# sortmerna/sortmerna

Hardware: AMD Instinct MI355X
Metric: reads/sec (150 bp vs smr_v4.3_default_db-sized DB) (higher is better)
Workload: dtype u8/i32

## Files before the change

### include/smr_hip.h

```cpp
#ifndef SMR_HIP_H
#define SMR_HIP_H
#include <stddef.h>
#include <stdint.h>

#ifdef __cplusplus
extern "C" {
#endif

#define SMR_OK 0
#define SMR_ERR_ARG (-1)
#define SMR_ERR_IO (-2)
#define SMR_ERR_DEVICE (-3)
#define SMR_ERR_CAPACITY (-4)
#define SMR_ERR_STATE (-5)

typedef struct smr_ctx smr_ctx;
typedef struct smr_index smr_index;
typedef struct smr_reads smr_reads;

typedef struct {
  uint32_t skiplengths[3];
  int32_t  num_seeds;
  int32_t  min_lis;
  int32_t  edges;
  int32_t  is_as_percent;
  int32_t  match;
  int32_t  mismatch;
  int32_t  score_N;
  int32_t  gap_open;
  int32_t  gap_ext;
  uint32_t num_alignments;
  int32_t  is_best;
  int32_t  is_full_search;
  int32_t  is_forward;
  int32_t  is_reverse;
  uint32_t minoccur;
  uint32_t minimal_score;
  uint32_t index_num;
  uint32_t part;
  int32_t  is_last_index_part;
} smr_params;

void smr_params_default(smr_params* p);
const char* smr_params_refused(const smr_params* p);

int smr_index_load_files(const char* prefix, uint32_t part, const char* ref_fasta, smr_index** out, char* err, size_t errcap);

int smr_index_build(const char* ref_fasta, uint32_t seed_win_len, double max_file_size_mb, uint32_t max_pos,
                    uint32_t threads, smr_index** parts_out, uint32_t cap_parts, uint32_t* n_parts_out,
                    char* err, size_t errcap);
int smr_index_write_files(const smr_index* const* parts, uint32_t n_parts, const char* ref_fasta, const char* prefix,
                          char* err, size_t errcap);
int smr_index_save(const smr_index*, const char* path, uint64_t stamp, char* err, size_t errcap);
int smr_index_load_flat(const char* path, uint64_t stamp, smr_index** out, char* err, size_t errcap);
int smr_index_selfcheck(smr_index*, char* err, size_t errcap);
void smr_index_free(smr_index*);

typedef struct {
  uint32_t lnwin;
  uint32_t n_kmers;
  uint64_t trie_words;
  uint32_t n_ids;
  uint64_t n_pos;
  uint32_t n_refs;
  uint64_t ref_bytes;
  uint64_t n_nodes, n_buckets, n_entries;
  double   bg[4];
  uint64_t full_len;
  uint64_t numseq;
  uint32_t n_parts;
} smr_index_info;
int smr_index_get_info(const smr_index*, smr_index_info* out);

uint32_t smr_minimal_score(double lambda, double K, const double bg[4], uint64_t full_ref_len, uint64_t numseq,
                           uint64_t all_reads_count, uint64_t all_reads_len, double evalue);
uint32_t smr_minimal_score_split(double lambda, double K, const double bg[4], uint64_t full_ref_len, uint64_t numseq,
                                 uint64_t all_reads_count, uint64_t all_reads_len, double evalue, uint32_t full_read_scale);

void smr_refstats_corrected(double K, const double bg[4], uint64_t full_ref_len, uint64_t numseq, uint64_t all_reads_count, uint64_t all_reads_len,
                            uint64_t* full_ref_corr, uint64_t* full_read_corr);
void smr_refstats_corrected_split(double K, const double bg[4], uint64_t full_ref_len, uint64_t numseq, uint64_t all_reads_count, uint64_t all_reads_len,
                                  uint32_t full_read_scale, uint64_t* full_ref_corr, uint64_t* full_read_corr);

int smr_reads_pack(const char* seqs, const uint64_t* offs, uint32_t n_reads, smr_reads** out);
int smr_reads_load_fastx(const char* path, uint64_t first, uint64_t count, smr_reads** out, char* err, size_t errcap);
int smr_reads_load_fastx_mt(const char* path, uint32_t threads, smr_reads** out, char* err, size_t errcap);
void smr_reads_free(smr_reads*);
int smr_reads_slice(const smr_reads*, uint64_t first, uint64_t count, smr_reads** out);
int smr_reads_load_fastx_text(const char* path, uint32_t threads, smr_reads** out, char* err, size_t errcap);
int smr_reads_is_fastq(const smr_reads*);
int smr_reads_record_text(const smr_reads*, uint32_t i, char* hdr, size_t hdr_cap, char* seq, size_t seq_cap, char* qual, size_t qual_cap, size_t lens[3]);
uint64_t smr_reads_digest(const smr_reads*);
uint32_t smr_reads_count(const smr_reads*);
uint64_t smr_reads_total_len(const smr_reads*);
uint32_t smr_reads_min_len(const smr_reads*);
uint32_t smr_reads_max_len(const smr_reads*);

int  smr_device_count(void);
int  smr_create(int device, smr_ctx** out, char* err, size_t errcap);
void smr_destroy(smr_ctx*);
const char* smr_last_error(const smr_ctx*);
int  smr_tuning_text(const smr_ctx*, char* buf, size_t cap);

int smr_index_upload(smr_ctx*, const smr_index*, int slot);
int smr_index_check_device(smr_ctx*, int slot, smr_index*);
int smr_index_pigeonhole(smr_index*, const uint32_t** pg, uint64_t* pg_words, const uint32_t** root3, uint64_t* root3_words, char* err, size_t errcap);
int smr_seed_tuples_fetch(smr_ctx*, uint64_t* tuples, uint64_t cap_tuples, uint32_t* cbase, uint32_t cap_cbase, uint32_t meta[8]);
int smr_seed_pool_info(smr_ctx*, uint64_t info[4]);
#define SMR_ROUTE_RECORD 1u
#define SMR_ROUTE_GATHER 2u
#define SMR_ROUTE_CHAIN 4u
#define SMR_ROUTE_EXT 8u
int smr_cand_info_enable(smr_ctx*, int on);
int smr_cand_info(smr_ctx*, uint64_t info[13]);
int smr_cand_routes(smr_ctx*, uint8_t* out, uint32_t n);
int smr_index_unload(smr_ctx*, int slot);

int smr_batch_select(smr_ctx*, int batch);

int smr_set_seed_mode(smr_ctx*, int exact_counters);

int smr_reads_upload(smr_ctx*, const smr_reads*, uint32_t max_alignments_per_read);
int smr_reads_upload_batch(smr_ctx*, int batch, const smr_reads*, uint32_t max_alignments_per_read);
#define SMR_FASTX_VIEW 1u
#define SMR_FASTX_KEEP 2u
#define SMR_FASTX_INFLATE 4u
int smr_reads_upload_fastx(smr_ctx*, const char* text, uint64_t n_bytes, uint32_t max_alignments_per_read, uint32_t flags, smr_reads** out);
int smr_reads_upload_fastx_batch(smr_ctx*, int batch, const char* text, uint64_t n_bytes, uint32_t max_alignments_per_read, uint32_t flags, smr_reads** out);
int smr_reads_upload_fastx_file(smr_ctx*, const char* path, uint32_t max_alignments_per_read, uint32_t flags, smr_reads** out, char* err, size_t errcap);
int smr_fastx_info(const smr_ctx*, uint64_t info[4]);
int smr_fastx_times(const smr_ctx*, double ms[5]);
typedef struct {
  int32_t layout;
  int32_t paired_in, paired_out, out2, sout;
  int32_t want_aligned, want_other;
} smr_fxsplit_opts;
int smr_fastx_split(smr_ctx*, int mates , const smr_fxsplit_opts*,
                    const uint8_t* hit , uint8_t* bytes, uint64_t cap, uint64_t off[9], uint64_t* need);
int smr_fastx_split_times(const smr_ctx*, double ms[4]);
typedef struct {
  int  want_sam, want_blast;
  char blast_cols[64];
  double lambda, K;
  uint64_t full_ref_corr, full_read_corr;
} smr_rows_opts;
int smr_rows_part(smr_ctx*, int slot, const smr_params*, const smr_index* ix, const smr_rows_opts*,
                  uint8_t* bytes, uint64_t cap, uint64_t off[3], uint64_t* need);
int smr_rows_times(const smr_ctx*, double ms[4]);
int smr_rows_fmt_batch(smr_ctx*, uint32_t n, const uint32_t* num, const uint32_t* den, char* out);
int smr_pairwise_part(smr_ctx*, int slot, const smr_params*, const smr_index* ix, double lambda, double K, uint64_t full_ref_corr, uint64_t full_read_corr,
                      uint8_t* bytes, uint64_t cap, uint64_t* need);
int smr_pairwise_times(const smr_ctx*, double ms[4]);
typedef struct { uint32_t ref_num, n_reads; uint64_t off; } smr_otu_group;
int smr_otu_part(smr_ctx*, int slot, const smr_params*, const smr_index* ix, double min_id, double min_cov,
                 uint8_t* bytes, uint64_t cap, smr_otu_group* groups, uint64_t groups_cap, uint64_t need[2] , int* any_yid_ycov);
int smr_otu_times(const smr_ctx*, double ms[5]);
int smr_otu_sort_batch(smr_ctx*, uint32_t n, const uint32_t* keys, uint32_t key_bits, uint32_t* perm);
int smr_fastx_denovo(smr_ctx*, int mates, const smr_fxsplit_opts*, const uint8_t* dn ,
                     uint8_t* bytes, uint64_t cap, uint64_t off[5], uint64_t* need);

uint32_t smr_gzip_chunk(void);
uint64_t smr_gzip_bound(uint64_t plain_bytes, uint64_t n_chunks);
int smr_gzip_batch(smr_ctx*, const uint8_t* plain, const uint64_t* off , uint32_t n_streams,
                   uint8_t* gz, uint64_t cap, uint64_t* gz_off , uint64_t* need);
int smr_fastx_split_gz(smr_ctx*, int mates, const smr_fxsplit_opts*, const uint8_t* hit,
                       uint8_t* gz, uint64_t cap, uint64_t gz_off[9], uint64_t plain_off[9], uint64_t* need);
int smr_fastx_denovo_gz(smr_ctx*, int mates, const smr_fxsplit_opts*, const uint8_t* dn,
                        uint8_t* gz, uint64_t cap, uint64_t gz_off[5], uint64_t plain_off[5], uint64_t* need);
uint64_t smr_gzip_lines_bound(uint64_t plain_bytes, uint32_t n_streams);
int smr_gzip_lines_batch(smr_ctx*, const uint8_t* plain, const uint64_t* off , uint32_t n_streams,
                         uint8_t* gz, uint64_t cap, uint64_t* gz_off , uint64_t* need);
int smr_rows_part_gz(smr_ctx*, int slot, const smr_params*, const smr_index* ix, const smr_rows_opts*,
                     uint8_t* gz, uint64_t cap, uint64_t gz_off[3], uint64_t plain_off[3], uint64_t* need);
int smr_pairwise_part_gz(smr_ctx*, int slot, const smr_params*, const smr_index* ix, double lambda, double K, uint64_t full_ref_corr, uint64_t full_read_corr,
                         uint8_t* gz, uint64_t cap, uint64_t* plain_bytes, uint64_t* need);
int smr_gzip_times(const smr_ctx*, double ms[5]);

int smr_rows_part_mates(smr_ctx*, int mates, int slot, const smr_params*, const smr_index* ix, const smr_rows_opts*,
                        uint8_t* bytes, uint64_t cap, uint64_t off[3], uint64_t* need);
int smr_pairwise_part_mates(smr_ctx*, int mates, int slot, const smr_params*, const smr_index* ix, double lambda, double K,
                            uint64_t full_ref_corr, uint64_t full_read_corr, uint8_t* bytes, uint64_t cap, uint64_t* need);
int smr_rows_part_mates_gz(smr_ctx*, int mates, int slot, const smr_params*, const smr_index* ix, const smr_rows_opts*,
                           uint8_t* gz, uint64_t cap, uint64_t gz_off[3], uint64_t plain_off[3], uint64_t* need);
int smr_pairwise_part_mates_gz(smr_ctx*, int mates, int slot, const smr_params*, const smr_index* ix, double lambda, double K,
                               uint64_t full_ref_corr, uint64_t full_read_corr, uint8_t* gz, uint64_t cap,
                               uint64_t* plain_bytes, uint64_t* need);
int smr_interleave_batch(smr_ctx*, uint32_t n, const uint8_t* a, const uint64_t* a_off, const uint8_t* b, const uint64_t* b_off,
                         uint8_t* out, uint64_t cap, uint64_t* need);
int smr_mates_times(const smr_ctx*, double ms[4]);

int smr_gunzip_batch(smr_ctx*, const uint8_t* gz, uint64_t n, uint64_t grain , uint8_t* plain, uint64_t cap, uint64_t* need);
int smr_gunzip_info(const smr_ctx*, uint64_t info[8]);
int smr_gunzip_times(const smr_ctx*, double ms[6]);
int smr_gunzip_tasks(const smr_ctx*, uint64_t* starts, uint64_t cap, uint64_t* count);
int smr_state_reset(smr_ctx*);

int smr_align_part(smr_ctx*, int slot, const smr_params*);
int smr_traceback(smr_ctx*, int slot, const smr_params*);

int smr_counters(smr_ctx*, uint64_t* out, uint32_t n_db);
int smr_counters_device(smr_ctx*, void** dptr, uint32_t* n_u64);
int smr_counters_accumulate(smr_ctx*, void* d_acc, uint32_t n_u64);

int smr_idcov_part(smr_ctx*, int slot, const smr_params*, double min_id, double min_cov);
int smr_idcov_counters(smr_ctx*, uint64_t out[4]);
int smr_idcov_counters_device(smr_ctx*, void** dptr, uint32_t* n_u64);
#define SMR_COUNTERS_WITH_IDCOV 70
int smr_idcov_batch(smr_ctx*, uint32_t n, const uint8_t* reads, const uint64_t* read_off, const uint8_t* refs, const uint64_t* ref_off,
                    const uint32_t* cigars, const uint64_t* cigar_off, const int32_t* read_begin, const int32_t* read_end, const uint32_t* readlen,
                    double min_id, double min_cov, uint32_t* out);

int    smr_results_fetch(smr_ctx*);
size_t smr_result_record(const smr_ctx*, uint32_t read_idx, uint8_t* buf, size_t cap);
size_t smr_result_record_batch(const smr_ctx*, int batch, uint32_t read_idx, uint8_t* buf, size_t cap);
int    smr_result_is_hit(const smr_ctx*, uint32_t read_idx);

int smr_state_import(smr_ctx*, const uint8_t* bytes, const uint64_t* off, uint32_t n);
int smr_state_export(smr_ctx*, uint8_t* bytes, uint64_t cap, uint64_t* off, uint32_t n, uint64_t* need);
int smr_counters_import(smr_ctx*, const uint64_t* in, uint32_t n_db);

int smr_seed_scan(smr_ctx*, int slot, const smr_params*, int strand, int pass, uint64_t* n_hits_out);
int smr_seed_hits_fetch(smr_ctx*, uint32_t* triples, uint64_t cap_triples, uint64_t* n_out);

typedef struct {
  double   seed_ms;  uint64_t seed_launches;
  double   chain_ms; uint64_t chain_launches;
  double   trace_ms; uint64_t trace_launches;
  uint64_t n_windows, n_lookup, n_node, n_entry, n_hit, n_read_bytes;
  uint64_t n_sw_fwd, n_sw_rev, n_sw_cells;
  uint64_t n_sw_spec, n_sw_spec_used;
  uint64_t n_seed_redo;
  uint64_t hit_list_cap;
  uint64_t n_seed_shared;
  uint64_t n_seed_shared_builds;
} smr_prof;
int smr_index_build_gpu(smr_ctx*, const char* ref_fasta, uint32_t lnwin, double max_mb, uint32_t max_pos,
                        smr_index** parts_out, uint32_t cap_parts, uint32_t* n_parts_out, char* err, size_t errcap);

int smr_sw_selfcheck(smr_ctx*, uint32_t n_cases, uint32_t seed, uint32_t max_len, uint64_t* n_bad);
int smr_sw_mode(smr_ctx*, int set_to);
int smr_walk_rounds(const smr_ctx*, uint32_t out[3]);
int smr_ssw_batch(smr_ctx*, uint32_t n_pairs, const uint8_t* reads, const uint64_t* read_off, const uint8_t* refs, const uint64_t* ref_off,
                  int match, int mismatch, int score_N, int gap_open, int gap_ext, uint32_t filters, int mode, int32_t* out);
int smr_sw_long_rows(int m);
typedef struct {
  uint32_t read, win_off;
  uint16_t aq, m, nref;
  uint8_t reversed, list_b;
} smr_sw16_task;
int smr_sw16_batch(smr_ctx*, uint32_t n_tasks, const smr_sw16_task* tasks, const uint8_t* ref, uint64_t ref_len, int force_any_n,
                   int match, int mismatch, int score_N, int gap_open, int gap_ext, uint32_t filters, int rows, uint32_t blocks, int32_t* out);
typedef struct {
  uint32_t read, win_off;
  uint16_t aq, m, nref, cols;
  uint8_t reversed, pad_[3];
} smr_sw16_prefix_task;
int smr_sw16_prefix_batch(smr_ctx*, uint32_t n_tasks, const smr_sw16_prefix_task* tasks, const uint8_t* ref, uint64_t ref_len, int force_any_n,
                          int match, int mismatch, int score_N, int gap_open, int gap_ext, int rows, uint32_t blocks, int32_t* out);
int smr_walk_prefix_stats(smr_ctx*, uint64_t out[8]);
int smr_sw16_launches(const smr_ctx*, uint64_t out[8]);
int smr_sw16_f16(smr_ctx*, int set_to, uint64_t* launches);
// ... 80 lines not shown
```

### sortmerna_amd/capi.py

```python
import ctypes as C
import os

from . import build as _build


class Params(C.Structure):
    _fields_ = [
        ("skiplengths", C.c_uint32 * 3), ("num_seeds", C.c_int32), ("min_lis", C.c_int32), ("edges", C.c_int32),
        ("is_as_percent", C.c_int32), ("match", C.c_int32), ("mismatch", C.c_int32), ("score_N", C.c_int32),
        ("gap_open", C.c_int32), ("gap_ext", C.c_int32), ("num_alignments", C.c_uint32), ("is_best", C.c_int32),
        ("is_full_search", C.c_int32), ("is_forward", C.c_int32), ("is_reverse", C.c_int32), ("minoccur", C.c_uint32),
        ("minimal_score", C.c_uint32), ("index_num", C.c_uint32), ("part", C.c_uint32),
        ("is_last_index_part", C.c_int32),
    ]


class IndexInfo(C.Structure):
    _fields_ = [
        ("lnwin", C.c_uint32), ("n_kmers", C.c_uint32), ("trie_words", C.c_uint64), ("n_ids", C.c_uint32),
        ("n_pos", C.c_uint64), ("n_refs", C.c_uint32), ("ref_bytes", C.c_uint64), ("n_nodes", C.c_uint64),
        ("n_buckets", C.c_uint64), ("n_entries", C.c_uint64), ("bg", C.c_double * 4), ("full_len", C.c_uint64),
        ("numseq", C.c_uint64), ("n_parts", C.c_uint32),
    ]


class ReportOpts(C.Structure):
    _fields_ = [("fastx", C.c_int), ("other", C.c_int), ("blast_tabular", C.c_int), ("blast_cols", C.c_char * 64), ("sam", C.c_int),
                ("blast_pairwise", C.c_int), ("sam_sq", C.c_int), ("paired_in", C.c_int), ("paired_out", C.c_int), ("out2", C.c_int), ("sout", C.c_int), ("zip_out", C.c_int),
                ("otu_map", C.c_int), ("denovo", C.c_int), ("min_id", C.c_double), ("min_cov", C.c_double)]


class FxSplitOpts(C.Structure):
    _fields_ = [("layout", C.c_int32), ("paired_in", C.c_int32), ("paired_out", C.c_int32), ("out2", C.c_int32), ("sout", C.c_int32),
                ("want_aligned", C.c_int32), ("want_other", C.c_int32)]


class RowsOpts(C.Structure):
    _fields_ = [("want_sam", C.c_int), ("want_blast", C.c_int), ("blast_cols", C.c_char * 64), ("lam", C.c_double), ("K", C.c_double),
                ("full_ref_corr", C.c_uint64), ("full_read_corr", C.c_uint64)]


class SummaryDb(C.Structure):
    _fields_ = [("ref_file", C.c_char_p), ("skiplengths", C.c_uint32 * 3), ("lam", C.c_double), ("K", C.c_double),
                ("minimal_score", C.c_uint32), ("reads_matched", C.c_uint64)]


class Summary(C.Structure):
    _fields_ = [("cmdline", C.c_char_p), ("pid", C.c_char_p), ("timestamp", C.c_char_p), ("seed_len", C.c_uint32),
                ("num_seeds", C.c_int32), ("edges", C.c_int32), ("match", C.c_int32), ("mismatch", C.c_int32), ("gap_open", C.c_int32),
                ("gap_ext", C.c_int32), ("score_N", C.c_int32), ("sam_sq", C.c_int32), ("threads", C.c_int32),
                ("reads_files", C.POINTER(C.c_char_p)), ("n_reads_files", C.c_uint32),
                ("total_reads", C.c_uint64), ("num_aligned", C.c_uint64), ("all_reads_len", C.c_uint64),
                ("min_read_len", C.c_uint32), ("max_read_len", C.c_uint32), ("dbs", C.POINTER(SummaryDb)), ("n_dbs", C.c_uint32),
                ("is_denovo", C.c_int), ("total_denovo", C.c_uint64), ("is_otu_map", C.c_int), ("total_id_cov", C.c_uint64), ("total_otu", C.c_uint64)]


class Prof(C.Structure):
    _fields_ = [
        ("seed_ms", C.c_double), ("seed_launches", C.c_uint64), ("chain_ms", C.c_double), ("chain_launches", C.c_uint64),
        ("trace_ms", C.c_double), ("trace_launches", C.c_uint64), ("n_windows", C.c_uint64), ("n_lookup", C.c_uint64),
        ("n_node", C.c_uint64), ("n_entry", C.c_uint64), ("n_hit", C.c_uint64), ("n_read_bytes", C.c_uint64),
        ("n_sw_fwd", C.c_uint64), ("n_sw_rev", C.c_uint64), ("n_sw_cells", C.c_uint64), ("n_sw_spec", C.c_uint64), ("n_sw_spec_used", C.c_uint64), ("n_seed_redo", C.c_uint64), ("hit_list_cap", C.c_uint64),
        ("n_seed_shared", C.c_uint64), ("n_seed_shared_builds", C.c_uint64),
    ]


class Kprof(C.Structure):
    _fields_ = [("name", C.c_char * 32), ("ms", C.c_double), ("launches", C.c_uint64), ("bytes", C.c_uint64)]


EXPORTS = [
    "smr_rows_part_mates", "smr_pairwise_part_mates", "smr_rows_part_mates_gz", "smr_pairwise_part_mates_gz", "smr_interleave_batch", "smr_mates_times",
    "smr_gzip_lines_bound", "smr_gzip_lines_batch", "smr_rows_part_gz", "smr_pairwise_part_gz", "smr_report_add_rows_gz", "smr_report_add_pairwise_gz",
    "smr_gunzip_batch", "smr_gunzip_info", "smr_gunzip_times", "smr_gunzip_tasks",
    "smr_gzip_chunk", "smr_gzip_bound", "smr_gzip_batch", "smr_fastx_split_gz", "smr_fastx_denovo_gz", "smr_gzip_times", "smr_report_add_fastx_gz", "smr_report_add_denovo_gz",
    "smr_otu_part", "smr_otu_times", "smr_otu_sort_batch", "smr_fastx_denovo", "smr_report_add_otu", "smr_report_skip_otu", "smr_report_add_denovo", "smr_report_skip_denovo",
    "smr_params_default", "smr_params_refused", "smr_index_load_files", "smr_index_build", "smr_index_build_gpu", "smr_index_write_files", "smr_index_save", "smr_index_load_flat", "smr_index_selfcheck", "smr_index_free",
    "smr_index_get_info", "smr_minimal_score", "smr_minimal_score_split", "smr_refstats_corrected_split", "smr_reads_pack", "smr_reads_load_fastx", "smr_reads_load_fastx_mt", "smr_reads_load_fastx_text", "smr_reads_is_fastq", "smr_reads_record_text", "smr_reads_free", "smr_reads_slice",
    "smr_reads_digest", "smr_reads_count", "smr_reads_total_len", "smr_reads_min_len", "smr_reads_max_len", "smr_create", "smr_device_count", "smr_destroy",
    "smr_last_error", "smr_tuning_text", "smr_index_upload", "smr_index_check_device", "smr_index_pigeonhole", "smr_seed_tuples_fetch", "smr_seed_pool_info", "smr_cand_info_enable", "smr_cand_info", "smr_cand_routes", "smr_index_unload", "smr_batch_select", "smr_set_seed_mode", "smr_reads_upload", "smr_reads_upload_batch", "smr_reads_upload_fastx", "smr_reads_upload_fastx_batch", "smr_reads_upload_fastx_file", "smr_fastx_info", "smr_fastx_times", "smr_fastx_split", "smr_fastx_split_times", "smr_rows_part", "smr_rows_times", "smr_rows_fmt_batch", "smr_pairwise_part", "smr_pairwise_times", "smr_state_reset", "smr_align_part",
    "smr_traceback", "smr_counters", "smr_counters_device", "smr_state_import", "smr_state_export", "smr_counters_import", "smr_results_fetch", "smr_result_record", "smr_result_record_batch", "smr_counters_accumulate",
    "smr_result_is_hit", "smr_seed_scan", "smr_seed_hits_fetch", "smr_sw_selfcheck", "smr_sw_mode", "smr_walk_rounds", "smr_ssw_batch", "smr_sw16_batch", "smr_sw16_prefix_batch", "smr_walk_prefix_stats", "smr_sw16_launches", "smr_sw16_f16", "smr_sw_long_rows", "smr_cigar_batch", "smr_idcov_part", "smr_idcov_counters", "smr_idcov_counters_device", "smr_idcov_batch", "smr_prof_reset", "smr_prof_get", "smr_prof_kernels", "smr_refstats_corrected", "smr_report_open",
    "smr_report_set_db", "smr_report_set_part", "smr_report_add", "smr_report_add_pair", "smr_report_add_fastx", "smr_report_skip_fastx", "smr_report_add_rows", "smr_report_skip_rows", "smr_report_add_pairwise", "smr_report_skip_pairwise", "smr_report_set_cmdline", "smr_report_otu_count", "smr_report_otu_merge", "smr_report_close", "smr_report_last_error",
    "smr_summary_write", "smr_readstats_record", "smr_readstats_key",
]

_lib = None


def load(rebuild_if_stale=True):
    global _lib
    if _lib is not None:
        return _lib
    path = _build.LIB
    if rebuild_if_stale and _build.is_stale():
        path = _build.build_library()
    if not os.path.isfile(path):
        raise RuntimeError("libsmr_hip.so is missing; run sortmerna_amd/build.py (needs hipcc)")
    _lib = bind(C.CDLL(path))
    return _lib


def bind(L):
    vp, cp, u32, u64, i32 = C.c_void_p, C.c_char_p, C.c_uint32, C.c_uint64, C.c_int
    L.smr_params_default.argtypes = [C.POINTER(Params)]
    L.smr_index_load_files.restype = i32
    L.smr_index_load_files.argtypes = [cp, u32, cp, C.POINTER(vp), cp, C.c_size_t]
    L.smr_index_build.restype = i32
    L.smr_index_build.argtypes = [cp, u32, C.c_double, u32, u32, C.POINTER(vp), u32, C.POINTER(u32), cp, C.c_size_t]
    L.smr_index_build_gpu.restype = i32
    L.smr_index_build_gpu.argtypes = [vp, cp, u32, C.c_double, u32, C.POINTER(vp), u32, C.POINTER(u32), cp, C.c_size_t]
    L.smr_index_write_files.restype = i32
    L.smr_index_write_files.argtypes = [C.POINTER(vp), u32, cp, cp, cp, C.c_size_t]
    L.smr_index_save.restype = i32
    L.smr_index_save.argtypes = [vp, cp, u64, cp, C.c_size_t]
    L.smr_index_load_flat.restype = i32
    L.smr_index_load_flat.argtypes = [cp, u64, C.POINTER(vp), cp, C.c_size_t]
    L.smr_index_selfcheck.restype = i32
    L.smr_index_selfcheck.argtypes = [vp, cp, C.c_size_t]
    L.smr_index_free.argtypes = [vp]
    L.smr_index_get_info.restype = i32
    L.smr_index_get_info.argtypes = [vp, C.POINTER(IndexInfo)]
    L.smr_minimal_score.restype = u32
    L.smr_minimal_score.argtypes = [C.c_double, C.c_double, C.POINTER(C.c_double), u64, u64, u64, u64, C.c_double]
    L.smr_minimal_score_split.restype = u32
    L.smr_minimal_score_split.argtypes = [C.c_double, C.c_double, C.POINTER(C.c_double), u64, u64, u64, u64, C.c_double, u32]
    L.smr_reads_pack.restype = i32
    L.smr_reads_pack.argtypes = [cp, vp, u32, C.POINTER(vp)]
    L.smr_reads_load_fastx.restype = i32
    L.smr_reads_load_fastx.argtypes = [cp, u64, u64, C.POINTER(vp), cp, C.c_size_t]
    L.smr_reads_load_fastx_mt.restype = i32
    L.smr_reads_load_fastx_mt.argtypes = [cp, u32, C.POINTER(vp), cp, C.c_size_t]
    L.smr_reads_load_fastx_text.restype = i32
    L.smr_reads_load_fastx_text.argtypes = [cp, u32, C.POINTER(vp), cp, C.c_size_t]
    L.smr_reads_is_fastq.restype = i32
    L.smr_reads_is_fastq.argtypes = [vp]
    L.smr_reads_record_text.restype = i32
    L.smr_reads_record_text.argtypes = [vp, u32, cp, C.c_size_t, cp, C.c_size_t, cp, C.c_size_t, C.POINTER(C.c_size_t)]
    L.smr_reads_free.argtypes = [vp]
    for f in ("smr_reads_count", "smr_reads_min_len", "smr_reads_max_len"):
        getattr(L, f).restype = u32
        getattr(L, f).argtypes = [vp]
    L.smr_reads_digest.restype = u64
    L.smr_reads_digest.argtypes = [vp]
    L.smr_reads_total_len.restype = u64
    L.smr_reads_total_len.argtypes = [vp]
    L.smr_create.restype = i32
    L.smr_create.argtypes = [i32, C.POINTER(vp), cp, C.c_size_t]
    L.smr_destroy.argtypes = [vp]
    L.smr_last_error.restype = cp
    L.smr_last_error.argtypes = [vp]
    L.smr_tuning_text.restype = i32
    L.smr_tuning_text.argtypes = [vp, cp, C.c_size_t]
    L.smr_index_upload.restype = i32
    L.smr_index_upload.argtypes = [vp, vp, i32]
    L.smr_index_check_device.restype = i32
    L.smr_index_check_device.argtypes = [vp, i32, vp]
    L.smr_index_pigeonhole.restype = i32
    L.smr_index_pigeonhole.argtypes = [vp, C.POINTER(C.POINTER(C.c_uint32)), C.POINTER(u64), C.POINTER(C.POINTER(C.c_uint32)), C.POINTER(u64), cp, C.c_size_t]
    L.smr_seed_tuples_fetch.restype = i32
    L.smr_seed_tuples_fetch.argtypes = [vp, vp, u64, vp, u32, C.POINTER(u32)]
    L.smr_seed_pool_info.restype = i32
    L.smr_seed_pool_info.argtypes = [vp, C.POINTER(u64)]
    L.smr_cand_info_enable.restype = i32
    L.smr_cand_info_enable.argtypes = [vp, i32]
    L.smr_cand_info.restype = i32
    L.smr_cand_info.argtypes = [vp, C.POINTER(u64)]
    L.smr_cand_routes.restype = i32
    L.smr_cand_routes.argtypes = [vp, vp, u32]
    L.smr_index_unload.restype = i32
    L.smr_index_unload.argtypes = [vp, i32]
    L.smr_batch_select.restype = i32
    L.smr_batch_select.argtypes = [vp, i32]
    L.smr_set_seed_mode.restype = i32
    L.smr_set_seed_mode.argtypes = [vp, i32]
    L.smr_reads_upload.restype = i32
    L.smr_reads_upload.argtypes = [vp, vp, u32]
    L.smr_state_reset.restype = i32
    L.smr_state_reset.argtypes = [vp]
    L.smr_align_part.restype = i32
    L.smr_align_part.argtypes = [vp, i32, C.POINTER(Params)]
    L.smr_traceback.restype = i32
    L.smr_traceback.argtypes = [vp, i32, C.POINTER(Params)]
    L.smr_counters.restype = i32
    L.smr_counters.argtypes = [vp, C.POINTER(u64), u32]
    L.smr_state_import.restype = i32
    L.smr_state_import.argtypes = [vp, vp, vp, u32]
    L.smr_state_export.restype = i32
    L.smr_state_export.argtypes = [vp, vp, u64, vp, u32, C.POINTER(u64)]
    L.smr_counters_import.restype = i32
    L.smr_counters_import.argtypes = [vp, C.POINTER(u64), u32]
    L.smr_counters_device.restype = i32
    L.smr_counters_device.argtypes = [vp, C.POINTER(vp), C.POINTER(u32)]
    L.smr_results_fetch.restype = i32
    L.smr_results_fetch.argtypes = [vp]
    L.smr_result_record.restype = C.c_size_t
    L.smr_result_record.argtypes = [vp, u32, vp, C.c_size_t]
    L.smr_result_record_batch.restype = C.c_size_t
    L.smr_result_record_batch.argtypes = [vp, i32, u32, vp, C.c_size_t]
    L.smr_counters_accumulate.restype = i32
    L.smr_counters_accumulate.argtypes = [vp, vp, u32]
    L.smr_result_is_hit.restype = i32
    L.smr_result_is_hit.argtypes = [vp, u32]
    L.smr_seed_scan.restype = i32
    L.smr_seed_scan.argtypes = [vp, i32, C.POINTER(Params), i32, i32, C.POINTER(u64)]
    L.smr_seed_hits_fetch.restype = i32
    L.smr_seed_hits_fetch.argtypes = [vp, vp, u64, C.POINTER(u64)]
    L.smr_sw_selfcheck.restype = i32
    L.smr_sw_selfcheck.argtypes = [vp, u32, u32, u32, C.POINTER(u64)]
    L.smr_ssw_batch.restype = i32
    L.smr_ssw_batch.argtypes = [vp, u32, vp, vp, vp, vp, i32, i32, i32, i32, i32, u32, i32, vp]
    L.smr_sw16_batch.restype = i32
    L.smr_sw16_batch.argtypes = [vp, u32, vp, vp, u64, i32, i32, i32, i32, i32, i32, u32, i32, u32, vp]
    L.smr_sw16_prefix_batch.restype = i32
    L.smr_sw16_prefix_batch.argtypes = [vp, u32, vp, vp, u64, i32, i32, i32, i32, i32, i32, i32, u32, vp]
    L.smr_walk_prefix_stats.restype = i32
    L.smr_walk_prefix_stats.argtypes = [vp, C.POINTER(u64)]
    L.smr_sw16_launches.restype = i32
    L.smr_sw16_launches.argtypes = [vp, C.POINTER(u64)]
    L.smr_sw16_f16.restype = i32
    L.smr_sw16_f16.argtypes = [vp, i32, C.POINTER(u64)]
    L.smr_sw_long_rows.restype = i32
    L.smr_sw_long_rows.argtypes = [i32]
    L.smr_readstats_record.restype = C.c_size_t
    L.smr_readstats_record.argtypes = [u64, u64, u32, u32, u64, u64, vp, u32, vp, C.c_size_t]
    L.smr_readstats_key.restype = C.c_size_t
    L.smr_readstats_key.argtypes = [vp, u32, vp, C.c_size_t]
    L.smr_reads_upload_batch.restype = i32
    L.smr_reads_upload_batch.argtypes = [vp, i32, vp, u32]
    L.smr_reads_upload_fastx.restype = i32
    L.smr_reads_upload_fastx.argtypes = [vp, vp, u64, u32, u32, C.POINTER(vp)]
    L.smr_reads_upload_fastx_batch.restype = i32
    L.smr_reads_upload_fastx_batch.argtypes = [vp, i32, vp, u64, u32, u32, C.POINTER(vp)]
    L.smr_reads_upload_fastx_file.restype = i32
    L.smr_reads_upload_fastx_file.argtypes = [vp, cp, u32, u32, C.POINTER(vp), cp, C.c_size_t]
    L.smr_fastx_info.restype = i32
    L.smr_fastx_info.argtypes = [vp, C.POINTER(u64)]
    L.smr_fastx_times.restype = i32
    L.smr_fastx_times.argtypes = [vp, C.POINTER(C.c_double)]
    L.smr_fastx_split.restype = i32
    L.smr_fastx_split.argtypes = [vp, i32, C.POINTER(FxSplitOpts), vp, vp, u64, C.POINTER(u64), C.POINTER(u64)]
    L.smr_fastx_split_times.restype = i32
    L.smr_fastx_split_times.argtypes = [vp, C.POINTER(C.c_double)]
    L.smr_rows_part.restype = i32
    L.smr_rows_part.argtypes = [vp, i32, C.POINTER(Params), vp, C.POINTER(RowsOpts), vp, u64, C.POINTER(u64), C.POINTER(u64)]
    L.smr_rows_times.restype = i32
    L.smr_rows_times.argtypes = [vp, C.POINTER(C.c_double)]
    L.smr_rows_fmt_batch.restype = i32
    L.smr_rows_fmt_batch.argtypes = [vp, u32, vp, vp, vp]
    L.smr_report_add_rows.restype = i32
    L.smr_report_add_rows.argtypes = [vp, u32, u32, vp, C.POINTER(u64)]
    L.smr_report_skip_rows.restype = i32
    L.smr_report_skip_rows.argtypes = [vp, i32]
    L.smr_pairwise_part.restype = i32
    L.smr_pairwise_part.argtypes = [vp, i32, C.POINTER(Params), vp, C.c_double, C.c_double, u64, u64, vp, u64, C.POINTER(u64)]
    L.smr_pairwise_times.restype = i32
    L.smr_pairwise_times.argtypes = [vp, C.POINTER(C.c_double)]
    L.smr_report_add_pairwise.restype = i32
    L.smr_report_add_pairwise.argtypes = [vp, u32, u32, vp, u64]
    L.smr_report_skip_pairwise.restype = i32
    L.smr_report_skip_pairwise.argtypes = [vp, i32]
    L.smr_otu_part.restype = i32
    L.smr_otu_part.argtypes = [vp, i32, C.POINTER(Params), vp, C.c_double, C.c_double, vp, u64, vp, u64, C.POINTER(u64), C.POINTER(i32)]
    L.smr_otu_times.restype = i32
    L.smr_otu_times.argtypes = [vp, C.POINTER(C.c_double)]
    L.smr_otu_sort_batch.restype = i32
    L.smr_otu_sort_batch.argtypes = [vp, u32, vp, u32, vp]
    L.smr_fastx_denovo.restype = i32
    L.smr_fastx_denovo.argtypes = [vp, i32, C.POINTER(FxSplitOpts), vp, vp, u64, C.POINTER(u64), C.POINTER(u64)]
    L.smr_gzip_chunk.restype = u32
    L.smr_gzip_chunk.argtypes = []
    L.smr_gzip_bound.restype = u64
    L.smr_gzip_bound.argtypes = [u64, u64]
    L.smr_gzip_batch.restype = i32
    L.smr_gzip_batch.argtypes = [vp, vp, C.POINTER(u64), u32, vp, u64, C.POINTER(u64), C.POINTER(u64)]
    L.smr_fastx_split_gz.restype = i32
    L.smr_fastx_split_gz.argtypes = [vp, i32, C.POINTER(FxSplitOpts), vp, vp, u64, C.POINTER(u64), C.POINTER(u64), C.POINTER(u64)]
    L.smr_fastx_denovo_gz.restype = i32
    L.smr_fastx_denovo_gz.argtypes = [vp, i32, C.POINTER(FxSplitOpts), vp, vp, u64, C.POINTER(u64), C.POINTER(u64), C.POINTER(u64)]
    L.smr_gzip_times.restype = i32
    L.smr_gzip_times.argtypes = [vp, C.POINTER(C.c_double)]
    L.smr_gzip_lines_bound.restype = u64
    L.smr_gzip_lines_bound.argtypes = [u64, u32]
    L.smr_gzip_lines_batch.restype = i32
    L.smr_gzip_lines_batch.argtypes = [vp, vp, C.POINTER(u64), u32, vp, u64, C.POINTER(u64), C.POINTER(u64)]
    L.smr_rows_part_mates.restype = i32
    L.smr_rows_part_mates.argtypes = [vp, i32, i32, C.POINTER(Params), vp, C.POINTER(RowsOpts), vp, u64, C.POINTER(u64), C.POINTER(u64)]
    L.smr_pairwise_part_mates.restype = i32
    L.smr_pairwise_part_mates.argtypes = [vp, i32, i32, C.POINTER(Params), vp, C.c_double, C.c_double, u64, u64, vp, u64, C.POINTER(u64)]
    L.smr_rows_part_mates_gz.restype = i32
    L.smr_rows_part_mates_gz.argtypes = [vp, i32, i32, C.POINTER(Params), vp, C.POINTER(RowsOpts), vp, u64, C.POINTER(u64), C.POINTER(u64), C.POINTER(u64)]
    L.smr_pairwise_part_mates_gz.restype = i32
    L.smr_pairwise_part_mates_gz.argtypes = [vp, i32, i32, C.POINTER(Params), vp, C.c_double, C.c_double, u64, u64, vp, u64, C.POINTER(u64), C.POINTER(u64)]
    L.smr_interleave_batch.restype = i32
    L.smr_interleave_batch.argtypes = [vp, u32, vp, C.POINTER(u64), vp, C.POINTER(u64), vp, u64, C.POINTER(u64)]
    L.smr_mates_times.restype = i32
    L.smr_mates_times.argtypes = [vp, C.POINTER(C.c_double)]
    L.smr_rows_part_gz.restype = i32
    L.smr_rows_part_gz.argtypes = [vp, i32, C.POINTER(Params), vp, C.POINTER(RowsOpts), vp, u64, C.POINTER(u64), C.POINTER(u64), C.POINTER(u64)]
    L.smr_pairwise_part_gz.restype = i32
    L.smr_pairwise_part_gz.argtypes = [vp, i32, C.POINTER(Params), vp, C.c_double, C.c_double, u64, u64, vp, u64, C.POINTER(u64), C.POINTER(u64)]
    L.smr_report_add_rows_gz.restype = i32
    L.smr_report_add_rows_gz.argtypes = [vp, u32, u32, vp, C.POINTER(u64)]
    L.smr_report_add_pairwise_gz.restype = i32
    L.smr_report_add_pairwise_gz.argtypes = [vp, u32, u32, vp, u64]
    L.smr_gunzip_batch.restype = i32
    L.smr_gunzip_batch.argtypes = [vp, vp, u64, u64, vp, u64, C.POINTER(u64)]
    L.smr_gunzip_info.restype = i32
    L.smr_gunzip_info.argtypes = [vp, C.POINTER(u64)]
    L.smr_gunzip_times.restype = i32
    L.smr_gunzip_times.argtypes = [vp, C.POINTER(C.c_double)]
    L.smr_gunzip_tasks.restype = i32
    L.smr_gunzip_tasks.argtypes = [vp, C.POINTER(u64), u64, C.POINTER(u64)]
    L.smr_report_add_fastx_gz.restype = i32
    L.smr_report_add_fastx_gz.argtypes = [vp, vp, C.POINTER(u64)]
    L.smr_report_add_denovo_gz.restype = i32
# ... 64 lines not shown
```

### sortmerna_amd/csrc/smr_devbuf.hpp

```cpp
#pragma once
#include <hip/hip_runtime.h>

#include <cstddef>

struct smr_ctx;
int dev_fail(smr_ctx* c, const char* call, hipError_t e);

template <class T> class DevBuf {
  T* p_ = nullptr;
  size_t cap_ = 0;

 public:
  DevBuf() = default;
  DevBuf(const DevBuf&) = delete;
  DevBuf& operator=(const DevBuf&) = delete;
  DevBuf(DevBuf&& o) noexcept : p_(o.p_), cap_(o.cap_) { o.p_ = nullptr; o.cap_ = 0; }
  DevBuf& operator=(DevBuf&& o) noexcept {
    if (this != &o) { release(); p_ = o.p_; cap_ = o.cap_; o.p_ = nullptr; o.cap_ = 0; }
    return *this;
  }
  ~DevBuf() { release(); }

  operator T*() const { return p_; }
  T* get() const { return p_; }
  size_t cap() const { return cap_; }

  void release() {
    if (p_) (void)hipFree(p_);
    p_ = nullptr; cap_ = 0;
  }
  int alloc(smr_ctx* c, size_t count) {
    release();
    if (count == 0) count = 1;
    const hipError_t e = hipMalloc((void**)&p_, count * sizeof(T));
    if (e != hipSuccess) { p_ = nullptr; return dev_fail(c, "hipMalloc", e); }
    cap_ = count;
    return 0;
  }
  int reserve(smr_ctx* c, size_t need) { return (p_ && cap_ >= need) ? 0 : alloc(c, need); }
  int reserve_headroom(smr_ctx* c, size_t total, size_t slack) {
    return cap_ >= total + slack ? 0 : alloc(c, (size_t)((total + (total >> 3) + 4095u) & ~4095ull));
  }
};

struct DevStream {
  hipStream_t s = nullptr;
  DevStream() = default;
  DevStream(const DevStream&) = delete;
  DevStream& operator=(const DevStream&) = delete;
  ~DevStream() { if (s) (void)hipStreamDestroy(s); }
  operator hipStream_t() const { return s; }
};
```

### sortmerna_amd/csrc/smr_engine.hip

```cpp
#include <hip/hip_runtime.h>

#include <algorithm>
#include <mutex>
#include <cstdio>
#include <cstdlib>
#include <cstring>
#include <string>
#include <vector>

#include "smr_kernels.hpp"
#include "smr_idcov.hpp"
#include "smr_import.hpp"
#include "smr_export.hpp"
#include "smr_fastx.hpp"
#include "smr_fxsplit.hpp"
#include "smr_rows.hpp"
#include "smr_pairwise.hpp"
#include "smr_mates.hpp"
#include "smr_otu.hpp"
#include "smr_gzip.hpp"
#include "smr_gunzip.hpp"
#include "smr_ibuild.hpp"
#include "smr_pgbuild.hpp"
#include "smr_hostmem.hpp"
#include "smr_devbuf.hpp"
#include "smr_stage.hpp"
#include "smr_score_text.hpp"
#include "smr_tuning.hpp"

using namespace smr;

namespace {

struct DevIndex {
  bool used = false;
  DevBuf<Lookup> lookup; DevBuf<uint32_t> trie, pos_off; DevBuf<uint2> pos_arr;
  DevBuf<uint32_t> pg, root3, lkc;
  DevBuf<uint8_t> ref_seq; DevBuf<uint64_t> ref_off;
  uint32_t n_refs = 0, n_ids = 0, lnwin = 0;
  uint32_t ref_any_n = 1;
  uint64_t trie_words = 0, n_pos = 0, ref_bytes = 0, pg_words = 0;
  DevBuf<uint8_t> rows_names; DevBuf<uint32_t> rows_name_off; int64_t rows_part = -1;
};

struct EvMark { hipEvent_t e; int kind; };
struct EvPool {
  std::vector<EvMark> events; std::vector<hipEvent_t> pool;
  EvPool() = default;
  EvPool(const EvPool&) = delete;
  EvPool& operator=(const EvPool&) = delete;
  ~EvPool() { for (auto& m : events) (void)hipEventDestroy(m.e); for (auto& e : pool) (void)hipEventDestroy(e); }
};

}

#define SMR_MAX_BATCHES 16
enum { KP_KEYS = 0, KP_SPLIT, KP_BINS, KP_PG0, KP_PG1, KP_FINISH, KP_CAND, KP_CHAIN, KP_BEGINS, KP_TRACE, KP_WALK, KP_SW16, KP_WNEXT, KP_IDCOV, KP_COUNT };
static const char* const KP_NAME[KP_COUNT] = {"k_seed_keys", "k_seed_split", "k_seed_bins", "k_seed_pg<0>", "k_seed_pg<1>", "k_seed_finish", "k_cand", "k_chain", "k_begins", "k_trace",
                                              "k_walk", "k_sw16", "k_wnext", "k_idcov"};

struct Batch {
  bool used = false;
  uint32_t n = 0, max_len = 0, slots = 1;
  uint32_t min_ge[7] = {~0u, ~0u, ~0u, ~0u, ~0u, ~0u, ~0u};
  uint64_t gen = 0;
  bool min_ge_known = false;
  DevBuf<uint32_t> d_words; DevBuf<uint64_t> d_rec_off; DevBuf<uint32_t> d_len;
  DevBuf<RState> d_saved, d_work; DevBuf<RWork> d_rw;
  DevBuf<uint8_t> d_marks;
  DevBuf<AlignRec> d_saved_aln, d_work_aln;
  DevBuf<unsigned long long> d_ctr;
  DevBuf<uint32_t> d_cigar; uint64_t cigar_words = 0;
  DevBuf<uint32_t> d_idcov; bool idcov_ran = false;
  std::vector<uint32_t> h_idcov;
  std::vector<RState> h_state; std::vector<AlignRec> h_aln; std::vector<uint32_t> h_cigar;
  std::vector<uint32_t> h_idx, h_map;
  uint32_t last_num_alignments = 1;
  DevBuf<uint8_t> fx_text; DevBuf<unsigned long long> fx_hoff, fx_soff; uint32_t fx_n = 0; bool fx_fastq = false, fx_kept = false;
  unsigned long long redo_seen = 0, win_seen = 0;
  bool fetched = false;
};

struct SharedSet { DevBuf<SeedTup> srt; DevBuf<uint16_t> wbin; DevBuf<uint32_t> cbase, sn; uint32_t maxwin = 0; bool built = false; };
struct SharedSort {
  SharedSet set[2][3];
  const void* batch = nullptr; uint64_t gen = 0; uint32_t lnwin = 0, skip[3] = {0, 0, 0}, n = 0, max_len = 0;
  uint64_t cap[3] = {0, 0, 0};
  bool usable = false;
  DevBuf<uint32_t> abits;
};
struct SeedScratch {
  DevBuf<uint32_t> chist, cbase, rows, bcnt, wseg[2], fbits[2], zbits, gflag, emap, sn, redo, hpre, hlist, hh;
  DevBuf<SeedTup> tmp, mid, srt; DevBuf<uint16_t> wbin; DevBuf<uint2> pieces;
};

struct FxScratch {
  DevBuf<uint8_t> text;
  DevBuf<uint32_t> tot, part_t, part_l, line_start, lrec, lcum, hdr_line, rcum, rlen, rwi;
  DevBuf<unsigned long long> hoff, soff;
  StageClock<6, 0> clk;
};

struct FxSplitScratch {
  DevBuf<uint4> rec; DevBuf<unsigned long long> woff, part, tot; DevBuf<uint8_t> hit, out;
  StageClock<6, 4> clk;
};

struct RowsScratch {
  DevBuf<uint4> stat, meta; DevBuf<unsigned long long> excl_s, excl_b, part_s, part_b; DevBuf<uint32_t> err; DevBuf<uint8_t> tab, out;
  uint32_t tab_n = 0; double tab_lambda = 0, tab_K = 0; uint64_t tab_ref = 0, tab_read = 0;
  StageClock<7, 4> clk;
};

struct OtuScratch {
  DevBuf<uint8_t> pass, out; DevBuf<uint2> meta; DevBuf<uint4> pairs; DevBuf<uint32_t> key[2], val[2], gstart, err;
  DevBuf<unsigned long long> excl, part, hist, wexcl, wpart, gexcl, gpart; DevBuf<OtuGroup> groups;
  StageClock<10, 5> clk;
};

struct GzScratch {
  DevBuf<uint8_t> in, slots, out; DevBuf<GzChunk> chunks; DevBuf<GzCode> codes; DevBuf<unsigned long long> slot_off, sizes, cut_tab;
  DevBuf<uint32_t> crc_tab, crc, tok, freq, ntok;
  StageClock<4, 5> clk;
};

struct GunzScratch {
  DevBuf<uint32_t> in, n_cand, crc; DevBuf<unsigned long long> cand; DevBuf<GunzTask> tasks; DevBuf<GunzRes> res; DevBuf<GunzUnit> units;
  DevBuf<uint16_t> sym; DevBuf<uint8_t> win, out;
  StageClock<8, 6> clk;
};

struct smr_ctx {
  const Tuning tune;
  explicit smr_ctx(const Tuning& t) : tune(t) {}
  int device = 0;
  DevStream stream, upload_stream;
  std::string err;
  std::mutex err_m, sel_m;
  int n_cu = 256;
  DevIndex idx[64];
  Batch bt[SMR_MAX_BATCHES];
  Batch* b = &bt[0];
  DevBuf<uint32_t> d_pool; uint64_t pool_words = 0;
  uint64_t n_pool_grown = 0;
  uint32_t pool_inline = 0;
  uint32_t hcap = 4;
  int seed_exact = tune.seed_exact;
  uint32_t cand_bloom = tune.cand_bloom;
  int seed_shared = tune.seed_shared;
  DevBuf<uint16_t> d_sw_scr; uint32_t sw_scr_stride = 0;
  int last_seed_slot = -1;
  SharedSort shared;
  uint64_t n_seed_shared = 0, n_seed_shared_builds = 0;
  uint32_t ccap = tune.ccap;
  SeedScratch seed; SeedBufs sb = {};
  uint64_t sb_slots = 0; uint32_t sb_nk = 0;
  uint32_t chain_blocks = 0;
  DevBuf<unsigned long long> d_tuples; uint32_t chain_scap = 512;
  uint32_t keys_need = 0;
  bool chain_ext = false;
  DevBuf<uint32_t> d_stab; DevBuf<unsigned long long> d_tuples2;
  size_t chain_lds_attr = 0, begins_lds_attr = 0, split_lds_attr = 0, bins_lds_attr = 0;
  DevBuf<uint32_t> d_fidx; DevBuf<RState> d_fstate; DevBuf<AlignRec> d_faln;
  DevBuf<uint32_t> d_fidcov;
  DevBuf<uint8_t> d_xbytes; DevBuf<unsigned long long> d_xoff, d_xpart;
  int sw_mode = tune.sw_packed;
  DevBuf<unsigned long long> d_keys; uint32_t keys_cap = 0;
  DevBuf<unsigned long long> d_pairs; DevBuf<uint32_t> d_lis; uint32_t pairs_cap = 0;
  DevBuf<uint2> d_hits; uint32_t hits_cap = 0;
  DevBuf<uint8_t> d_rdq;
  DevBuf<uint2> d_mrec; DevBuf<uint32_t> d_mpool;
  DevBuf<uint2> d_wlist[2]; DevBuf<WState> d_wstate[2]; DevBuf<WTask> d_wtask[2]; DevBuf<uint2> d_wres[2];
  DevBuf<uint32_t> d_wtidx, d_wslow; DevBuf<unsigned long long> d_wctr; size_t walk_cap = 0; uint32_t walk_kcap = 0;
  size_t walk_lds_attr = 0, pg_lds_attr = 0, search_lds_attr = 0;
  int sw16_f16 = tune.sw16_f16;
  uint64_t sw16h_launches = 0;
  uint64_t sw16_launches[8] = {};
  uint32_t walk_need[3] = {0, 0, 0};
  DevBuf<unsigned long long> d_wpstat;
  bool pfx_live = true; uint32_t pfx_parts_off = 0; unsigned long long pfx_seen[2] = {0, 0};
  DevBuf<unsigned long long> d_wstat; uint32_t wstat_n = 0; int wstat_pass[8] = {}; uint32_t wstat_rm[8] = {};
  DevBuf<int> d_bound;
  DevBuf<uint32_t> d_tasks;
  DevBuf<uint8_t> d_trflags;
  DevBuf<int> d_trrows;
  EvPool ev;
  double kp_ms[KP_COUNT] = {}; uint64_t kp_l[KP_COUNT] = {};
  DevBuf<unsigned long long> d_ctr_snap;
  bool cinfo_on = false; DevBuf<uint8_t> d_croute; uint32_t croute_n = 0;
  uint32_t cinfo_attempts = 0, cinfo_retry[5] = {0, 0, 0, 0, 0};
  FxScratch fx[2];
  uint64_t fx_info[4] = {0, 0, 0, 0}; double fx_ms[5] = {0, 0, 0, 0, 0};
  FxSplitScratch fxs;
  RowsScratch rows;
  StageClock<7, 4> pair_clk;
  RowsScratch rows_m;
  DevBuf<uint8_t> mates_out; DevBuf<unsigned long long> mates_off;
  StageClock<7, 4> mates_clk[2];
  StageClock<3, 2> mates_zip_clk;
  OtuScratch otu;
  GzScratch gz;
  std::mutex gz_tab_m;
  GunzScratch gunz[2];
  uint64_t gunz_info[8] = {}; double gunz_ms[6] = {}; std::vector<uint64_t> gunz_tasks;
};
struct KpSave { double ms[KP_COUNT]; uint64_t l[KP_COUNT]; };

#define SEED_REDO_CAP 16384u

int dev_fail(smr_ctx* c, const char* call, hipError_t e) {
  std::lock_guard<std::mutex> l_(c->err_m);
  c->err = std::string(call) + ": " + hipGetErrorString(e);
  return SMR_ERR_DEVICE;
}

namespace {

#define HIPCHK(ctx, call)                                          \
  do {                                                             \
    hipError_t e_ = (call);                                        \
    if (e_ != hipSuccess) return dev_fail((ctx), #call, e_);       \
  } while (0)

void set_err(smr_ctx* c, const std::string& msg) { std::lock_guard<std::mutex> l_(c->err_m); c->err = msg; }


template <class T> struct arg_of { typedef T type; };
template <class... P> void launch(smr_ctx* c, void (*k)(P...), dim3 grid, dim3 block, size_t lds, typename arg_of<P>::type... a) {
  hipLaunchKernelGGL(k, grid, block, lds, c->stream, a...);
}
template <class... P> void launch_on(hipStream_t st, void (*k)(P...), dim3 grid, dim3 block, size_t lds, typename arg_of<P>::type... a) {
  hipLaunchKernelGGL(k, grid, block, lds, st, a...);
}
template <class... F> int raise_lds_limit(smr_ctx* c, size_t& high_water, size_t bytes, size_t free_bytes, F... kernels) {
  if (bytes <= free_bytes || bytes <= high_water) return SMR_OK;
  for (const void* k : {(const void*)kernels...}) HIPCHK(c, hipFuncSetAttribute(k, hipFuncAttributeMaxDynamicSharedMemorySize, (int)bytes));
  high_water = bytes;
  return SMR_OK;
}

const char* scheme_unsupported(int mismatch, int score_N, int gap_open, int gap_ext);
DParams make_dparams(const smr_ctx* c, const DevIndex& di, const smr_params* p) {
  DParams P;
  memset(&P, 0, sizeof P);
  P.lnwin = di.lnwin; P.partialwin = di.lnwin / 2;
  if (p->skiplengths[0] == 0 || p->skiplengths[1] == 0 || p->skiplengths[2] == 0) {
    P.skip[0] = di.lnwin; P.skip[1] = di.lnwin / 2; P.skip[2] = 3;
  } else { P.skip[0] = p->skiplengths[0]; P.skip[1] = p->skiplengths[1]; P.skip[2] = p->skiplengths[2]; }
  P.num_seeds = p->num_seeds; P.min_lis = p->min_lis; P.edges = p->edges; P.is_as_percent = p->is_as_percent;
  P.match = p->match; P.mismatch = p->mismatch; P.score_N = p->score_N; P.gap_open = p->gap_open; P.gap_ext = p->gap_ext;
  P.minimal_score = p->minimal_score; P.num_alignments = p->num_alignments;
  P.is_best = p->is_best; P.is_full_search = p->is_full_search; P.is_forward = p->is_forward; P.is_reverse = p->is_reverse;
  P.minoccur = p->minoccur; P.index_num = p->index_num; P.part = p->part; P.is_last_index_part = p->is_last_index_part;
  P.slots = c->b->slots;
  P.sw_mode = scheme_unsupported(p->mismatch, p->score_N, p->gap_open, p->gap_ext) ? -1 : c->sw_mode;
  P.sw_scratch = c->d_sw_scr; P.sw_scratch_stride = c->sw_scr_stride;
  return P;
}

const char* scheme_unsupported(int mismatch, int score_N, int gap_open, int gap_ext) {
  const int mm = std::max(-mismatch, -std::min(score_N, 0));
  if (2 * gap_open < mm || 2 * gap_ext < mm) return "scoring scheme outside the supported range (2*gap_open and 2*gap_ext must be >= |mismatch|)";
  if (score_N > 0) return "scoring scheme outside the supported range (score_N must be <= 0: the kernels pad sequences with N)";
  if (gap_open <= gap_ext) return "scoring scheme outside the supported range (gap_open must be greater than gap_ext: the reference's 16-bit kernel ends its lazy-F loop early otherwise, ssw.c:496-507)";
  return nullptr;
}

int check_params(smr_ctx* c, const smr_params* p, bool sw = true) {
  if (!p) { set_err(c, "null params"); return SMR_ERR_ARG; }
  if (p->index_num >= 64) { set_err(c, "index_num must be < 64"); return SMR_ERR_ARG; }
  if ((uint64_t)p->minoccur >= 0x3FFFFFFFull) { set_err(c, "minoccur must be < 2^30 - 1"); return SMR_ERR_ARG; }
  if (p->num_seeds < 1 || p->gap_open < 0 || p->gap_ext < 0 || p->match <= 0 || p->mismatch > 0) { set_err(c, "bad scoring/seed options"); return SMR_ERR_ARG; }
  if (p->match > 127 || p->mismatch < -127 || p->score_N > 127 || p->score_N < -127 || p->gap_open > 255 || p->gap_ext > 255) { set_err(c, "scores must fit int8 / gaps uint8 like the reference's"); return SMR_ERR_ARG; }
  if (sw && (p->edges < 1 || p->edges > 10)) { set_err(c, "edges must be 1..10 (nucleotides or percent), like the reference's --edges"); return SMR_ERR_ARG; }
  if (p->num_alignments > 0 && p->num_alignments > c->b->slots) { set_err(c, "num_alignments exceeds max_alignments_per_read given to smr_reads_upload"); return SMR_ERR_ARG; }
  return SMR_OK;
}

int part_refuse_state(smr_ctx* c, const char* who, uint32_t no_cigar, uint32_t bad_ref, uint32_t past) {
  const std::string W = std::string(who) + ": ";
  if (no_cigar) { set_err(c, W + std::to_string(no_cigar) + " alignments of this (index, part) have no CIGAR yet (call smr_traceback first)"); return SMR_ERR_STATE; }
  if (bad_ref) { set_err(c, W + std::to_string(bad_ref) + " alignments with ref_num out of range"); return SMR_ERR_ARG; }
  if (past) { set_err(c, W + std::to_string(past) + " alignments whose CIGAR runs past its read or its reference"); return SMR_ERR_ARG; }
  return SMR_OK;
}

DIndex dindex(const DevIndex& d) {
  DIndex x; x.lookup = d.lookup; x.trie = d.trie; x.pg = d.pg; x.lkc = d.lkc; x.root3 = reinterpret_cast<const uint2*>(d.root3.get()); x.pos_off = d.pos_off; x.pos_arr = d.pos_arr; x.ref_seq = d.ref_seq; x.ref_off = d.ref_off;
  x.n_refs = d.n_refs; x.n_ids = d.n_ids; x.lnwin = d.lnwin; x.partialwin = d.lnwin / 2; x.ref_any_n = d.ref_any_n;
  return x;
}
DReads dreads(const Batch& b) { DReads r; r.words = b.d_words; r.rec_off = b.d_rec_off; r.len = b.d_len; r.n = b.n; r.max_len = b.max_len; return r; }
DReads dreads(const smr_ctx* c) { return dreads(*c->b); }

constexpr uint32_t CHAIN_WAVES_PER_CU = 12;
uint32_t chain_blocks(smr_ctx* c) {
  if (c->chain_blocks == 0) c->chain_blocks = (uint32_t)c->n_cu * CHAIN_WAVES_PER_CU;
  return c->chain_blocks;
}
int ensure_chain_scratch(smr_ctx* c) {
  const size_t nb = chain_blocks(c);
  int rc;
  const uint32_t need_keys = std::max(std::max(c->chain_scap, 1024u), c->keys_need);
  if (c->keys_cap < need_keys) { if ((rc = c->d_keys.alloc(c, nb * need_keys))) return rc; c->keys_cap = need_keys; }
  if (c->pairs_cap == 0) c->pairs_cap = 4096;
  if (!c->d_pairs && ((rc = c->d_pairs.alloc(c, nb * c->pairs_cap)) || (rc = c->d_lis.alloc(c, nb * 2 * c->pairs_cap)) || (rc = c->d_tuples.alloc(c, nb * c->pairs_cap)))) return rc;
  if (c->chain_ext) {
    if (!c->d_stab && (rc = c->d_stab.alloc(c, nb * 4 * CH_EXT_CAP))) return rc;
    if (!c->d_tuples2 && (rc = c->d_tuples2.alloc(c, nb * c->pairs_cap))) return rc;
  }
  if (c->hits_cap == 0) c->hits_cap = 4096;
  if (!c->d_hits && (rc = c->d_hits.alloc(c, nb * c->hits_cap))) return rc;
  return SMR_OK;
}

void ev_mark(smr_ctx* c, int kind) {
  EvMark m; m.kind = kind;
  if (!c->ev.pool.empty()) { m.e = c->ev.pool.back(); c->ev.pool.pop_back(); }
  else (void)hipEventCreate(&m.e);
  (void)hipEventRecord(m.e, c->stream);
  c->ev.events.push_back(m);
}
void ev_stop(smr_ctx* c) { ev_mark(c, -1); }
void ev_drop(smr_ctx* c) {
  for (auto& m : c->ev.events) c->ev.pool.push_back(m.e);
  c->ev.events.clear();
}
void ev_collect(smr_ctx* c) {
  for (size_t i = 0; i + 1 < c->ev.events.size(); i++) {
    const int k = c->ev.events[i].kind;
    float ms = 0;
    if (k >= 0 && hipEventElapsedTime(&ms, c->ev.events[i].e, c->ev.events[i + 1].e) == hipSuccess) { c->kp_ms[k] += ms; c->kp_l[k]++; }
  }
  ev_drop(c);
}
KpSave kp_save(const smr_ctx* c) { KpSave k; memcpy(k.ms, c->kp_ms, sizeof k.ms); memcpy(k.l, c->kp_l, sizeof k.l); return k; }
void kp_restore(smr_ctx* c, const KpSave& k) { memcpy(c->kp_ms, k.ms, sizeof k.ms); memcpy(c->kp_l, k.l, sizeof k.l); }

uint32_t num_windows(uint32_t max_len, uint32_t L, uint32_t stride) {
  return max_len >= L ? (max_len - L + stride) / stride : 1;
}

#include "smr_engine_seed.hpp"
#include "smr_engine_chain.hpp"
}


#include "smr_engine_ibuild.hpp"

#include "smr_engine_swseam.hpp"

extern "C" int smr_device_count(void) {
  int n = 0;
  return hipGetDeviceCount(&n) == hipSuccess ? n : 0;
}

extern "C" int smr_create(int device, smr_ctx** out, char* err, size_t errcap) {
  if (!out) return SMR_ERR_ARG;
  int ndev = 0;
  hipError_t e = hipGetDeviceCount(&ndev);
  if (e != hipSuccess || ndev == 0) {
    if (err && errcap) snprintf(err, errcap, "no HIP device available (%s): libsmr_hip has no CPU fallback", e == hipSuccess ? "count=0" : hipGetErrorString(e));
    return SMR_ERR_DEVICE;
  }
  if (device < 0 || device >= ndev) { if (err && errcap) snprintf(err, errcap, "device %d out of range (%d devices)", device, ndev); return SMR_ERR_ARG; }
  const TuningLimits lim = {WK_MAX, PG_CAND_CAP0, PG_CAND_CAP_MAX, CAND_BLOOM_WORDS, C_NSHARD, SEED_HOT_BIN_MIN, SEED_HOT_SUB, SMR_SW_SELFCHECK_CASES};
  auto c = new smr_ctx(read_tuning(lim));
  c->device = device;
  if (hipSetDevice(device) != hipSuccess || hipStreamCreate(&c->stream.s) != hipSuccess || hipStreamCreate(&c->upload_stream.s) != hipSuccess ||
      c->d_ctr_snap.alloc(c, C_TOTAL) != SMR_OK) {
    if (err && errcap) snprintf(err, errcap, "cannot initialise device %d", device);
    delete c; return SMR_ERR_DEVICE;
  }
  say(c->tune, "environment switches of this context:\n%s", tuning_text(c->tune).c_str());
  hipDeviceProp_t prop;
  if (hipGetDeviceProperties(&prop, device) == hipSuccess) c->n_cu = prop.multiProcessorCount;
  if (c->b->d_ctr.alloc(c, C_TOTAL) != SMR_OK) { if (err && errcap) snprintf(err, errcap, "hipMalloc failed"); delete c; return SMR_ERR_DEVICE; }
  (void)hipMemset(c->b->d_ctr, 0, C_TOTAL * 8);
  c->b->used = true;
  if (c->sw_mode >= 1) {
    const uint32_t cases = c->tune.sw_selfcheck;
    uint64_t bad = 0;
    if (cases > 0 && (smr_sw_selfcheck(c, cases, 20260926u, 700, &bad) != SMR_OK || bad != 0)) {
      fprintf(stderr, "libsmr_hip: packed Smith-Waterman kernel disagrees with the 32-bit kernel on %llu self-check cases; using the 32-bit kernel\n", (unsigned long long)bad);
      c->sw_mode = 0;
    }
  }
  if (c->sw16_f16) {
    uint64_t bad = 0;
    const uint32_t cases = c->tune.sw_selfcheck;
    if (cases > 0 && (sw16h_selfcheck(c, cases, 20261019u, &bad) != SMR_OK || bad != 0)) {
      say(c->tune, "k_sw16h (packed f16) disagrees with k_sw16 on %llu self-check results; using k_sw16\n", (unsigned long long)bad);
      c->sw16_f16 = 0;
    }
    c->sw16h_launches = 0;
  }
  *out = c;
  return SMR_OK;
}

extern "C" void smr_destroy(smr_ctx* c) {
  if (!c) return;
  (void)hipSetDevice(c->device);
  (void)hipStreamSynchronize(c->stream);
  delete c;
}

extern "C" int smr_tuning_text(const smr_ctx* c, char* buf, size_t cap) {
  if (!c) return SMR_ERR_ARG;
  const std::string s = tuning_text(c->tune);
  if (buf && cap > s.size()) memcpy(buf, s.c_str(), s.size() + 1);
  return (int)s.size() + 1;
}

extern "C" const char* smr_last_error(const smr_ctx* c) {
  if (!c) return "null context";
  static thread_local std::string copy;
  { std::lock_guard<std::mutex> l(const_cast<smr_ctx*>(c)->err_m); copy = c->err; }
  return copy.c_str();
}

namespace {
__global__ void __launch_bounds__(256) k_pos2_build(const uint32_t* __restrict__ pos_off, const uint2* __restrict__ pos_arr, uint32_t n_ids, uint2* __restrict__ pos2) {
  const uint32_t id = blockIdx.x * blockDim.x + threadIdx.x;
  if (id >= n_ids) return;
  const uint32_t lo = pos_off[id], n = pos_off[id + 1] - lo;
  uint2* o = pos2 + (size_t)lo + id;
  o[0] = make_uint2(n, id);
  for (uint32_t q = 0; q < n; q++) o[1 + q] = pos_arr[lo + q];
}

int build_pigeonhole_device(smr_ctx* c, DevIndex& d, uint32_t nk, uint32_t pw) {
  DevPool pool;
  const uint32_t nb = 2 * nk;
  IB_GET(cnt, uint32_t, nb); IB_GET(eoff, uint32_t, nb); IB_GET(words, smr::u64, nb); IB_GET(woff, smr::u64, nb); IB_GET(derr, uint32_t, 1);
  HIPCHK(c, hipMemsetAsync(derr, 0, 4, c->stream));
  launch(c, smr::k_pgb_sizes, dim3((nb + 255) / 256), dim3(256), 0, (const Lookup*)d.lookup, (const uint32_t*)d.trie, nk, pw, cnt, words);
  smr::u64 W = 0;
  int rc = dev_scan<smr::u64>(c, pool, words, woff, nb, &W); if (rc) return rc;
  if (W / 3 > 0xFFFFFFF0ull || W / 4 > 0xFFFFFFF0ull) { set_err(c, "pigeonhole arena exceeds 2^34 words"); return SMR_ERR_CAPACITY; }
  uint32_t E = 0;
  if ((rc = dev_scan<uint32_t>(c, pool, cnt, eoff, nb, &E))) return rc;
  if ((rc = d.pg.alloc(c, (size_t)W + 4))) return rc;
  if ((rc = d.root3.alloc(c, (size_t)2 * nb))) return rc;
  HIPCHK(c, hipMemsetAsync(d.pg + W, 0, 16, c->stream));
  IB_GET(estr, uint32_t, E); IB_GET(eid, uint32_t, E); IB_GET(eblk, uint32_t, E);
  IB_GET(k0, smr::u64, E); IB_GET(k1, smr::u64, E); IB_GET(v0, uint32_t, E); IB_GET(v1, uint32_t, E);
  launch(c, smr::k_pgb_collect, dim3((nb + 255) / 256), dim3(256), 0, (const Lookup*)d.lookup, (const uint32_t*)d.trie, nk, pw,
                     (const uint32_t*)cnt, (const uint32_t*)eoff, (const smr::u64*)woff, d.root3, d.pg, estr, eid, eblk, derr, (const uint32_t*)d.pos_off);
  uint32_t herr = 0;
  HIPCHK(c, hipMemcpyAsync(&herr, derr, 4, hipMemcpyDeviceToHost, c->stream));
  HIPCHK(c, hipStreamSynchronize(c->stream));
  if (herr) { set_err(c, (herr & 1u) ? "a mini-trie is too large for the pigeonhole layout" : "pigeonhole arena exceeds 2^34 words"); return SMR_ERR_CAPACITY; }
  int blockbits = 1; while ((1u << blockbits) < nb) blockbits++;
  const uint32_t gE = (uint32_t)(((smr::u64)E + 255) / 256);
  for (int order = 0; order < 2 && E; order++) {
    const uint32_t kbits = order == 0 ? 2 * (pw + 1) : 2 * (pw - pw / 2);
    smr::u64 *ka = k0, *kb = k1; uint32_t *va = v0, *vb = v1;
    if (order == 0) launch(c, smr::k_pgb_keys<0>, dim3(gE), dim3(256), 0, (const uint32_t*)estr, (const uint32_t*)eblk, (smr::u64)E, pw, kbits, ka, va);
    else launch(c, smr::k_pgb_keys<1>, dim3(gE), dim3(256), 0, (const uint32_t*)estr, (const uint32_t*)eblk, (smr::u64)E, pw, kbits, ka, va);
    if ((rc = dev_radix_sort(c, pool, ka, kb, va, vb, E, 0, (int)kbits + blockbits))) return rc;
    if (order == 0) launch(c, smr::k_pgb_emit<0>, dim3(gE), dim3(256), 0, (const smr::u64*)ka, (const uint32_t*)va, (smr::u64)E, pw, kbits,
                                       (const uint32_t*)estr, (const uint32_t*)eid, (const uint32_t*)eoff, (const uint32_t*)d.root3, d.pg);
    else launch(c, smr::k_pgb_emit<1>, dim3(gE), dim3(256), 0, (const smr::u64*)ka, (const uint32_t*)va, (smr::u64)E, pw, kbits,
                            (const uint32_t*)estr, (const uint32_t*)eid, (const uint32_t*)eoff, (const uint32_t*)d.root3, d.pg);
  }
  HIPCHK(c, hipStreamSynchronize(c->stream));
  HIPCHK(c, hipGetLastError());
  d.pg_words = W;
  return SMR_OK;
}
}

extern "C" int smr_index_upload(smr_ctx* c, const smr_index* ix, int slot) {
  if (!c || !ix || slot < 0 || slot >= 64) return SMR_ERR_ARG;
  HIPCHK(c, hipSetDevice(c->device));
  if (c->idx[slot].used) smr_index_unload(c, slot);
  DevIndex& d = c->idx[slot];
  d.lnwin = ix->lnwin; d.n_refs = ix->n_refs(); d.n_ids = ix->n_ids(); d.trie_words = ix->trie.size(); d.n_pos = ix->pos_arr.size() / 2; d.ref_bytes = ix->ref_seq.size();
  int rc;
  smr_build_lkc(*const_cast<smr_index*>(ix));
  if ((rc = d.lkc.alloc(c, ix->lkc.size()))) return rc;
  HIPCHK(c, hipMemcpyAsync(d.lkc, ix->lkc.data(), ix->lkc.size() * 4, hipMemcpyHostToDevice, c->stream));
  if ((rc = d.lookup.alloc(c, ix->lookup.size()))) return rc;
  if ((rc = d.trie.alloc(c, ix->trie.size()))) return rc;
  HIPCHK(c, hipMemcpyAsync(d.lookup, ix->lookup.data(), ix->lookup.size() * sizeof(Lookup), hipMemcpyHostToDevice, c->stream));
  HIPCHK(c, hipMemcpyAsync(d.trie, ix->trie.data(), ix->trie.size() * 4, hipMemcpyHostToDevice, c->stream));
  if ((uint64_t)ix->pos_arr.size() / 2 + ix->n_ids() >= 0x7FFFFFF0ull) { set_err(c, "index part limit: positions + distinct seeds < 2^31"); return SMR_ERR_CAPACITY; }
  if ((rc = d.pos_off.alloc(c, ix->pos_off.size()))) return rc;
  HIPCHK(c, hipMemcpyAsync(d.pos_off, ix->pos_off.data(), ix->pos_off.size() * 4, hipMemcpyHostToDevice, c->stream));
  {
    DevBuf<uint2> raw;
    if ((rc = raw.alloc(c, ix->pos_arr.size() / 2))) return rc;
    HIPCHK(c, hipMemcpyAsync(raw, ix->pos_arr.data(), ix->pos_arr.size() * 4, hipMemcpyHostToDevice, c->stream));
    if ((rc = d.pos_arr.alloc(c, ix->pos_arr.size() / 2 + (size_t)d.n_ids + 1))) return rc;
    if (d.n_ids) launch(c, k_pos2_build, dim3((d.n_ids + 255u) / 256u), dim3(256), 0, d.pos_off, raw, d.n_ids, d.pos_arr);
    HIPCHK(c, hipStreamSynchronize(c->stream));
  }
  bool host_pg = c->tune.pg_host;
  { std::lock_guard<std::mutex> l_(const_cast<smr_index*>(ix)->pg_mutex); host_pg = host_pg || !ix->root3.empty(); }
  if (host_pg) {
    std::string why;
    if (!smr_build_pigeonhole(*const_cast<smr_index*>(ix), 0, why)) { set_err(c, why); return SMR_ERR_CAPACITY; }
    if ((rc = d.pg.alloc(c, ix->pg.size()))) return rc;
    if ((rc = d.root3.alloc(c, ix->root3.size()))) return rc;
    HIPCHK(c, hipMemcpyAsync(d.pg, ix->pg.data(), ix->pg.size() * 4, hipMemcpyHostToDevice, c->stream));
    HIPCHK(c, hipMemcpyAsync(d.root3, ix->root3.data(), ix->root3.size() * 4, hipMemcpyHostToDevice, c->stream));
    d.pg_words = ix->pg.size() >= 4 ? ix->pg.size() - 4 : 0;
  } else if ((rc = build_pigeonhole_device(c, d, (uint32_t)ix->lookup.size(), ix->lnwin / 2))) return rc;
  say(c->tune, "index part: tries %.2f GB, pigeonhole arena %.2f GB (%s), positions %.2f GB\n", ix->trie.size() * 4e-9, d.pg_words * 4e-9,
      host_pg ? "host-built" : "built on the device", ix->pos_arr.size() * 4e-9);
  if ((rc = d.ref_seq.alloc(c, ix->ref_seq.size() + 64))) return rc;
  if ((rc = d.ref_off.alloc(c, ix->ref_off.size()))) return rc;
  HIPCHK(c, hipMemcpyAsync(d.ref_seq, ix->ref_seq.data(), ix->ref_seq.size(), hipMemcpyHostToDevice, c->stream));
  d.ref_any_n = (!ix->ref_seq.empty() && memchr(ix->ref_seq.data(), 4, ix->ref_seq.size())) ? 1u : 0u;
  HIPCHK(c, hipMemcpyAsync(d.ref_off, ix->ref_off.data(), ix->ref_off.size() * 8, hipMemcpyHostToDevice, c->stream));
  HIPCHK(c, hipStreamSynchronize(c->stream));
  d.used = true;
  return SMR_OK;
}

extern "C" int smr_index_check_device(smr_ctx* c, int slot, smr_index* ix) {
  if (!c || !ix || slot < 0 || slot >= 64 || !c->idx[slot].used) return SMR_ERR_ARG;
  HIPCHK(c, hipSetDevice(c->device));
  const DevIndex& d = c->idx[slot];
  std::string why;
  if (!smr_build_pigeonhole(*ix, 0, why)) { set_err(c, why); return SMR_ERR_CAPACITY; }
  if (ix->pg.size() != d.pg_words + 4) { set_err(c, "pigeonhole layout: the device arena has " + std::to_string(d.pg_words) + " words, the host's " + std::to_string(ix->pg.size() - 4)); return SMR_ERR_STATE; }
  std::vector<uint32_t> r3(ix->root3.size()), pg(ix->pg.size());
  HIPCHK(c, hipMemcpy(r3.data(), d.root3, r3.size() * 4, hipMemcpyDeviceToHost));
  HIPCHK(c, hipMemcpy(pg.data(), d.pg, pg.size() * 4, hipMemcpyDeviceToHost));
  for (size_t q = 0; q < r3.size(); q++) if (r3[q] != ix->root3[q]) { set_err(c, "pigeonhole layout: block table differs at word " + std::to_string(q)); return SMR_ERR_STATE; }
  for (size_t q = 0; q < pg.size(); q++) if (pg[q] != ix->pg.data()[q]) { set_err(c, "pigeonhole layout: arena differs at word " + std::to_string(q)); return SMR_ERR_STATE; }
  return SMR_OK;
}

extern "C" int smr_index_unload(smr_ctx* c, int slot) {
  if (!c || slot < 0 || slot >= 64) return SMR_ERR_ARG;
  c->idx[slot] = DevIndex();
  return SMR_OK;
}

extern "C" int smr_batch_select(smr_ctx* c, int batch) {
  if (!c || batch < 0 || batch >= SMR_MAX_BATCHES) return SMR_ERR_ARG;
  HIPCHK(c, hipSetDevice(c->device));
  Batch& B = c->bt[batch];
  if (!B.d_ctr) {
    int rc = B.d_ctr.alloc(c, C_TOTAL); if (rc) return rc;
    HIPCHK(c, hipMemset(B.d_ctr, 0, C_TOTAL * 8));
  }
  B.used = true;
  { std::lock_guard<std::mutex> l(c->sel_m); c->b = &B; }
  return SMR_OK;
}

extern "C" int smr_set_seed_mode(smr_ctx* c, int exact_counters) {
  if (!c) return SMR_ERR_ARG;
  c->seed_exact = exact_counters ? 1 : 0;
  return SMR_OK;
}

namespace {
int reset_batch(smr_ctx* c, Batch& B, hipStream_t st) {
  B.gen++;
  HIPCHK(c, hipMemsetAsync(B.d_saved, 0, (size_t)B.n * sizeof(RState), st));
  HIPCHK(c, hipMemsetAsync(B.d_saved_aln, 0, (size_t)B.n * B.slots * sizeof(AlignRec), st));
  HIPCHK(c, hipMemsetAsync(B.d_ctr, 0, (size_t)C_WINDOWS * 8, st));
  HIPCHK(c, hipMemsetAsync(B.d_ctr + C_ERR_HITCAP, 0, (size_t)(C_SW_SPEC - C_ERR_HITCAP) * 8, st));
  HIPCHK(c, hipMemsetAsync(B.d_ctr + C_PCUR, 0, (size_t)C_NSHARD * C_PCUR_STRIDE * 8, st));
  HIPCHK(c, hipMemsetAsync(B.d_ctr + C_IDCOV, 0, 4 * 8, st));
  if (B.d_idcov) HIPCHK(c, hipMemsetAsync(B.d_idcov, 0, std::min(B.d_idcov.cap() / 4, (size_t)B.n) * 16, st));
  B.idcov_ran = false;
  HIPCHK(c, hipStreamSynchronize(st));
  B.fetched = false;
  return SMR_OK;
}
int batch_reserve(smr_ctx* c, Batch& B, size_t words, uint32_t n, uint32_t min_len, uint32_t max_len, uint32_t max_aln, hipStream_t st) {
  int rc;
  if (B.fx_kept) { B.fx_text.release(); B.fx_hoff.release(); B.fx_soff.release(); B.fx_n = 0; B.fx_kept = false; }
  if (!B.d_ctr) { if ((rc = B.d_ctr.alloc(c, C_TOTAL))) return rc; HIPCHK(c, hipMemsetAsync(B.d_ctr, 0, C_TOTAL * 8, st)); }
  const size_t nw = words + 4, nr = (size_t)n + 1, na = std::max<size_t>((size_t)n * max_aln, 1);
  if ((rc = B.d_words.reserve(c, nw))) return rc;
  if ((rc = B.d_rec_off.reserve(c, nr)) || (rc = B.d_len.reserve(c, nr)) || (rc = B.d_saved.reserve(c, nr)) || (rc = B.d_work.reserve(c, nr)) || (rc = B.d_rw.reserve(c, nr)) ||
      (rc = B.d_marks.reserve(c, nr))) return rc;
  if ((rc = B.d_saved_aln.reserve(c, na)) || (rc = B.d_work_aln.reserve(c, na))) return rc;
  B.n = n; B.max_len = max_len; B.slots = max_aln; B.used = true;
  for (int k = 0; k < 7; k++) B.min_ge[k] = ~0u;
  B.min_ge_known = false;
  if (n && min_len >= 100) { for (int k = 0; k < 7; k++) B.min_ge[k] = min_len; B.min_ge_known = true; }
  return SMR_OK;
}
int batch_fresh_state(smr_ctx* c, Batch& B, hipStream_t st) {
  HIPCHK(c, hipMemsetAsync(B.d_rw, 0, (size_t)B.n * sizeof(RWork), st));
  HIPCHK(c, hipMemsetAsync(B.d_work, 0, (size_t)B.n * sizeof(RState), st));
  B.cigar_words = 0; B.d_cigar.release();
  if (B.d_idcov.cap() < (size_t)B.n * 4) B.d_idcov.release();
  return reset_batch(c, B, st);
}
int upload_into(smr_ctx* c, Batch& B, const smr_reads* r, uint32_t max_aln, hipStream_t st) {
  if (r->view) { set_err(c, "the batch was made with SMR_FASTX_VIEW: its packed words are on the device only"); return SMR_ERR_STATE; }
  if (max_aln == 0) max_aln = 1;
  int rc;
  if ((rc = batch_reserve(c, B, r->words.size(), r->n, r->min_len, r->max_len, max_aln, st))) return rc;
  HIPCHK(c, hipMemcpyAsync(B.d_words, r->words.data(), r->words.size() * 4, hipMemcpyHostToDevice, st));
  HIPCHK(c, hipMemcpyAsync(B.d_rec_off, r->rec_off.data(), r->rec_off.size() * 8, hipMemcpyHostToDevice, st));
  if (r->n) HIPCHK(c, hipMemcpyAsync(B.d_len, r->len.data(), r->len.size() * 4, hipMemcpyHostToDevice, st));
  return batch_fresh_state(c, B, st);
}
}

extern "C" const char* smr_params_refused(const smr_params* p) {
  if (!p) return "null params";
  if (p->edges < 1 || p->edges > 10) return "edges must be 1..10 (nucleotides or percent), like the reference's --edges";
  return nullptr;
}

extern "C" int smr_state_reset(smr_ctx* c) {
  if (!c || !c->b->d_saved) return SMR_ERR_STATE;
  HIPCHK(c, hipSetDevice(c->device));
  return reset_batch(c, *c->b, c->stream);
}

extern "C" int smr_reads_upload(smr_ctx* c, const smr_reads* r, uint32_t max_aln) {
  if (!c || !r) return SMR_ERR_ARG;
  HIPCHK(c, hipSetDevice(c->device));
  return upload_into(c, *c->b, r, max_aln, c->stream);
}

extern "C" int smr_reads_upload_batch(smr_ctx* c, int batch, const smr_reads* r, uint32_t max_aln) {
  if (!c || !r || batch < 0 || batch >= SMR_MAX_BATCHES) return SMR_ERR_ARG;
  {
    std::lock_guard<std::mutex> l(c->sel_m);
    if (&c->bt[batch] == c->b) { std::lock_guard<std::mutex> l2(c->err_m); c->err = "smr_reads_upload_batch: the batch is the selected one (use smr_reads_upload)"; return SMR_ERR_STATE; }
  }
  HIPCHK(c, hipSetDevice(c->device));
  return upload_into(c, c->bt[batch], r, max_aln, c->upload_stream);
}

namespace {
int ensure_pool(smr_ctx* c) {
  uint64_t want_pool = std::max<uint64_t>((uint64_t)c->b->n * 64 + (1u << 20), 1u << 22);
  if (c->tune.pool_words) want_pool = c->tune.pool_words;
  if (c->pool_words < want_pool) { int rc = c->d_pool.alloc(c, want_pool); if (rc) return rc; c->pool_words = want_pool; }
  return SMR_OK;
}

int grow_pool(smr_ctx* c) {
  const uint64_t w = c->pool_words * 2;
  if (w > 0x7FFFFFF0ull) { set_err(c, "seed-hit pool exceeds 8 GiB"); return SMR_ERR_CAPACITY; }
  int rc = c->d_pool.alloc(c, w); if (rc) return rc;
  c->pool_words = w; c->n_pool_grown++;
  return SMR_OK;
}
}

__global__ void k_ctr_begin(unsigned long long* __restrict__ ctr, const unsigned long long* __restrict__ snap) {
  for (int k = threadIdx.x; k < C_TOTAL; k += blockDim.x) {
    const bool zero = k == C_NUM_SHORT || (k >= C_ERR_HITCAP && k <= C_ERR_TRACE) || k == C_ERR_SCAP || k == C_ERR_REDO || k == C_POOL_CURSOR || k == C_WORK_NEXT || k >= C_PCUR;
    ctr[k] = zero ? 0ull : snap[k];
  }
}

namespace {
int refuse_percent_edges(smr_ctx* c, const DevIndex& di, const smr_params* p) {
  if (!p->is_as_percent) return SMR_OK;
  Batch& B = *c->b;
  if (!B.min_ge_known) {
// ... 179 lines not shown
  if (!c || !c->b->d_saved) return SMR_ERR_STATE;
  HIPCHK(c, hipSetDevice(c->device));
  Batch& B = *c->b;
  int rc;
  const size_t need_r = std::max<size_t>(B.n, 1), need_a = std::max<size_t>((size_t)B.n * B.slots, 1);
  if ((rc = c->d_fidx.reserve(c, need_r)) || (rc = c->d_fstate.reserve(c, need_r)) || (rc = c->d_faln.reserve(c, need_a))) return rc;
  HIPCHK(c, hipMemsetAsync(&B.d_ctr[C_FETCH_N], 0, 8, c->stream));
  if (B.n) launch(c, k_results_compact, dim3((B.n + 1023) / 1024), dim3(1024), 0, B.n, B.slots, (const RState*)B.d_saved, (const AlignRec*)B.d_saved_aln,
                              c->d_fidx, c->d_fstate, c->d_faln, B.d_ctr);
  std::vector<unsigned long long> h;
  rc = read_ctr(c, h); if (rc) return rc;
  const uint64_t cw = std::min<uint64_t>(h[C_CIGAR_CURSOR], B.cigar_words);
  const size_t nhit = (size_t)std::min<unsigned long long>(h[C_FETCH_N], B.n);
  B.h_cigar.resize(cw);
  B.h_idx.resize(nhit); B.h_state.resize(nhit); B.h_aln.resize(nhit * B.slots);
  if (nhit) {
    HIPCHK(c, hipMemcpyAsync(B.h_idx.data(), c->d_fidx, nhit * 4, hipMemcpyDeviceToHost, c->stream));
    HIPCHK(c, hipMemcpyAsync(B.h_state.data(), c->d_fstate, nhit * sizeof(RState), hipMemcpyDeviceToHost, c->stream));
    HIPCHK(c, hipMemcpyAsync(B.h_aln.data(), c->d_faln, nhit * B.slots * sizeof(AlignRec), hipMemcpyDeviceToHost, c->stream));
  }
  if (cw) HIPCHK(c, hipMemcpyAsync(B.h_cigar.data(), B.d_cigar, cw * 4, hipMemcpyDeviceToHost, c->stream));
  B.h_idcov.clear();
  if (B.d_idcov && nhit) {
    if ((rc = c->d_fidcov.reserve(c, need_r * 4))) return rc;
    B.h_idcov.resize(nhit * 4);
    launch(c, k_idcov_gather, dim3((uint32_t)((nhit + 255) / 256)), dim3(256), 0, (const uint32_t*)c->d_fidx, (const unsigned long long*)&B.d_ctr[C_FETCH_N],
                       (const uint32_t*)B.d_idcov, c->d_fidcov);
    HIPCHK(c, hipMemcpyAsync(B.h_idcov.data(), c->d_fidcov, nhit * 16, hipMemcpyDeviceToHost, c->stream));
  }
  B.h_map.assign(B.n, 0xFFFFFFFFu);
  HIPCHK(c, hipStreamSynchronize(c->stream));
  for (size_t j = 0; j < nhit; j++) B.h_map[B.h_idx[j]] = (uint32_t)j;
  B.fetched = true;
  return SMR_OK;
}

static size_t record_of(const Batch& B, uint32_t i, uint8_t* buf, size_t cap);
extern "C" size_t smr_result_record(const smr_ctx* c, uint32_t i, uint8_t* buf, size_t cap) { return c ? record_of(*c->b, i, buf, cap) : 0; }
extern "C" size_t smr_result_record_batch(const smr_ctx* c, int batch, uint32_t i, uint8_t* buf, size_t cap) {
  return (c && batch >= 0 && batch < SMR_MAX_BATCHES) ? record_of(c->bt[batch], i, buf, cap) : 0;
}
static size_t record_of(const Batch& B, uint32_t i, uint8_t* buf, size_t cap) {
  const Batch* const b_ = &B;
  struct { const Batch* b; } cc{b_}; const auto* c = &cc;
  if (!c->b->fetched || i >= c->b->n) return 0;
  const uint32_t j = c->b->h_map[i];
  if (j == 0xFFFFFFFFu) return 0;
  const RState& s = c->b->h_state[j];
  if (s.n_align == 0) return 0;
  const AlignRec* al = c->b->h_aln.data() + (size_t)j * c->b->slots;
  size_t need = 24 + 3 + 2 + 4 + 4 + 8 + 4 + 4 + 8;
  for (uint32_t k = 0; k < s.n_align; k++) need += 8 + 8 + (size_t)(al[k].has_cigar ? al[k].cigar_len : 0) * 4 + 24 + 6 + 1;
  if (!buf || cap < need) return need;
  uint8_t* p = buf;
  auto put = [&](const void* v, size_t n) { memcpy(p, v, n); p += n; };
  uint8_t z8 = 0;
  const uint32_t z4[4] = {0, 0, 0, 0};
  const uint32_t* ic = c->b->h_idcov.size() >= 4 * ((size_t)j + 1) ? c->b->h_idcov.data() + 4 * (size_t)j : z4;
  put(&s.lastIndex, 4); put(&s.lastPart, 4); put(ic, 16);
  put(&s.is_done, 1); put(&s.is_hit, 1); put(&z8, 1);
  put(&s.max_SW_count, 2);
  int32_t na = (int32_t)c->b->last_num_alignments; put(&na, 4);
  put(&s.hit_seeds, 4);
  uint64_t asz = 16;
  for (uint32_t k = 0; k < s.n_align; k++) asz += 8 + 8 + (uint64_t)(al[k].has_cigar ? al[k].cigar_len : 0) * 4 + 24 + 6 + 1;
  put(&asz, 8); put(&s.min_index, 4); put(&s.max_index, 4);
  uint64_t nal = s.n_align; put(&nal, 8);
  for (uint32_t k = 0; k < s.n_align; k++) {
    const AlignRec& a = al[k];
    uint64_t cl = a.has_cigar ? a.cigar_len : 0;
    uint64_t rl = 8 + cl * 4 + 24 + 6 + 1; put(&rl, 8); put(&cl, 8);
    if (cl) put(c->b->h_cigar.data() + a.cigar_off, cl * 4);
    put(&a.ref_num, 4); put(&a.ref_begin1, 4); put(&a.ref_end1, 4); put(&a.read_begin1, 4); put(&a.read_end1, 4); put(&a.readlen, 4);
    put(&a.score1, 2); put(&a.part, 2); put(&a.index_num, 2); put(&a.strand, 1);
  }
  return (size_t)(p - buf);
}
extern "C" int smr_result_is_hit(const smr_ctx* c, uint32_t i) {
  if (!c || !c->b->fetched || i >= c->b->n || c->b->h_map[i] == 0xFFFFFFFFu) return 0;
  return c->b->h_state[c->b->h_map[i]].is_hit;
}

__global__ void k_force_pass(uint32_t n, DParams P, int pass, const uint32_t* __restrict__ len, RWork* __restrict__ rw) {
  uint32_t i = blockIdx.x * blockDim.x + threadIdx.x;
  if (i >= n) return;
  RWork w = rw[i];
  w.strand_active = len[i] >= P.lnwin ? 1 : 0; w.search = 1; w.pass_n = (uint8_t)pass; w.win_shift = P.skip[pass];
  for (int q = 0; q < 3; q++) w.blk_cnt[q] = 0;
  w.hit_total = 0; w.valid = w.strand_active;
  rw[i] = w;
}

extern "C" int smr_seed_scan(smr_ctx* c, int slot, const smr_params* p, int strand, int pass, uint64_t* n_hits_out) {
  if (!c || slot < 0 || slot >= 64 || pass < 0 || pass > 2) return SMR_ERR_ARG;
  if (!c->idx[slot].used || !c->b->d_saved) { set_err(c, "index slot empty or no reads uploaded"); return SMR_ERR_STATE; }
  HIPCHK(c, hipSetDevice(c->device));
  int rc = check_params(c, p); if (rc) return rc;
  const DevIndex& di = c->idx[slot];
  DParams P = make_dparams(c, di, p);
  c->last_seed_slot = slot;
  if ((rc = ensure_pool(c))) return rc;
  ev_drop(c);
  const uint32_t tb = 256, nb = (c->b->n + tb - 1) / tb;
  std::vector<unsigned long long> h;
  for (int attempt = 0; attempt < 16; attempt++) {
    HIPCHK(c, hipMemsetAsync(&c->b->d_ctr[C_ERR_HITCAP], 0, 16, c->stream));
    HIPCHK(c, hipMemsetAsync(&c->b->d_ctr[C_PCUR], 0, C_NSHARD * C_PCUR_STRIDE * 8, c->stream));
    HIPCHK(c, hipMemsetAsync(&c->b->d_ctr[C_HIT], 0, 8, c->stream));
    HIPCHK(c, hipMemsetAsync(&c->b->d_ctr[C_SHARDS], 0, C_SHARD_W * C_NSHARD * 8, c->stream));
    launch(c, k_begin_part, dim3(nb), dim3(tb), 0, dreads(c), P, c->b->d_saved, c->b->d_saved_aln, c->b->d_work, c->b->d_work_aln, c->b->d_rw, c->b->d_ctr);
    DParams Q = P; Q.is_forward = 1; Q.is_reverse = 1;
    launch(c, k_begin_strand, dim3(nb), dim3(tb), 0, c->b->n, Q, strand ? 1 : 0, c->b->d_work, c->b->d_rw);
    launch(c, k_force_pass, dim3(nb), dim3(tb), 0, c->b->n, P, pass, c->b->d_len, c->b->d_rw);
    if ((rc = launch_seed(c, di, P, pass))) return rc;
    if ((rc = read_ctr(c, h))) return rc;
    ev_collect(c);
    bool retry = false;
    if (h[C_ERR_HITCAP]) { if (!grow_hcap(c, P.partialwin)) return SMR_ERR_CAPACITY; retry = true; }
    if (h[C_ERR_POOL]) { if ((rc = grow_pool(c))) return rc; retry = true; }
    if (!retry) { if (n_hits_out) *n_hits_out = h[C_HIT]; return SMR_OK; }
  }
  set_err(c, "capacity retries exhausted");
  return SMR_ERR_CAPACITY;
}

extern "C" int smr_seed_tuples_fetch(smr_ctx* c, uint64_t* tuples, uint64_t cap_tuples, uint32_t* cbase, uint32_t cap_cbase, uint32_t meta[8]) {
  if (!c || !meta) return SMR_ERR_ARG;
  if (!c->sb.srt || !c->sb.sn) { set_err(c, "no seed stage has run"); return SMR_ERR_STATE; }
  HIPCHK(c, hipSetDevice(c->device));
  uint32_t sn[SN_COUNT];
  HIPCHK(c, hipMemcpy(sn, c->sb.sn, sizeof sn, hipMemcpyDeviceToHost));
  const uint32_t nt = (uint32_t)std::min<uint64_t>(sn[SN_TUPLES], 2 * c->sb_slots);
  meta[0] = nt; meta[1] = std::min(sn[SN_FWD], nt); meta[2] = c->sb.nc; meta[3] = c->sb.fb; meta[4] = c->sb.cb; meta[5] = c->sb.nkh; meta[6] = c->ccap; meta[7] = sn[SN_REDO];
  if (tuples) { if (cap_tuples < nt) return SMR_ERR_CAPACITY; if (nt) HIPCHK(c, hipMemcpy(tuples, c->sb.srt, (size_t)nt * sizeof(SeedTup), hipMemcpyDeviceToHost)); }
  if (cbase) { if (cap_cbase < c->sb.nc + 1u) return SMR_ERR_CAPACITY; HIPCHK(c, hipMemcpy(cbase, c->sb.cbase, (size_t)(c->sb.nc + 1u) * 4, hipMemcpyDeviceToHost)); }
  return SMR_OK;
}

extern "C" int smr_seed_pool_info(smr_ctx* c, uint64_t info[4]) {
  if (!c || !info) return SMR_ERR_ARG;
  HIPCHK(c, hipSetDevice(c->device));
  std::vector<unsigned long long> cur(C_NSHARD * C_PCUR_STRIDE, 0ull);
  if (c->b->d_ctr) {
    HIPCHK(c, hipMemcpyAsync(cur.data(), &c->b->d_ctr[C_PCUR], cur.size() * 8, hipMemcpyDeviceToHost, c->stream));
    HIPCHK(c, hipStreamSynchronize(c->stream));
  }
  const uint64_t region = std::min<uint64_t>(c->pool_words, 0x7FFFFFF0ull) / C_NSHARD;
  uint64_t hi = 0;
  for (int s = 0; s < C_NSHARD; s++) if (cur[s * C_PCUR_STRIDE]) hi = std::max<uint64_t>(hi, s * region + cur[s * C_PCUR_STRIDE]);
  info[0] = c->pool_words; info[1] = c->n_pool_grown; info[2] = hi; info[3] = c->pool_inline;
  return SMR_OK;
}

extern "C" int smr_cand_info_enable(smr_ctx* c, int on) {
  if (!c) return SMR_ERR_ARG;
  c->cinfo_on = on != 0;
  if (!c->cinfo_on) c->croute_n = 0;
  return SMR_OK;
}
extern "C" int smr_cand_info(smr_ctx* c, uint64_t info[13]) {
  if (!c || !info) return SMR_ERR_ARG;
  info[0] = c->cinfo_attempts;
  for (int q = 0; q < 5; q++) info[1 + q] = c->cinfo_retry[q];
  info[6] = c->chain_ext ? 1 : 0; info[7] = c->chain_scap; info[8] = c->keys_cap; info[9] = c->pairs_cap; info[10] = c->hits_cap;
  info[11] = c->cinfo_on ? 1 : 0; info[12] = c->croute_n;
  return SMR_OK;
}
extern "C" int smr_cand_routes(smr_ctx* c, uint8_t* out, uint32_t n) {
  if (!c || !out) return SMR_ERR_ARG;
  if (!c->cinfo_on || !c->d_croute || n != c->croute_n) { set_err(c, "smr_cand_routes: no route bytes for that many reads (smr_cand_info_enable before smr_align_part)"); return SMR_ERR_STATE; }
  HIPCHK(c, hipSetDevice(c->device));
  if (n) { HIPCHK(c, hipMemcpyAsync(out, c->d_croute, (size_t)n, hipMemcpyDeviceToHost, c->stream)); HIPCHK(c, hipStreamSynchronize(c->stream)); }
  return SMR_OK;
}

extern "C" int smr_seed_hits_fetch(smr_ctx* c, uint32_t* triples, uint64_t cap_triples, uint64_t* n_out) {
  if (!c || !n_out) return SMR_ERR_ARG;
  HIPCHK(c, hipSetDevice(c->device));
  std::vector<unsigned long long> h;
  int rc = read_ctr(c, h); if (rc) return rc;
  uint64_t words = h[C_POOL_CURSOR] ? std::min<uint64_t>(c->pool_words, 0x7FFFFFF0ull) : 0;
  std::vector<uint32_t> pool(words);
  std::vector<RWork> rw(c->b->n);
  if (words) HIPCHK(c, hipMemcpy(pool.data(), c->d_pool, words * 4, hipMemcpyDeviceToHost));
  if (c->b->n) HIPCHK(c, hipMemcpy(rw.data(), c->b->d_rw, (size_t)c->b->n * sizeof(RWork), hipMemcpyDeviceToHost));
  std::vector<uint32_t> po;
  if (c->last_seed_slot >= 0 && c->idx[c->last_seed_slot].used) {
    const DevIndex& di = c->idx[c->last_seed_slot];
    po.resize((size_t)di.n_ids + 1);
    HIPCHK(c, hipMemcpy(po.data(), di.pos_off, po.size() * 4, hipMemcpyDeviceToHost));
  }
  auto orig = [&](uint32_t idp) -> uint32_t {
    if (po.size() < 2) return idp;
    size_t lo = 0, hi = po.size() - 1;
    while (hi - lo > 1) { const size_t mid = (lo + hi) / 2; if ((uint64_t)po[mid] + mid <= idp) lo = mid; else hi = mid; }
    return (uint32_t)lo;
  };
  uint64_t o = 0;
  for (uint32_t r = 0; r < c->b->n; r++) {
    for (int pp = 0; pp < 3; pp++) {
      const uint32_t cnt = rw[r].blk_cnt[pp], bo = rw[r].blk_off[pp];
      for (uint32_t q = 0; q < cnt && (uint64_t)bo + 2 * q + 1 < words; q++) {
        if (triples && o < cap_triples) { triples[3 * o] = r; triples[3 * o + 1] = orig(pool[bo + 2 * q]); triples[3 * o + 2] = pool[bo + 2 * q + 1]; }
        o++;
      }
    }
  }
  *n_out = o;
  return SMR_OK;
}

extern "C" int smr_prof_reset(smr_ctx* c) {
  if (!c) return SMR_ERR_ARG;
  HIPCHK(c, hipSetDevice(c->device));
  for (int k = 0; k < KP_COUNT; k++) { c->kp_ms[k] = 0; c->kp_l[k] = 0; }
  c->n_seed_shared = c->n_seed_shared_builds = 0;
  if (c->d_wpstat) HIPCHK(c, hipMemsetAsync(c->d_wpstat, 0, WPS_N * 8, c->stream));
  for (int k = 0; k < SMR_MAX_BATCHES; k++)
    if (c->bt[k].d_ctr) {
      HIPCHK(c, hipMemsetAsync(&c->bt[k].d_ctr[C_WINDOWS], 0, 9 * 8, c->stream));
      HIPCHK(c, hipMemsetAsync(&c->bt[k].d_ctr[C_SW_SPEC], 0, 3 * 8, c->stream));
      HIPCHK(c, hipMemsetAsync(&c->bt[k].d_ctr[C_TUP_F], 0, C_SHARD_NX * 8, c->stream));
      HIPCHK(c, hipMemsetAsync(&c->bt[k].d_ctr[C_SHARDS], 0, C_SHARD_W * C_NSHARD * 8, c->stream));
    }
  HIPCHK(c, hipStreamSynchronize(c->stream));
  return SMR_OK;
}
extern "C" int smr_prof_get(smr_ctx* c, smr_prof* o) {
  if (!c || !o) return SMR_ERR_ARG;
  HIPCHK(c, hipSetDevice(c->device));
  std::vector<unsigned long long> h(C_TOTAL, 0), t(C_TOTAL);
  for (int k = 0; k < SMR_MAX_BATCHES; k++) {
    if (!c->bt[k].d_ctr) continue;
    HIPCHK(c, hipMemcpyAsync(t.data(), c->bt[k].d_ctr, C_TOTAL * 8, hipMemcpyDeviceToHost, c->stream));
    HIPCHK(c, hipStreamSynchronize(c->stream));
    if (c->tune.debug_phases) {
      unsigned long long ph[7] = {0, 0, 0, 0, 0, 0, 0};
      for (int s2 = 0; s2 < C_NSHARD; s2++) for (int q = 0; q < 7; q++) ph[q] += t[C_SHARDS + C_SHARD_W * s2 + C_SHARD_PH + q];
      fprintf(stderr, "[smr] phase cycles (batch %d): %llu %llu %llu %llu %llu %llu %llu  (-DSMR_CHAIN_PHASES: claim, gather+prefix, walk1, walk2+cands, pairs+sort, "
              "window/lis/book, sw; -DSMR_SEED_PHASES (k_seed_pg): setup, directory ranges, entries, -, candidate selection, output, -)\n", k, ph[0], ph[1], ph[2], ph[3], ph[4], ph[5], ph[6]);
    }
    fold_shards(t);
    for (int q = 0; q < C_COUNT; q++) h[q] += t[q];
  }
  o->seed_ms = c->kp_ms[KP_KEYS] + c->kp_ms[KP_SPLIT] + c->kp_ms[KP_BINS] + c->kp_ms[KP_PG0] + c->kp_ms[KP_PG1] + c->kp_ms[KP_FINISH]; o->seed_launches = c->kp_l[KP_KEYS];
  o->chain_ms = c->kp_ms[KP_CAND] + c->kp_ms[KP_CHAIN] + c->kp_ms[KP_BEGINS] + c->kp_ms[KP_WALK] + c->kp_ms[KP_SW16] + c->kp_ms[KP_WNEXT]; o->chain_launches = c->kp_l[KP_CAND] + c->kp_l[KP_BEGINS];
  o->trace_ms = c->kp_ms[KP_TRACE]; o->trace_launches = c->kp_l[KP_TRACE];
  o->n_windows = h[C_WINDOWS]; o->n_lookup = h[C_LOOKUP]; o->n_node = h[C_NODE]; o->n_entry = h[C_ENTRY]; o->n_hit = h[C_HIT]; o->n_read_bytes = h[C_READ_BYTES];
  o->n_sw_fwd = h[C_SW_FWD]; o->n_sw_rev = h[C_SW_REV]; o->n_sw_cells = h[C_SW_CELLS];
  o->n_sw_spec = h[C_SW_SPEC]; o->n_sw_spec_used = h[C_SW_SPEC_USED]; o->n_seed_redo = h[C_SEED_REDO]; o->hit_list_cap = c->hcap;
  o->n_seed_shared = c->n_seed_shared; o->n_seed_shared_builds = c->n_seed_shared_builds;
  return SMR_OK;
}

extern "C" int smr_prof_kernels(smr_ctx* c, smr_kprof* out, uint32_t cap, uint32_t* n_out) {
  if (!c || !out || !n_out) return SMR_ERR_ARG;
  HIPCHK(c, hipSetDevice(c->device));
  std::vector<unsigned long long> h(C_TOTAL, 0), t(C_TOTAL);
  for (int k = 0; k < SMR_MAX_BATCHES; k++) {
    if (!c->bt[k].d_ctr) continue;
    HIPCHK(c, hipMemcpyAsync(t.data(), c->bt[k].d_ctr, C_TOTAL * 8, hipMemcpyDeviceToHost, c->stream));
    HIPCHK(c, hipStreamSynchronize(c->stream));
    fold_shards(t);
    for (int q = 0; q < C_COUNT; q++) h[q] += t[q];
  }
  const unsigned long long T = h[C_TUP_ALL];
  unsigned long long bytes[KP_COUNT] = {};
  bytes[KP_KEYS] = h[C_B_KEYS] + sizeof(SeedTup) * T;
  bytes[KP_SPLIT] = bytes[KP_BINS] = 2 * sizeof(SeedTup) * T;
  bytes[KP_PG0] = h[C_B_PG0]; bytes[KP_PG1] = h[C_B_PG1]; bytes[KP_FINISH] = h[C_B_FIN];
  uint32_t n = 0;
  for (int k = 0; k < KP_COUNT && n < cap; k++, n++) {
    memset(&out[n], 0, sizeof out[n]);
    snprintf(out[n].name, sizeof out[n].name, "%s", KP_NAME[k]);
    out[n].ms = c->kp_ms[k]; out[n].launches = c->kp_l[k]; out[n].bytes = bytes[k];
  }
  *n_out = n;
  return SMR_OK;
}
```

### sortmerna_amd/csrc/smr_engine_chain.hpp

```cpp

uint32_t chain_edges(const DParams& P, uint32_t len) { return P.is_as_percent ? (uint32_t)((P.edges / 100.0) * len) + 1 : (uint32_t)std::max(P.edges, 0); }
void chain_lds(const smr_ctx* c, const DParams& P, uint32_t& ml, uint32_t& rf, uint32_t& rq, size_t& bytes) {
  const uint32_t mq_len = std::min<uint32_t>(c->b->max_len, SW_X4_MAX_ROWS);
  ml = (c->b->max_len + 15) & ~15u;
  rf = (c->b->max_len + 2 * chain_edges(P, c->b->max_len) + 16 + 15) & ~15u;
  rq = std::min(rf, (mq_len + 2 * chain_edges(P, mq_len) + 16 + 15) & ~15u);
  bytes = 5 * (size_t)std::min<uint32_t>(ml, SW_X4_MAX_ROWS) + (size_t)9 * rq + (size_t)CH_KEYS_LDS * 8 + (size_t)std::max<uint32_t>(4u * CH_PAIRS_LDS, 2u * c->chain_scap) * 4 +
          (size_t)CH_HITS_LDS * 8 + (size_t)(CH_HITS_LDS + 8) * 4 + (size_t)c->chain_scap * 4;
}
void chain_lds(const smr_ctx* c, const DParams& P, uint32_t& ml, uint32_t& rf, size_t& bytes) { uint32_t rq; chain_lds(c, P, ml, rf, rq, bytes); }
int ensure_bound(smr_ctx* c, uint32_t blocks, uint32_t rf) {
  if (c->b->max_len <= SW_X4_MAX_ROWS) return SMR_OK;
  int rc = c->d_bound.reserve(c, (size_t)blocks * 2 * rf);
  return rc ? rc : c->d_rdq.reserve(c, (size_t)blocks * ((c->b->max_len + 15) & ~15u));
}

struct AlignPlan { uint32_t ml, rf, rq; size_t lds; bool lng, striped, split, x4, begins_sw16; int rows; };
int sw16_rows(uint32_t max_len) {
  const uint32_t wmq = std::min<uint32_t>(max_len, WK_MAX_ROWS);
  return wmq <= 104 ? 13 : wmq <= 152 ? 19 : wmq <= 208 ? 26 : 32;
}
AlignPlan align_plan(const smr_ctx* c, const DParams& P) {
  AlignPlan a;
  chain_lds(c, P, a.ml, a.rf, a.rq, a.lds);
// ... 46 lines not shown
    need[c->wstat_pass[e]] = std::max(need[c->wstat_pass[e]], want);
  }
  for (int p = 0; p < 3; p++) if (need[p]) {
    const uint32_t prev = c->walk_need[p] ? c->walk_need[p] : c->tune.walk_rounds;
    c->walk_need[p] = std::min(c->tune.walk_rounds, need[p] >= prev ? need[p] : prev - std::max(1u, (prev - need[p]) / 2u));
  }
  c->wstat_n = 0;
  return SMR_OK;
}

#define WALK_PREFIX_RETRY 64u
#define WALK_PREFIX_MIN_SEEN 64ull
int adapt_walk_prefix(smr_ctx* c) {
  if (!c->tune.walk_prefix || !c->d_wpstat) return SMR_OK;
  if (!c->pfx_live) { if (++c->pfx_parts_off >= WALK_PREFIX_RETRY) { c->pfx_live = true; c->pfx_parts_off = 0; } return SMR_OK; }
  unsigned long long h[WPS_N];
  HIPCHK(c, hipMemcpyAsync(h, c->d_wpstat, sizeof h, hipMemcpyDeviceToHost, c->stream));
  HIPCHK(c, hipStreamSynchronize(c->stream));
  if (h[WPS_DECIDED] < c->pfx_seen[0] || h[WPS_REDONE] < c->pfx_seen[1]) c->pfx_seen[0] = c->pfx_seen[1] = 0;
  const unsigned long long dec = h[WPS_DECIDED] - c->pfx_seen[0], redo = h[WPS_REDONE] - c->pfx_seen[1];
  c->pfx_seen[0] = h[WPS_DECIDED]; c->pfx_seen[1] = h[WPS_REDONE];
  if (dec + redo >= WALK_PREFIX_MIN_SEEN && dec < 2 * redo) {
    c->pfx_live = false; c->pfx_parts_off = 0;
    say(c->tune, "prefix tasks off for %u parts: %llu intervals decided, %llu undecided in the last part\n", WALK_PREFIX_RETRY, dec, redo);
  }
  return SMR_OK;
}

int launch_chain(smr_ctx* c, const DevIndex& di, const DParams& P, const AlignPlan& plan, int pass, int is_last_strand) {
  Batch& B = *c->b;
  const uint32_t ml = plan.ml, rf = plan.rf, rq = plan.rq;
  const size_t lds = plan.lds;
  const bool split = plan.split;
  int rc;
  HIPCHK(c, hipMemsetAsync(&B.d_ctr[C_WORK_NEXT], 0, 8, c->stream));
  if ((rc = raise_lds_limit(c, c->chain_lds_attr, lds, 64 * 1024, chain_kernel(0, 0, 0), chain_kernel(1, 0, 0), chain_kernel(0, 1, 0), chain_kernel(1, 1, 0),
                            chain_kernel(0, 0, 1), chain_kernel(1, 0, 1), chain_kernel(0, 1, 1), chain_kernel(1, 1, 1)))) return rc;
  const uint32_t blocks = std::min<uint32_t>(c->chain_blocks, std::max(B.n, 1u));
  if ((rc = ensure_bound(c, c->chain_blocks, rf))) return rc;
  int* const gb = plan.lng ? c->d_bound.get() : nullptr;
  uint8_t* const grd = plan.lng ? c->d_rdq.get() : nullptr;
  if (c->tune.handover) {
    if ((rc = c->d_mrec.reserve(c, B.n)) || (rc = c->d_mpool.reserve(c, (size_t)((B.n + CAND_BLOCK - 1u) / CAND_BLOCK) * CAND_BLOCK * CAND_REC_WORDS))) return rc;
  }
  const uint2* const mrec = c->tune.handover ? c->d_mrec.get() : nullptr;
  const uint32_t wml = (std::min<uint32_t>(B.max_len, WK_MAX_ROWS) + 15) & ~15u;
  const uint32_t RMX = c->tune.walk_rounds, WK = c->tune.walk_k;
  const uint32_t RM = (!c->tune.walk_rounds_fixed && c->walk_need[pass]) ? std::min(RMX, c->walk_need[pass]) : RMX;
  if (split) {
    const size_t n = B.n;
    if (c->walk_cap < n || c->walk_kcap < WK) {
      for (int q = 0; q < 2; q++)
        if ((rc = c->d_wlist[q].alloc(c, n)) || (rc = c->d_wstate[q].alloc(c, n)) || (rc = c->d_wtask[q].alloc(c, n * WK)) || (rc = c->d_wres[q].alloc(c, n * WK))) return rc;
      if ((rc = c->d_wtidx.alloc(c, 3 * n * WK)) || (rc = c->d_wslow.alloc(c, n))) return rc;
      c->walk_cap = n; c->walk_kcap = WK;
    }
    if ((rc = c->d_wctr.reserve(c, (size_t)(RMX + 2) * WC_STRIDE)) || (rc = c->d_wstat.reserve(c, (size_t)8 * 32))) return rc;
    HIPCHK(c, hipMemsetAsync(c->d_wctr, 0, (size_t)(RMX + 2) * WC_STRIDE * 8, c->stream));
    if (!c->d_wpstat) { if ((rc = c->d_wpstat.alloc(c, WPS_N))) return rc; HIPCHK(c, hipMemsetAsync(c->d_wpstat, 0, WPS_N * 8, c->stream)); }
    if ((rc = raise_lds_limit(c, c->walk_lds_attr, (size_t)wml + rq, 64 * 1024, k_walk<true>))) return rc;
  }
  const size_t n_tix = (size_t)c->walk_cap * c->walk_kcap;
  unsigned long long* const n_slow = split ? c->d_wctr + (size_t)(RMX + 1) * WC_STRIDE : nullptr;
  const dim3 per_read((B.n + 255u) / 256u);
  ev_mark(c, KP_CAND);
  launch(c, k_cand, dim3((B.n + CAND_BLOCK - 1u) / CAND_BLOCK), dim3(256), CAND_LDS_BYTES(c->cand_bloom, c->tune.handover), dreads(c), dindex(di), P, pass, is_last_strand, B.d_work, B.d_rw, c->d_pool, B.d_marks, c->cand_bloom,
         c->tune.handover ? c->d_mrec.get() : nullptr, c->d_mpool, c->d_mpool.cap());
  if (split) {
    ev_mark(c, KP_WNEXT);
    launch(c, k_wlist, dim3((B.n + 1023u) / 1024u), dim3(1024), 0, dreads(c), B.d_marks, mrec, (uint32_t)WK_MAX_ROWS, c->d_wlist[0], c->d_wslow, c->d_wctr, n_slow, c->tune.walk_debug ? n_slow + 8 : nullptr, (P.num_seeds >= 2 && c->tune.walk_gather) ? 1 : 0);
    if (c->cinfo_on) launch(c, k_cand_route, per_read, dim3(256), 0, B.n, B.d_marks, mrec, c->d_wlist[0], c->d_wctr, 0, c->d_croute);
    const uint32_t walk_blocks = (uint32_t)c->n_cu * 4u * SMR_WALK_WAVES_PER_SIMD;
    for (uint32_t rnd = 0; rnd < RM; rnd++) {
      const int cur = (int)(rnd & 1u), prv = cur ^ 1;
      unsigned long long* const wc = c->d_wctr + (size_t)rnd * WC_STRIDE;
      const bool fin = rnd + 1 == RM;
      ev_mark(c, KP_WALK);
      launch(c, fin ? k_walk<true> : k_walk<false>, dim3(fin ? walk_blocks * 3u / SMR_WALK_WAVES_PER_SIMD : walk_blocks), dim3(64), fin ? (size_t)wml + rq : 0,
             dreads(c), dindex(di), P, pass, is_last_strand, B.d_work, B.d_work_aln, B.d_rw, B.d_ctr, mrec, c->d_mpool, c->d_pool, c->d_wlist[cur],
             c->d_wstate[prv], c->d_wtask[prv], c->d_wres[prv], c->d_wstate[cur], c->d_wtask[cur], c->d_wtidx, c->d_wtidx + n_tix, c->d_wtidx + 2 * n_tix, wc, WK, n_tix, (int)rnd, wml, rq, c->tune.walk_assume,
             c->pfx_live ? c->tune.walk_prefix : 0u, c->d_wpstat);
      if (fin) continue;
      ev_mark(c, KP_SW16);
      launch_sw16(c, plan.rows, 0, 0, dreads(c), dindex(di), P, c->d_wtask[cur], c->d_wtidx, c->d_wtidx + n_tix, c->d_wtidx + 2 * n_tix, wc, c->d_wres[cur]);
      ev_mark(c, KP_WNEXT);
      launch(c, k_wnext, dim3((uint32_t)c->n_cu * 2u), dim3(1024), 0, P, is_last_strand, B.d_work, B.d_rw, B.d_ctr, c->d_wlist[cur], c->d_wstate[cur],
             c->d_wres[cur], c->d_wlist[prv], wc, wc + WC_STRIDE, WK, n_tix, (int)rnd);
    }
    if (!c->tune.walk_rounds_fixed && c->wstat_n < 8) {
      launch(c, k_wstat, dim3(1), dim3(32), 0, c->d_wctr, c->d_wstat + (size_t)c->wstat_n * 32, RM);
      c->wstat_pass[c->wstat_n] = pass; c->wstat_rm[c->wstat_n] = RM; c->wstat_n++;
    }
    if (c->tune.walk_debug) {
      std::vector<unsigned long long> h((size_t)(RMX + 2) * WC_STRIDE);
      HIPCHK(c, hipMemcpyAsync(h.data(), c->d_wctr, h.size() * 8, hipMemcpyDeviceToHost, c->stream));
      HIPCHK(c, hipStreamSynchronize(c->stream));
      { const unsigned long long* q = &h[(size_t)(RMX + 1) * WC_STRIDE];
        fprintf(stderr, "libsmr_hip: walk rounds (pass %d): slow %llu (positions <= 64 / 128 / 256 / 512 / more / > 64 hits: %llu %llu %llu %llu %llu %llu);", pass, q[0], q[8], q[9], q[10], q[11], q[12], q[13]); }
      for (uint32_t rnd = 0; rnd < RM; rnd++) fprintf(stderr, " %llu/%llu+%llu+%llu", h[(size_t)rnd * WC_STRIDE + WC_NLIST], h[(size_t)rnd * WC_STRIDE + WC_NTASK], h[(size_t)rnd * WC_STRIDE + WC_NTASK2], h[(size_t)rnd * WC_STRIDE + WC_NTASK3]);
      fprintf(stderr, "\n");
      unsigned long long ps[WPS_N];
      HIPCHK(c, hipMemcpyAsync(ps, c->d_wpstat, sizeof ps, hipMemcpyDeviceToHost, c->stream));
      HIPCHK(c, hipStreamSynchronize(c->stream));
      fprintf(stderr, "libsmr_hip: prefix tasks so far (SMR_WALK_PREFIX=%u): scored %llu decided %llu redone %llu; look-ahead tasks of reads expected to align under best N %llu, their cells %llu\n",
              c->tune.walk_prefix, ps[WPS_SCORED], ps[WPS_DECIDED], ps[WPS_REDONE], ps[WPS_AHEAD], ps[WPS_AHEAD_CELLS]);
    }
  }
  ev_mark(c, KP_CHAIN);
  for (int ext = 0; ext <= (c->chain_ext ? 1 : 0); ext++) {
    if (ext) HIPCHK(c, hipMemsetAsync(&B.d_ctr[C_WORK_NEXT], 0, 8, c->stream));
    if (c->cinfo_on) launch(c, k_cand_route, per_read, dim3(256), 0, B.n, B.d_marks, nullptr, nullptr, nullptr, 1 + ext, c->d_croute);
    launch(c, chain_kernel(ext, plan.lng, plan.striped), dim3(blocks), dim3(64), lds, dreads(c), dindex(di), P, pass, is_last_strand, B.d_work, B.d_work_aln, B.d_rw, c->d_pool, B.d_ctr,
           c->d_tuples, c->d_keys, c->d_pairs, c->d_lis, c->d_hits, c->keys_cap, c->pairs_cap, c->hits_cap, ml, rf, c->chain_scap, c->chain_ext ? c->d_stab.get() : nullptr,
           c->chain_ext ? c->d_tuples2.get() : nullptr, rq, gb, grd, B.d_marks, mrec, c->d_mpool, split ? c->d_wslow.get() : nullptr, n_slow);
  }
  ev_stop(c);
  HIPCHK(c, hipGetLastError());
  return SMR_OK;
}

int launch_begins(smr_ctx* c, const DevIndex& di, const DParams& P, const AlignPlan& plan) {
  Batch& B = *c->b;
  int rc;
  const uint64_t ntot = (uint64_t)B.n * B.slots;
  if ((rc = c->d_tasks.reserve(c, 2 * ntot))) return rc;
  const int x4 = plan.x4 ? 1 : 0;
  const size_t lds_b = x4 ? (size_t)4 * (plan.ml + plan.rf) : (plan.lng ? 0 : (size_t)plan.ml + plan.rf);
  const uint32_t bg_blocks = (uint32_t)c->n_cu * 8u;
  if ((rc = ensure_bound(c, std::max(bg_blocks, c->chain_blocks), plan.rf))) return rc;
  if ((rc = raise_lds_limit(c, c->begins_lds_attr, lds_b, 64 * 1024, begins_kernel(0, 0), begins_kernel(1, 0), begins_kernel(0, 1), begins_kernel(1, 1)))) return rc;
  HIPCHK(c, hipMemsetAsync(&B.d_ctr[C_BEGIN_N], 0, 16, c->stream));
  ev_mark(c, KP_BEGINS);
  launch(c, k_begins_collect, dim3((uint32_t)((ntot + 1023) / 1024)), dim3(1024), 0, B.n, B.slots, B.d_work, B.d_rw, B.d_work_aln, c->d_tasks, B.d_ctr);
  const size_t task_cap = (size_t)c->walk_cap * c->walk_kcap;
  if (plan.begins_sw16 && c->d_wtask[0] && c->d_wctr && ntot <= task_cap) {
    for (int stage = 0; stage < 2; stage++) {
      HIPCHK(c, hipMemsetAsync(c->d_wctr, 0, (size_t)WC_STRIDE * 8, c->stream));
      launch(c, k_begins_prep, dim3((uint32_t)c->n_cu * 2u), dim3(1024), 0, dindex(di), B.slots, c->d_tasks, &B.d_ctr[C_BEGIN_N], B.d_work_aln, stage, c->d_wtask[0], c->d_wtidx, c->d_wctr);
      launch_sw16(c, plan.rows, 4, 0, dreads(c), dindex(di), P, c->d_wtask[0], c->d_wtidx, c->d_wtidx + task_cap, c->d_wtidx + 2 * task_cap, c->d_wctr, c->d_wres[0]);
      launch(c, k_begins_apply, dim3((uint32_t)c->n_cu * 4u), dim3(256), 0, c->d_tasks, &B.d_ctr[C_BEGIN_N], B.d_work_aln, stage, c->d_wtask[0], c->d_wres[0], B.d_ctr);
    }
  } else
    launch(c, begins_kernel(plan.lng, plan.striped), dim3(bg_blocks), dim3(64), lds_b, dreads(c), dindex(di), P, c->d_tasks, B.d_work_aln, B.d_ctr, plan.ml, plan.rf, x4,
           plan.lng ? c->d_bound.get() : nullptr, plan.lng ? c->d_rdq.get() : nullptr);
  ev_stop(c);
  return SMR_OK;
}

void fold_shards(std::vector<unsigned long long>& h) {
  for (int s = 0; s < C_NSHARD; s++)
    for (int k = 0; k < C_SHARD_W; k++) {
      if (k < C_SHARD_X) h[C_WINDOWS + k] += h[C_SHARDS + C_SHARD_W * s + k];
      else if (k < C_SHARD_X + C_SHARD_NX) h[C_TUP_F + k - C_SHARD_X] += h[C_SHARDS + C_SHARD_W * s + k];
      h[C_SHARDS + C_SHARD_W * s + k] = 0;
    }
  unsigned long long mx = 0;
  for (int s = 0; s < C_NSHARD; s++) mx = std::max(mx, h[C_PCUR + s * C_PCUR_STRIDE]);
  h[C_POOL_CURSOR] = mx;
}

int read_ctr(smr_ctx* c, std::vector<unsigned long long>& h) {
  h.resize(C_TOTAL);
  HIPCHK(c, hipMemcpyAsync(h.data(), c->b->d_ctr, C_TOTAL * 8, hipMemcpyDeviceToHost, c->stream));
  HIPCHK(c, hipStreamSynchronize(c->stream));
  fold_shards(h);
  return SMR_OK;
}
```

### sortmerna_amd/csrc/smr_kernels.hpp

```cpp
#pragma once
#include <hip/hip_runtime.h>
#include <stdint.h>

#include "smr_host.hpp"

#include <smr_device_ops.hpp>
#include <smr_h16_ops.hpp>

namespace smr {

struct DIndex {
  const Lookup* lookup;
  const uint32_t* lkc;
  const uint32_t* trie;
  const uint32_t* pg;
  const uint2* root3;
  const uint32_t* pos_off;
  const uint2* pos_arr;
  const uint8_t* ref_seq;
  const uint64_t* ref_off;
  uint32_t n_refs, n_ids, lnwin, partialwin;
  uint32_t ref_any_n;
};

struct DReads {
  const uint32_t* words;
  const uint64_t* rec_off;
  const uint32_t* len;
  uint32_t n, max_len;
};

struct RState {
  uint32_t lastIndex, lastPart, hit_seeds, min_index, max_index, n_align;
  uint16_t max_SW_count;
  uint8_t is_done, is_hit;
};

struct RWork {
  int32_t best;
  uint32_t blk_off[3];
  uint32_t blk_cnt[3];
  uint32_t hit_total;
  uint32_t win_shift;
  uint8_t is_new_hit;
  uint8_t is04;
  uint8_t aval;
  uint8_t reversed;
  uint8_t valid;
  uint8_t strand_active;
  uint8_t search;
  uint8_t pass_n;
  uint8_t has_amb;
  uint8_t pad_[3];
};

struct AlignRec {
  uint32_t ref_num;
  int32_t ref_begin1, ref_end1, read_begin1, read_end1;
  uint32_t readlen;
  uint16_t score1, part, index_num;
  uint8_t strand, has_cigar;
  uint32_t cigar_off, cigar_len;
};

struct DParams {
  uint32_t lnwin, partialwin;
  uint32_t skip[3];
  int32_t num_seeds, min_lis, edges, is_as_percent;
  int32_t match, mismatch, score_N, gap_open, gap_ext;
  uint32_t minimal_score, num_alignments;
  int32_t is_best, is_full_search, is_forward, is_reverse;
  uint32_t minoccur, index_num, part;
  int32_t is_last_index_part;
  uint32_t slots;
  int32_t sw_mode;
  uint16_t* sw_scratch;
  uint32_t sw_scratch_stride;
};
__device__ __forceinline__ uint16_t* sw_scr(const DParams& P) { return P.sw_scratch ? P.sw_scratch + (size_t)blockIdx.x * P.sw_scratch_stride : nullptr; }

enum {
  C_NUM_ALIGNED = 0, C_NUM_SHORT = 1, C_PER_DB = 2,
  C_WINDOWS = 66, C_LOOKUP, C_NODE, C_ENTRY, C_HIT, C_READ_BYTES, C_SW_FWD, C_SW_REV, C_SW_CELLS,
  C_ERR_HITCAP, C_ERR_POOL, C_ERR_SLOTS, C_ERR_PAIRS, C_ERR_CIGAR, C_ERR_TRACE, C_POOL_CURSOR, C_WORK_NEXT,
  C_CIGAR_CURSOR, C_TRACE_NEXT, C_ERR_SCAP, C_ERR_REDO, C_TRACE_DEFER, C_BEGIN_N, C_BEGIN_NEXT, C_FETCH_N, C_SW_SPEC, C_SW_SPEC_USED, C_SEED_REDO,
  C_TUP_F, C_TUP_ALL, C_B_KEYS, C_B_PG0, C_B_PG1, C_B_FIN,
  C_IDCOV, C_IDCOV_FEW = C_IDCOV + 4, C_IDCOV_MANY, C_IDCOV_NOCIG, C_COUNT = 112,
  C_NSHARD = 64, C_SHARD_W = 32, C_SHARD_X = 9, C_SHARD_NX = 6, C_SHARD_PH = 16, C_SHARDS = C_COUNT, C_PCUR = C_SHARDS + C_SHARD_W * C_NSHARD, C_PCUR_STRIDE = 16 , C_TOTAL = C_PCUR + C_NSHARD * C_PCUR_STRIDE
};
static_assert(C_IDCOV_NOCIG < C_COUNT, "counter block");
__device__ __forceinline__ void ctr_add(unsigned long long* ctr, int idx, unsigned long long v) {
  atomicAdd(&ctr[C_SHARDS + (blockIdx.x & (C_NSHARD - 1)) * C_SHARD_W + (idx >= C_TUP_F ? C_SHARD_X + idx - C_TUP_F : idx - C_WINDOWS)], v);
}

__device__ __constant__ uint8_t c_lev[(16 + 8 + 4 + 2) * 14] = {
    3,14,14,14,14,14,14,14,14,14,14,14,14,14, 3,14,14,14,14,14,14,14,14,14,14,14,14,14,
    7,14,14,14,4,4,4,4,14,14,14,14,14,14, 7,14,14,14,4,4,4,4,14,14,14,14,14,14,
    0,14,2,2,14,14,2,2,14,14,14,14,14,14, 0,14,2,2,14,14,2,2,14,14,14,14,14,14,
    0,14,2,2,4,4,6,6,14,14,14,14,14,14, 0,14,2,2,4,4,6,6,14,14,14,14,14,14,
    3,1,14,1,14,1,14,1,14,14,14,14,14,14, 3,1,14,1,14,1,14,1,14,14,14,14,14,14,
    7,1,14,1,4,5,4,5,14,14,14,14,14,14, 7,1,14,1,4,5,4,5,14,14,14,14,14,14,
    0,1,2,3,14,1,2,3,14,14,14,14,14,14, 0,1,2,3,14,1,2,3,14,14,14,14,14,14,
    0,1,2,3,4,5,6,7,14,14,14,14,14,14, 0,1,2,3,4,5,6,7,14,14,14,14,14,14,
    3,14,14,14,14,14,14,14,14,14,14,14,14,14, 13,14,14,14,10,10,10,10,14,14,14,14,14,14,
    8,14,2,2,14,14,2,2,14,14,14,14,14,14, 8,14,2,2,10,10,12,12,14,14,14,14,14,14,
    3,1,14,1,14,1,14,1,14,14,14,14,14,14, 13,1,14,1,10,11,10,11,14,14,14,14,14,14,
    8,1,2,3,14,1,2,3,14,14,14,14,14,14, 8,1,2,3,10,11,12,13,14,14,14,14,14,14,
    12,14,14,14,14,14,14,14,12,14,14,14,14,14, 9,14,10,10,14,14,10,10,9,14,14,14,10,10,
    12,1,14,1,14,1,14,1,12,14,14,1,14,1, 9,1,10,12,14,1,10,12,9,14,14,1,10,12,
    10,14,14,14,14,14,14,14,14,10,14,14,14,14, 10,10,14,10,14,10,14,10,14,10,14,14,10,14};
#define LEV_T1 (16 * 14)
#define LEV_T2 (LEV_T1 + 8 * 14)
#define LEV_T3 (LEV_T2 + 4 * 14)
#define LEV_SIZE ((16 + 8 + 4 + 2) * 14)

__device__ __forceinline__ int lane_id() { return (int)(threadIdx.x & 63); }

__device__ __forceinline__ uint32_t block_append(unsigned long long* counter, bool take) {
  __shared__ uint32_t s_wcnt[16], s_wbase[16];
  const uint32_t lane = threadIdx.x & 63u, wv = threadIdx.x >> 6, nwv = (blockDim.x + 63u) >> 6;
  const unsigned long long m = __ballot(take);
  if (lane == 0) s_wcnt[wv] = (uint32_t)__popcll(m);
  __syncthreads();
  if (threadIdx.x == 0) {
    uint32_t tot = 0;
    for (uint32_t q = 0; q < nwv; q++) { s_wbase[q] = tot; tot += s_wcnt[q]; }
    const uint32_t base = tot ? (uint32_t)atomicAdd(counter, (unsigned long long)tot) : 0u;
    for (uint32_t q = 0; q < nwv; q++) s_wbase[q] += base;
  }
  __syncthreads();
  return s_wbase[wv] + (uint32_t)__popcll(m & ((1ull << lane) - 1ull));
}

__device__ __forceinline__ uint32_t read_nt(const uint32_t* rec, uint32_t len, uint32_t k, uint32_t reversed, uint32_t aval) {
  uint32_t j = reversed ? (len - 1 - k) : k;
  uint32_t cw = (len + 15) >> 4;
  uint32_t code = (rec[j >> 4] >> ((j & 15) * 2)) & 3u;
  uint32_t amb = (rec[cw + (j >> 5)] >> (j & 31)) & 1u;
  if (reversed) code = 3u - code;
  return amb ? aval : code;
}

__global__ void k_begin_part(DReads rd, DParams P, const RState* __restrict__ saved, const AlignRec* __restrict__ saved_aln,
                             RState* __restrict__ work, AlignRec* __restrict__ work_aln, RWork* __restrict__ rw,
                             unsigned long long* __restrict__ ctr) {
  uint32_t i = blockIdx.x * blockDim.x + threadIdx.x;
  uint32_t is_short = 0;
  if (i < rd.n) {
    RState s = saved[i];
    work[i] = s;
    for (uint32_t k = 0; k < s.n_align; k++) work_aln[(size_t)i * P.slots + k] = saved_aln[(size_t)i * P.slots + k];
    RWork w;
    w.best = P.min_lis > 0 ? P.min_lis : 0;
    for (int q = 0; q < 3; q++) { w.blk_off[q] = 0; w.blk_cnt[q] = 0; }
    w.hit_total = 0; w.win_shift = P.skip[0];
    w.is_new_hit = 0; w.is04 = 0; w.aval = 0; w.reversed = 0;
    is_short = rd.len[i] < P.lnwin;
    w.valid = (!is_short && !s.is_done) ? 1 : 0;
    w.strand_active = 0; w.search = 0; w.pass_n = 0;
    {
      const uint32_t ln = rd.len[i]; const uint32_t* rec = rd.words + rd.rec_off[i];
      uint32_t cw = (ln + 15) >> 4, mw = (ln + 31) >> 5, any = 0;
      for (uint32_t q = 0; q < mw; q++) any |= rec[cw + q];
      w.has_amb = any ? 1 : 0; w.pad_[0] = w.pad_[1] = w.pad_[2] = 0;
    }
    rw[i] = w;
  }
  unsigned long long m = __ballot(is_short);
  if (lane_id() == 0 && m) atomicAdd(&ctr[C_NUM_SHORT], (unsigned long long)__popcll(m));
}

__global__ void k_begin_strand(uint32_t n, DParams P, int count, const RState* __restrict__ work, RWork* __restrict__ rw) {
  uint32_t i = blockIdx.x * blockDim.x + threadIdx.x;
  if (i >= n) return;
  RWork w = rw[i];
  w.strand_active = 0;
  if (w.valid && !work[i].is_done) {
    int single = (P.is_forward != 0) ^ (P.is_reverse != 0);
    if ((single && P.is_reverse) || count == 1) {
      if (!w.reversed) {
        w.reversed = 1;
        w.aval = (w.aval == 0) ? 3 : (w.aval == 3 ? 0 : 4);
      }
    }
    w.strand_active = 1; w.search = 1; w.pass_n = 0; w.win_shift = P.skip[0];
    for (int q = 0; q < 3; q++) w.blk_cnt[q] = 0;
    w.hit_total = 0;
  }
  rw[i] = w;
}

__global__ void k_commit_part(uint32_t n, DParams P, RState* __restrict__ saved, AlignRec* __restrict__ saved_aln,
                              const RState* __restrict__ work, const AlignRec* __restrict__ work_aln, const RWork* __restrict__ rw) {
  uint32_t i = blockIdx.x * blockDim.x + threadIdx.x;
  if (i >= n) return;
  if (rw[i].valid && rw[i].is_new_hit) {
    RState s = work[i];
    saved[i] = s;
    for (uint32_t k = 0; k < s.n_align; k++) saved_aln[(size_t)i * P.slots + k] = work_aln[(size_t)i * P.slots + k];
  }
}

}

#include "smr_seed.hpp"
#include "smr_seed_pg.hpp"
#include "smr_chain.hpp"
#include "smr_walk.hpp"
#include "smr_trace.hpp"
```

### sortmerna_amd/csrc/smr_seed_pg.hpp

```cpp
#pragma once

namespace smr {

#define PG_CAND_CAP0 256u
#define PG_CAND_CAP_MAX 2048u
#define PG_NIL 0xFFFFu
#ifndef PG_OCC
#define PG_OCC 7
#endif
#define PG_WAVES 1
#ifndef PG_TRIP
#define PG_TRIP 4
#endif
#define PG_LDS_WORDS(ccap) (4u * (ccap) + 128u)

__device__ __forceinline__ uint32_t pg_scan_add(uint32_t x) { return wave_scan_add(x); }
__device__ __forceinline__ uint32_t pg_scan_max(uint32_t x) {
  x = max(x, (uint32_t)__builtin_amdgcn_update_dpp(0, (int)x, 0x111, 0xF, 0xF, false));
  x = max(x, (uint32_t)__builtin_amdgcn_update_dpp(0, (int)x, 0x112, 0xF, 0xF, false));
  x = max(x, (uint32_t)__builtin_amdgcn_update_dpp(0, (int)x, 0x114, 0xF, 0xF, false));
  x = max(x, (uint32_t)__builtin_amdgcn_update_dpp(0, (int)x, 0x118, 0xF, 0xF, false));
  x = max(x, (uint32_t)__builtin_amdgcn_update_dpp(0, (int)x, 0x142, 0xA, 0xF, false));
  x = max(x, (uint32_t)__builtin_amdgcn_update_dpp(0, (int)x, 0x143, 0xC, 0xF, false));
  return x;
}

__device__ __forceinline__ uint32_t pg_reversed(uint32_t s) {
  const uint32_t rv = __brev(s);
  return ((rv & 0xAAAAAAAAu) >> 1) | ((rv & 0x55555555u) << 1);
}
__device__ __forceinline__ uint32_t pg_rkey(uint32_t rev, uint32_t from, uint32_t cnt) { return (rev >> (32u - 2u * (from + cnt))) & ((1u << (2u * cnt)) - 1u); }

struct __attribute__((aligned(4))) PgPair { uint32_t lo, hi; };

struct PgRow { uint32_t T, P, m, u, w; int s; SMR_GLOBAL_U32* tt; bool have; };
struct PgOwn { uint32_t exm, P9, mab, blo, bhi, t1, t2, t3, d0, d1, d2, d3; };
__device__ __forceinline__ const uint32_t* pg_strings_at(const uint32_t* pg, uint32_t rtx, uint32_t rty) {
  const uint32_t cA = (rty >> 24) & 15u, cB = rty >> 28;
  return pg + (size_t)rtx * 4 + (cA ? (1u << (2 * cA)) + (1u << (2 * cB)) + 2u : 0u);
}
__device__ __forceinline__ SMR_GLOBAL_U32* pg_ptr(uint32_t lo, uint32_t hi) { return (SMR_GLOBAL_U32*)((unsigned long long)hi << 32 | lo); }

__device__ __forceinline__ void pg_row_fetch(PgRow& R, uint32_t g0, uint32_t wtot, int lane, uint32_t* own, const PgOwn& O, uint32_t& carry, const uint32_t* pg) {
  uint32_t u = 0;
  SMR_GLOBAL_U32* tt = (SMR_GLOBAL_U32*)pg;
  bool have = false;
  if (g0 < wtot) {
    const uint32_t g = g0 + (uint32_t)lane;
    own[lane] = 0;
    __builtin_amdgcn_wave_barrier();
    if (O.exm - g0 < 64u) own[O.exm - g0] = (uint32_t)lane + 1u;
    __builtin_amdgcn_wave_barrier();
    const uint32_t ow = max(pg_scan_max(own[lane]), carry);
    carry = (uint32_t)__builtin_amdgcn_readlane((int)ow, 63);
    const int s = (int)ow - 1;
    const uint32_t oP = __shfl(O.P9, s, 64), om = __shfl(O.mab, s, 64), olo = __shfl(O.blo, s, 64), ohi = __shfl(O.bhi, s, 64);
    const uint32_t t1 = __shfl(O.t1, s, 64), t2 = __shfl(O.t2, s, 64), t3 = __shfl(O.t3, s, 64);
    const uint32_t d0 = __shfl(O.d0, s, 64), d1 = __shfl(O.d1, s, 64), d2 = __shfl(O.d2, s, 64), d3 = __shfl(O.d3, s, 64);
    have = g < wtot;
    const bool p1 = g >= t1, p2 = g >= t2, p3 = g >= t3;
    u = have ? g + (p3 ? d3 : p2 ? d2 : p1 ? d1 : d0) : 0u;
    tt = have ? pg_ptr(olo, ohi) : (SMR_GLOBAL_U32*)pg;
    R.P = oP; R.m = om; R.w = p3 ? 3u : p2 ? 2u : p1 ? 1u : 0u; R.s = s;
  }
  R.u = u; R.tt = tt; R.have = have;
  R.T = tt[u];
}
__device__ __forceinline__ void pg_row_apply(const PgRow& R, uint32_t pw, uint32_t h, bool full, uint32_t ccap, uint32_t* s_ncand,
                                             uint32_t* cdk, uint32_t* cdv, uint32_t* cdn, uint32_t* hd) {
  if (!R.have) return;
  const uint32_t T = R.T, oP = R.P, u = R.u, w = R.w;
  const uint32_t mA = R.m & 0xFFFFu, mB = R.m >> 16;
  const uint32_t tb = (T >> (2 * h)) & mB;
  const bool dup = (w != 0 && ((T ^ oP) & mA) == 0) || (w == 3 && (tb == ((oP >> (2 * h)) & mB) || tb == ((oP >> (2 * h - 2)) & mB)));
  const uint32_t r = dup ? 0u : lev1_entry(oP, T, pw);
  if (r & 1u) {
    const uint32_t p = atomicAdd(s_ncand, 1u);
    if (p < ccap) {
      cdk[p] = u | ((uint32_t)R.s << 25);
      cdn[p] = atomicExch(&hd[R.s], p) | ((((r & 2u) && !full) ? CK_COND : CK_PLAIN) << 16);
    }
  }
}

__device__ __forceinline__ void pg_resolve(uint32_t nrec, int lane, uint32_t blo, uint32_t bhi, uint32_t rty, uint32_t* cdk, uint32_t* cdv, uint32_t* cnt) {
  for (uint32_t p0 = 0; p0 < nrec; p0 += 64) {
    const uint32_t p = p0 + (uint32_t)lane;
    const uint32_t rec = p < nrec ? cdk[p] : 0u;
    const int s = (int)(rec >> 25) & 63;
    const uint32_t olo = __shfl(blo, s, 64), ohi = __shfl(bhi, s, 64), om = __shfl(rty, s, 64);
    if (p < nrec) {
      const uint32_t u = rec & 0x1FFFFFFu, on = om & 0xFFFFFFu, ocA = (om >> 24) & 15u;
      SMR_GLOBAL_U32* ri = pg_ptr(olo, ohi) + (ocA ? 2 : 1) * (size_t)on + 2 * (size_t)u;
      cdk[p] = ri[0]; cdv[p] = ri[1];
      atomicAdd(&cnt[s], 1u);
    }
  }
}

template <int DIR>
__global__ void __launch_bounds__(64 * PG_WAVES, PG_OCC / PG_WAVES) k_seed_pg(DIndex ix, DParams P, int pass, SeedBufs sb, uint32_t ccap,
                                                uint32_t* __restrict__ pool, uint32_t pool_words, unsigned long long* __restrict__ ctr, int swz) {
  const uint32_t n_tup = min(sb.sn[SN_TUPLES], sb.cap_tuples), n_fwd = min(sb.sn[SN_FWD], n_tup);
  const uint32_t c0 = DIR ? n_fwd >> 6 : 0u, nw = (DIR ? (n_tup + 63u) >> 6 : (n_fwd + 63u) >> 6) - c0, per = (nw + 7u) >> 3;
  SMR_DYN_LDS(uint32_t, lds_dyn);
  uint32_t* cdk = lds_dyn + (threadIdx.x >> 6) * PG_LDS_WORDS(ccap);
  uint32_t* cdv = cdk + ccap;
  uint32_t* cdn = cdv + ccap;
  uint32_t* hp = cdn + ccap;
  uint32_t* hd = hp + ccap;
  uint32_t* own = hd + 64;
  __shared__ uint32_t s_ncand_[PG_WAVES];
  uint32_t& s_ncand = s_ncand_[threadIdx.x >> 6];
  const int lane = lane_id();
  const uint32_t pw = P.partialwin, h = pw / 2;
  const bool full = P.is_full_search != 0;
#ifdef SMR_SEED_PHASES
  unsigned long long tph[7] = {0, 0, 0, 0, 0, 0, 0}, tlast = clock64();
#define GPH(i) { const unsigned long long tn_ = clock64(); tph[i] += tn_ - tlast; tlast = tn_; }
#else
#define GPH(i)
#endif

  auto chunk_of = [&](uint32_t it, uint32_t& vb) -> int {
    if (swz) { if ((it >> 3) >= per) return 0; vb = (it & 7u) * per + (it >> 3); if (vb >= nw) return 2; }
    else { vb = it; if (vb >= nw) return 0; }
    vb += c0;
    return 1;
  };
  bool pf = false, pf_bounds = false;
  uint32_t pf_vb = 0, pf_c = 0, pf_nx = 0;
  SeedTup pf_t = 0;
  const uint32_t stride = gridDim.x * (blockDim.x >> 6);
  __shared__ unsigned long long s_acc[PG_WAVES][3];
  unsigned long long* acc = s_acc[threadIdx.x >> 6];
  if (lane == 0) { acc[0] = 0; acc[1] = 0; acc[2] = 0; }
  for (uint32_t it = uni(blockIdx.x * (blockDim.x >> 6) + (threadIdx.x >> 6)); ; it += stride) {
  uint32_t vb = 0;
  { const int ck = chunk_of(it, vb); if (ck == 0) break; if (ck == 2) continue; }
  __syncthreads();
  const uint32_t pos = vb * 64u + lane;
  bool mine = DIR ? (pos >= n_fwd && pos < n_tup) : pos < n_fwd;
  uint32_t nh = 0, P9 = 0, slot = 0, gfl = 0;
  uint2 rt = make_uint2(NONE, 0);
  uint32_t n_rep = 0;
  {
    const bool hit = pf && pf_vb == vb;
    const SeedTup t = hit ? pf_t : (pos < n_tup ? sb.srt[pos] : 0ull);
    const bool rep = mine && ((t & SEED_TUP_DUP) || !seed_read_active(sb, (uint32_t)t));
    n_rep = (uint32_t)__popcll(__ballot(rep));
    if (rep) mine = false;
    if (!__any(mine)) {
      pf = false; pf_bounds = false;
      if (lane == 0) acc[2] += 8ull * n_rep + 2u;
      continue;
    }
    uint32_t c = hit ? pf_c : (uint32_t)sb.wbin[vb];
    uint32_t nx = (hit && pf_bounds) ? pf_nx : sb.cbase[c + 1];
    pf = false; pf_bounds = false;
    if (mine) {
      while (pos >= nx) { c++; nx = sb.cbase[c + 1]; }
      SeedKey tk;
      tk.slot = (uint32_t)t; tk.chars = (uint32_t)(t >> 32) & ((1u << sb.cb) - 1u); tk.key = (c << sb.fb) | (uint32_t)(t >> (32u + sb.cb));
      rt = ix.root3[2 * (tk.key - (DIR ? sb.nkh : 0u)) + DIR];
      P9 = tk.chars; slot = tk.slot;
      if (DIR == 1) gfl = sb.gflag[slot >> 11];
    }
  }
  const bool counted = mine;
  if (mine) {
    if (DIR == 1 && ((gfl >> ((slot >> 6) & 31u)) & 1u) && ((sb.zbits[slot >> 5] >> (slot & 31u)) & 1u)) mine = false;
  }
  if (lane == 0) s_ncand = 0;
  __syncthreads();
  GPH(0)

  uint32_t rs0 = 0, rs1 = 0, rs2 = 0, rs3 = 0, rn0 = 0, rn1 = 0, rn2 = 0, rn3 = 0;
  uint32_t kA = 0, kb0 = 0, kb1 = 0, cA = 0, cB = 0, n = 0;
  if (mine && rt.x != NONE) {
    n = rt.y & 0xFFFFFFu; cA = (rt.y >> 24) & 15u; cB = rt.y >> 28;
    const uint32_t* blk = ix.pg + (size_t)rt.x * 4;
    if (cA == 0) { rn0 = n; }
    else {
      const uint32_t nA = (1u << (2 * cA)) + 1u, nB = (1u << (2 * cB)) + 1u;
      const uint32_t* dirA = blk; const uint32_t* dirB = blk + nA;
      const uint32_t rev = pg_reversed(P9);
      kA = pg_rkey(rev, 0, cA); kb0 = pg_rkey(rev, h, cB); kb1 = pg_rkey(rev, h - 1, cB);
      uint32_t lo2, hi2;
      if (cB == pw - h) { const uint32_t k2 = pg_rkey(rev, h + 1, cB - 1); lo2 = 4 * k2; hi2 = lo2 + 4; }
      else { lo2 = pg_rkey(rev, h + 1, cB); hi2 = lo2 + 1; }
      const PgPair pa = *reinterpret_cast<const PgPair*>(dirA + kA), pb = *reinterpret_cast<const PgPair*>(dirB + kb0), pc = *reinterpret_cast<const PgPair*>(dirB + kb1);
      const uint32_t d0 = dirB[lo2], d1 = dirB[hi2];
      rs0 = pa.lo; rn0 = pa.hi - pa.lo;
      rs1 = pb.lo; rn1 = pb.hi - pb.lo;
      if (kb1 != kb0) { rs2 = pc.lo; rn2 = pc.hi - pc.lo; }
      rs3 = d0; rn3 = d1 - d0;
      (void)nB;
    }
  }
  const uint32_t tot = rn0 + rn1 + rn2 + rn3;
  const bool srch = mine && rt.x != NONE;
  const unsigned long long w_node = 4ull * (uint32_t)__popcll(__ballot(srch && cA)) + (uint32_t)__popcll(__ballot(srch && !cA));
  GPH(1)
  const uint32_t sinc = pg_scan_add(tot);
  const uint32_t excl = sinc - tot, wtot = (uint32_t)__builtin_amdgcn_readlane((int)sinc, 63);
  const unsigned long long w_entry = wtot;
  const uint32_t c1 = rn0, c2 = c1 + rn1, c3 = c2 + rn2;
  const uint32_t u1 = n + rs1, u2 = n + rs2, u3 = n + rs3;
  hd[lane] = PG_NIL;
  uint32_t carry = 0;
  PgOwn O; O.exm = tot ? excl : 0x80000000u; O.P9 = P9;
  {
    const uint32_t* at = pg_strings_at(ix.pg, rt.x == NONE ? 0u : rt.x, rt.y);
    O.blo = (uint32_t)(unsigned long long)at; O.bhi = (uint32_t)((unsigned long long)at >> 32);
    O.mab = ((1u << (2 * cA)) - 1u) | (((1u << (2 * cB)) - 1u) << 16);
  }
  O.t1 = excl + c1; O.t2 = excl + c2; O.t3 = excl + c3;
  O.d0 = rs0 - excl; O.d1 = u1 - O.t1; O.d2 = u2 - O.t2; O.d3 = u3 - O.t3;
  PgRow A, B;
  A.T = A.P = A.m = A.u = A.w = 0; A.s = 0; A.tt = (SMR_GLOBAL_U32*)ix.pg; A.have = false;
  B = A;
  for (uint32_t g0 = 0; g0 < wtot + 64u; g0 += 128) {
    pg_row_fetch(B, g0, wtot, lane, own, O, carry, ix.pg);
    GPH(2)
    pg_row_apply(A, pw, h, full, ccap, &s_ncand, cdk, cdv, cdn, hd);
    GPH(3)
    pg_row_fetch(A, g0 + 64u, wtot, lane, own, O, carry, ix.pg);
    GPH(2)
    pg_row_apply(B, pw, h, full, ccap, &s_ncand, cdk, cdv, cdn, hd);
    GPH(3)
  }
  __syncthreads();
  GPH(2)
  {
    uint32_t nvb = 0;
    if (chunk_of(it + stride, nvb) == 1) {
      const uint32_t npos = nvb * 64u + lane;
      pf_t = npos < n_tup ? sb.srt[npos] : 0ull;
      pf_c = sb.wbin[nvb];
      pf_vb = nvb; pf = true;
    }
  }
  if (s_ncand > ccap) {
    if (lane == 0) {
      atomicAdd(&ctr[C_SEED_REDO], 1ull);
      const uint32_t p = atomicAdd(&sb.sn[SN_REDO], 1u);
      if (p < sb.cap_redo) sb.redo[p] = vb; else atomicAdd(&ctr[C_ERR_REDO], 1ull);
    }
    continue;
  }
  own[lane] = 0;
  __builtin_amdgcn_wave_barrier();
  pg_resolve(s_ncand, lane, O.blo, O.bhi, rt.y, cdk, cdv, own);
  __syncthreads();
  const uint32_t hb = pg_scan_add(own[lane]) - own[lane];
  GPH(6)
  bool zero = false;
  {
    const uint32_t head = hd[lane];
    uint32_t last = 0;
    bool more = head != PG_NIL;
    while (__any(more)) {
      uint32_t best = 0xFFFFFFFFu, bi = 0;
      if (more) for (uint32_t q = head; q != PG_NIL; q = cdn[q] & 0xFFFFu) {
        const uint32_t k = cdk[q];
        if (k >= last && k < best) { best = k; bi = q; }
      }
      if (!more || best == 0xFFFFFFFFu) { more = false; continue; }
      const uint32_t idc = cdv[bi], kc = cdn[bi] >> 16;
      bool present = false;
      for (uint32_t f = 0; f < nh; f++) if ((hp[hb + f] & ~SEED_CAND_COND) == idc) { present = true; break; }
      if (DIR == 0 && kc == CK_COND && !present) { hp[hb] = idc; nh = 1; zero = true; more = false; }
      else if (!present) { hp[hb + nh] = idc | ((DIR && kc == CK_COND) ? SEED_CAND_COND : 0u); nh++; }
      last = best + 1;
    }
  }
  GPH(4)
  if (pf) { pf_nx = sb.cbase[pf_c + 1]; pf_bounds = true; }
  const bool wr = mine && nh > 0;
  const bool inl = wr && nh == 1 && sb.seg_inline;
  const uint32_t need = (wr && !inl) ? 1 + nh : 0;
  const uint32_t incl = pg_scan_add(need);
  const uint32_t total = (uint32_t)__builtin_amdgcn_readlane((int)incl, 63);
  uint32_t base = 0;
  if (total) {
    if (lane == 0) {
      const uint32_t shard = vb & (C_NSHARD - 1), region = pool_words / C_NSHARD;
      const unsigned long long old = atomicAdd(&ctr[C_PCUR + shard * C_PCUR_STRIDE], (unsigned long long)total);
      if (old + total > region) { atomicAdd(&ctr[C_ERR_POOL], 1ull); base = NONE; } else base = shard * region + (uint32_t)old;
    }
    base = __shfl(base, 0, 64);
  }
  if (inl) wseg_put(sb, DIR, slot, SEED_SEG_INLINE | (hp[hb] & (SEED_SEG_ID | (DIR ? SEED_CAND_COND : 0u))) | (zero ? SEED_ZERO_BIT : 0u), zero);
  else if (wr && base != NONE) {
    const uint32_t o = base + incl - need;
    pool[o] = nh;
    for (uint32_t q = 0; q < nh; q++) pool[o + 1 + q] = hp[hb + q];
    wseg_put(sb, DIR, slot, o | (zero ? SEED_ZERO_BIT : 0u), zero);
  }
  unsigned long long w_bytes = (uint32_t)__popcll(__ballot(counted)) * ((uint32_t)sizeof(SeedTup) + 8u + (DIR ? 1u : 0u))
                             + 32u * (uint32_t)__popcll(__ballot(srch && cA)) + 4u * (uint32_t)__popcll(__ballot(wr));
  w_bytes += 4ull * wtot + 4ull * total + 8ull * min(s_ncand, ccap) + 2u + 8ull * n_rep;
  if (lane == 0) { acc[0] += w_node; acc[1] += w_entry; acc[2] += w_bytes; }
#ifdef SMR_SEED_PHASES
  GPH(5)
  if (lane == 0) for (int q = 0; q < 7; q++) if (tph[q]) { atomicAdd(&ctr[C_SHARDS + (vb & (C_NSHARD - 1)) * C_SHARD_W + C_SHARD_PH + q], tph[q]); tph[q] = 0; }
#endif
  }
  if (lane == 0) { if (acc[0]) ctr_add(ctr, C_NODE, acc[0]); if (acc[1]) ctr_add(ctr, C_ENTRY, acc[1]); if (acc[2]) ctr_add(ctr, DIR ? C_B_PG1 : C_B_PG0, acc[2]); }
}

}
```

### sortmerna_amd/csrc/smr_tuning.hpp

```cpp
#pragma once
#include <algorithm>
#include <cstdarg>
#include <cstdint>
#include <cstdio>
#include <cstdlib>
#include <string>

namespace smr {

struct TuningLimits { uint32_t walk_k_max, cand_cap0, cand_cap_max, bloom_words_max, pool_words_min, hot_bin, hot_sub, selfcheck_cases; };

struct Tuning {
  int sw_packed = 2;
  bool seed_exact = false;
  int seed_shared = 1;
  uint32_t hot_min = 1024;
  uint32_t hot_bin = 0;
  uint32_t hot_sub = 0;
  bool seg_inline = true;
  int handover = 1;
  int walk_split = 1;
  uint32_t walk_rounds = 8;
  bool walk_rounds_fixed = false;
  uint32_t walk_k = 4;
  int walk_gather = 1;
  uint32_t walk_assume = 3;
  uint32_t walk_prefix = 44;
  int sw16_f16 = 1;
  bool begins_x4 = false;
  bool pg_host = false;
  bool trace_global_rows = false;
  uint32_t cand_bloom = 128;
  uint32_t ccap = 0;
  uint64_t pool_words = 0;
  uint64_t cigar_words = 0;
  uint32_t sw_selfcheck = 0;
  bool verbose = false;
  bool seed_debug = false;
  bool walk_debug = false;
  bool debug_phases = false;
};

#define SMR_TUNING_TABLE(X)                                                                                                              \
  X(SMR_SW_PACKED, sw_packed) X(SMR_SEED_EXACT, seed_exact) X(SMR_SEED_SHARED, seed_shared) X(SMR_SEED_DEDUP, hot_min)                   \
  X(SMR_SEED_HOT_BIN, hot_bin) X(SMR_SEED_HOT_SUB, hot_sub) X(SMR_SEG_INLINE, seg_inline) X(SMR_HANDOVER, handover)                     \
  X(SMR_WALK_SPLIT, walk_split) X(SMR_WALK_ROUNDS, walk_rounds) X(SMR_WALK_K, walk_k) X(SMR_WALK_GATHER, walk_gather)                   \
  X(SMR_WALK_ASSUME, walk_assume) X(SMR_BEGINS_X4, begins_x4) X(SMR_PG_HOST, pg_host) X(SMR_TRACE_GLOBAL_ROWS, trace_global_rows)       \
  X(SMR_CAND_BLOOM, cand_bloom) X(SMR_PG_CAND_CAP, ccap) X(SMR_SEED_POOL_WORDS, pool_words) X(SMR_CIGAR_POOL_WORDS, cigar_words)        \
  X(SMR_SW_SELFCHECK, sw_selfcheck) X(SMR_VERBOSE, verbose) X(SMR_SEED_DEBUG, seed_debug) X(SMR_WALK_DEBUG, walk_debug)                 \
  X(SMR_DEBUG_PHASES, debug_phases)

inline Tuning read_tuning(const TuningLimits& L) {
  Tuning t;
  t.hot_bin = L.hot_bin; t.hot_sub = L.hot_sub; t.ccap = L.cand_cap0; t.sw_selfcheck = L.selfcheck_cases;
  const char* e;
  if ((e = getenv("SMR_SW_PACKED"))) t.sw_packed = atoi(e);
  if ((e = getenv("SMR_SEED_EXACT"))) t.seed_exact = atoi(e) != 0;
  if ((e = getenv("SMR_SEED_SHARED"))) t.seed_shared = atoi(e);
  if ((e = getenv("SMR_SEED_DEDUP"))) t.hot_min = (uint32_t)std::max(0, atoi(e));
  if ((e = getenv("SMR_SEED_HOT_BIN"))) t.hot_bin = (uint32_t)std::max(1, atoi(e));
  if ((e = getenv("SMR_SEED_HOT_SUB"))) t.hot_sub = (uint32_t)std::max(1, atoi(e));
  if ((e = getenv("SMR_SEG_INLINE"))) t.seg_inline = atoi(e) != 0;
  if ((e = getenv("SMR_HANDOVER"))) t.handover = atoi(e);
  if ((e = getenv("SMR_WALK_SPLIT"))) t.walk_split = atoi(e);
  if ((e = getenv("SMR_WALK_ROUNDS"))) { t.walk_rounds = (uint32_t)std::max(1, std::min(32, atoi(e))); t.walk_rounds_fixed = true; }
  if ((e = getenv("SMR_WALK_K"))) t.walk_k = (uint32_t)std::max(1, std::min((int)L.walk_k_max, atoi(e)));
  if ((e = getenv("SMR_WALK_GATHER"))) t.walk_gather = atoi(e);
  if ((e = getenv("SMR_WALK_ASSUME"))) t.walk_assume = (uint32_t)atoi(e);
  if ((e = getenv("SMR_WALK_PREFIX"))) t.walk_prefix = (uint32_t)std::max(0, std::min(100, atoi(e)));
  if ((e = getenv("SMR_SW16_F16"))) t.sw16_f16 = atoi(e) != 0 ? 1 : 0;
  t.begins_x4 = getenv("SMR_BEGINS_X4") != nullptr;
  if ((e = getenv("SMR_PG_HOST"))) t.pg_host = atoi(e) != 0;
  t.trace_global_rows = getenv("SMR_TRACE_GLOBAL_ROWS") != nullptr;
  if ((e = getenv("SMR_CAND_BLOOM"))) { uint32_t b = 64; while (b < L.bloom_words_max && b < (uint32_t)atoi(e)) b <<= 1; t.cand_bloom = b; }
  if ((e = getenv("SMR_PG_CAND_CAP"))) t.ccap = std::min<uint32_t>(L.cand_cap_max, std::max<uint32_t>(4u, (uint32_t)atoi(e)));
  if ((e = getenv("SMR_SEED_POOL_WORDS"))) t.pool_words = std::min<uint64_t>(std::max<uint64_t>(strtoull(e, nullptr, 0), L.pool_words_min), 0x7FFFFFF0ull);
  if ((e = getenv("SMR_CIGAR_POOL_WORDS"))) t.cigar_words = std::max<uint64_t>(strtoull(e, nullptr, 10), 16);
  if ((e = getenv("SMR_SW_SELFCHECK"))) t.sw_selfcheck = (uint32_t)atoi(e);
  t.verbose = getenv("SMR_VERBOSE") != nullptr;
  t.seed_debug = getenv("SMR_SEED_DEBUG") != nullptr;
  t.walk_debug = getenv("SMR_WALK_DEBUG") != nullptr;
  t.debug_phases = getenv("SMR_DEBUG_PHASES") != nullptr;
  return t;
}

inline std::string tuning_text(const Tuning& t) {
  std::string s;
#define SMR_TUNING_LINE(name, member) s += #name "=" + std::to_string(+t.member) + "\n";
  SMR_TUNING_TABLE(SMR_TUNING_LINE)
#undef SMR_TUNING_LINE
  return s;
}

__attribute__((format(printf, 2, 3))) inline void say(const Tuning& t, const char* fmt, ...) {
  if (!t.verbose) return;
  va_list a;
  va_start(a, fmt);
  fputs("libsmr_hip: ", stderr);
  vfprintf(stderr, fmt, a);
  va_end(a);
}

inline uint32_t tuning_host_threads(uint32_t cap) { const char* e = getenv("SMR_HOST_THREADS"); return e ? std::min<uint32_t>(cap, (uint32_t)std::max(1, atoi(e))) : cap; }
inline uint32_t tuning_load_threads(uint32_t dflt) { const char* e = getenv("SMR_LOAD_THREADS"); return e ? std::min<uint32_t>(256, std::max(1, atoi(e))) : dflt; }
inline bool tuning_ib_timing() { return getenv("SMR_IB_TIMING") != nullptr; }

}
```

### sortmerna_amd/engine.py

```python
import ctypes as C

import numpy as np

from . import capi


OTU_GROUP = np.dtype([("ref_num", np.uint32), ("n_reads", np.uint32), ("off", np.uint64)])


class SmrError(RuntimeError):
    pass


def default_params(**kw):
    p = capi.Params()
    capi.load().smr_params_default(C.byref(p))
    for k, v in kw.items():
        if k == "skiplengths":
            for i in range(3):
                p.skiplengths[i] = v[i]
        else:
            if not hasattr(p, k):
                raise AttributeError(k)
            setattr(p, k, v)
# ... 619 lines not shown
        args = (self.h, n, a.ctypes.data, a_off.ctypes.data_as(u64p), b.ctypes.data, b_off.ctypes.data_as(u64p))
        self._chk(self.L.smr_interleave_batch(*args, None, 0, C.byref(need)), "smr_interleave_batch")
        buf = np.zeros(max(need.value, 1), dtype=np.uint8)
        if need.value:
            self._chk(self.L.smr_interleave_batch(*args, buf.ctypes.data, need.value, C.byref(need)), "smr_interleave_batch")
        return buf[:need.value].tobytes()

    def mates_times(self):
        return self._times("smr_mates_times", ("selected", "mates", "interleave", "d2h"))

    def rows_fmt_batch(self, num, den):
        num = np.ascontiguousarray(num, dtype=np.uint32)
        den = np.ascontiguousarray(den, dtype=np.uint32)
        out = np.zeros((len(num), 16), dtype=np.uint8)
        self._chk(self.L.smr_rows_fmt_batch(self.h, len(num), num.ctypes.data, den.ctypes.data, out.ctypes.data), "smr_rows_fmt_batch")
        return [bytes(r).rstrip(b"\0").decode() for r in out] if len(num) < 4096 else out.view("S16").ravel().astype(str).tolist()

    def reset_state(self):
        self._chk(self.L.smr_state_reset(self.h), "smr_state_reset")

    def import_state(self, records):
        if isinstance(records, tuple):
            blob, off = records
            blob = np.ascontiguousarray(blob, dtype=np.uint8)
            off = np.ascontiguousarray(off, dtype=np.uint64)
            if blob.size == 0:
                blob = np.zeros(1, dtype=np.uint8)
            self._chk(self.L.smr_state_import(self.h, blob.ctypes.data, off.ctypes.data, len(off) - 1), "smr_state_import")
            return
        off = np.zeros(len(records) + 1, dtype=np.uint64)
        if records:
            off[1:] = np.cumsum([len(r) for r in records], dtype=np.uint64)
        blob = np.frombuffer(b"".join(records) + b"\0", dtype=np.uint8)
        self._chk(self.L.smr_state_import(self.h, blob.ctypes.data, off.ctypes.data, len(records)), "smr_state_import")

    def export_state(self):
        n = self.n_reads
        off = np.zeros(n + 1, dtype=np.uint64)
        need = C.c_uint64(0)
        self._chk(self.L.smr_state_export(self.h, None, 0, off.ctypes.data, n, C.byref(need)), "smr_state_export")
        blob = np.zeros(need.value, dtype=np.uint8)
        if need.value:
            self._chk(self.L.smr_state_export(self.h, blob.ctypes.data, need.value, off.ctypes.data, n, C.byref(need)), "smr_state_export")
        return blob, off

    def export_records(self):
        blob, off = self.export_state()
        raw = blob.tobytes()
        return [raw[int(off[i]):int(off[i + 1])] for i in range(len(off) - 1)]

    def import_counters(self, values, n_db):
        if isinstance(values, dict):
            values = [values["num_aligned"], values["num_short"]] + list(values["reads_matched_per_db"])
        if len(values) != 2 + n_db:
            raise SmrError("import_counters: %d values for n_db = %d (expected %d)" % (len(values), n_db, 2 + n_db))
        arr = (C.c_uint64 * (2 + n_db))(*[int(v) for v in values])
        self._chk(self.L.smr_counters_import(self.h, arr, n_db), "smr_counters_import")

    def align_part(self, slot, params):
        self._chk(self.L.smr_align_part(self.h, slot, C.byref(params)), "smr_align_part")

    def traceback(self, slot, params):
        self._chk(self.L.smr_traceback(self.h, slot, C.byref(params)), "smr_traceback")

    def idcov_part(self, slot, params, min_id, min_cov):
        self._chk(self.L.smr_idcov_part(self.h, slot, C.byref(params), float(min_id), float(min_cov)), "smr_idcov_part")

    def idcov_counters(self):
        out = (C.c_uint64 * 4)()
        self._chk(self.L.smr_idcov_counters(self.h, out), "smr_idcov_counters")
        return dict(n_yid_ycov=out[0], n_yid_ncov=out[1], n_nid_ycov=out[2], num_denovo=out[3])

    def idcov_counters_device(self):
        p = C.c_void_p()
        n = C.c_uint32()
        self._chk(self.L.smr_idcov_counters_device(self.h, C.byref(p), C.byref(n)), "smr_idcov_counters_device")
        return p.value, n.value

    def idcov_batch(self, reads, refs, cigars, read_begin, read_end, readlen, min_id, min_cov):
        n = len(reads)
        ro = np.zeros(n + 1, dtype=np.uint64); fo = np.zeros(n + 1, dtype=np.uint64); co = np.zeros(n + 1, dtype=np.uint64)
        ro[1:] = np.cumsum([len(x) for x in reads]); fo[1:] = np.cumsum([len(x) for x in refs]); co[1:] = np.cumsum([len(x) for x in cigars])
        rb = np.frombuffer(b"".join(bytes(x) for x in reads) + b"\0", dtype=np.uint8).copy(); fb = np.frombuffer(b"".join(bytes(x) for x in refs) + b"\0", dtype=np.uint8).copy()
        cg = np.concatenate([np.asarray(x, dtype=np.uint32) for x in cigars] + [np.zeros(1, dtype=np.uint32)])
        b1 = np.asarray(read_begin, dtype=np.int32); e1 = np.asarray(read_end, dtype=np.int32); rl = np.asarray(readlen, dtype=np.uint32)
        out = np.zeros((max(n, 1), 4), dtype=np.uint32)
        self._chk(self.L.smr_idcov_batch(self.h, n, rb.ctypes.data, ro.ctypes.data, fb.ctypes.data, fo.ctypes.data, cg.ctypes.data, co.ctypes.data,
                                         b1.ctypes.data, e1.ctypes.data, rl.ctypes.data, float(min_id), float(min_cov), out.ctypes.data), "smr_idcov_batch")
        return out[:n]

    def counters(self, n_db=1):
        out = (C.c_uint64 * (2 + n_db))()
        self._chk(self.L.smr_counters(self.h, out, n_db), "smr_counters")
        return dict(num_aligned=out[0], num_short=out[1], reads_matched_per_db=[out[2 + i] for i in range(n_db)])

    def counters_device(self):
        p = C.c_void_p()
        n = C.c_uint32()
        self._chk(self.L.smr_counters_device(self.h, C.byref(p), C.byref(n)), "smr_counters_device")
        return p.value, n.value

    def counters_accumulate(self, d_acc, n_u64):
        self._chk(self.L.smr_counters_accumulate(self.h, d_acc, n_u64), "smr_counters_accumulate")

    def fetch(self):
        self._chk(self.L.smr_results_fetch(self.h), "smr_results_fetch")

    def record(self, i):
        n = self.L.smr_result_record(self.h, i, None, 0)
        if n == 0:
            return b""
        buf = C.create_string_buffer(n)
        self.L.smr_result_record(self.h, i, buf, n)
        return buf.raw

    def records(self):
        return [self.record(i) for i in range(self.n_reads)]

    def record_batch(self, batch, i):
        n = self.L.smr_result_record_batch(self.h, batch, i, None, 0)
        if n == 0:
            return b""
        buf = C.create_string_buffer(n)
        self.L.smr_result_record_batch(self.h, batch, i, buf, n)
        return buf.raw

    def is_hit(self, i):
        return bool(self.L.smr_result_is_hit(self.h, i))

    def seed_scan(self, slot, params, strand, pass_):
        n = C.c_uint64()
        self._chk(self.L.smr_seed_scan(self.h, slot, C.byref(params), strand, pass_, C.byref(n)), "smr_seed_scan")
        return n.value

    def seed_hits(self):
        n = C.c_uint64()
        self._chk(self.L.smr_seed_hits_fetch(self.h, None, 0, C.byref(n)), "smr_seed_hits_fetch")
        arr = np.zeros((max(n.value, 1), 3), dtype=np.uint32)
        self._chk(self.L.smr_seed_hits_fetch(self.h, arr.ctypes.data, n.value, C.byref(n)), "smr_seed_hits_fetch")
        return arr[: n.value]

    def seed_tuples(self):
        meta = (C.c_uint32 * 8)()
        self._chk(self.L.smr_seed_tuples_fetch(self.h, None, 0, None, 0, meta), "smr_seed_tuples_fetch")
        tup = np.zeros(max(meta[0], 1), dtype=np.uint64)
        cbase = np.zeros(meta[2] + 1, dtype=np.uint32)
        self._chk(self.L.smr_seed_tuples_fetch(self.h, tup.ctypes.data, len(tup), cbase.ctypes.data, len(cbase), meta), "smr_seed_tuples_fetch")
        return tup[: meta[0]], cbase, dict(n=meta[0], n_fwd=meta[1], nc=meta[2], fb=meta[3], cb=meta[4], nkh=meta[5], ccap=meta[6], redo=meta[7])

    def tuning(self):
        buf = C.create_string_buffer(max(self.L.smr_tuning_text(self.h, None, 0), 1))
        self.L.smr_tuning_text(self.h, buf, len(buf))
        return {k: int(v) for k, v in (line.split("=") for line in buf.value.decode().splitlines())}

    def seed_pool_info(self):
        info = (C.c_uint64 * 4)()
        self._chk(self.L.smr_seed_pool_info(self.h, info), "smr_seed_pool_info")
        return dict(words=info[0], grown=info[1], hi=info[2], inline=bool(info[3]))

    def cand_info_enable(self, on=True):
        self._chk(self.L.smr_cand_info_enable(self.h, int(bool(on))), "smr_cand_info_enable")

    def cand_info(self):
        info = (C.c_uint64 * 13)()
        self._chk(self.L.smr_cand_info(self.h, info), "smr_cand_info")
        return dict(attempts=info[0], retries=dict(HITCAP=info[1], POOL=info[2], PAIRS=info[3], REDO=info[4], SCAP=info[5]), chain_ext=bool(info[6]),
                    chain_scap=info[7], keys_cap=info[8], pairs_cap=info[9], hits_cap=info[10], routes_on=bool(info[11]), routes_n=info[12])

    def cand_routes(self):
        n = self.cand_info()["routes_n"]
        out = np.zeros(max(n, 1), dtype=np.uint8)
        self._chk(self.L.smr_cand_routes(self.h, out.ctypes.data, n), "smr_cand_routes")
        return out[:n]

    def prof_reset(self):
        self._chk(self.L.smr_prof_reset(self.h), "smr_prof_reset")

    def prof(self):
        p = capi.Prof()
        self._chk(self.L.smr_prof_get(self.h, C.byref(p)), "smr_prof_get")
        return p

    def prof_kernels(self):
        a = (capi.Kprof * 16)()
        n = C.c_uint32()
        self._chk(self.L.smr_prof_kernels(self.h, a, 16, C.byref(n)), "smr_prof_kernels")
        return {a[i].name.decode(): {"ms": a[i].ms, "launches": int(a[i].launches), "bytes": int(a[i].bytes)} for i in range(n.value)}

    def close(self):
        if self.h:
            self.L.smr_destroy(self.h)
            self.h = None


def align(engine, reads, index_parts, params_per_index, with_cigar=True, max_alignments_per_read=None, id_cov=None, resume=None, first_index_num=0):
    if id_cov is not None and not with_cigar:
        raise SmrError("align: id_cov needs the CIGARs (with_cigar=True)")
    if id_cov is not None and resume is not None:
        raise SmrError("align: id_cov with resume is not supported here (the pass needs the references of the earlier --ref as well)")
    p0 = params_per_index[0]
    slots = max_alignments_per_read or (p0.num_alignments if p0.num_alignments > 0 else 32)
    if reads is not None:
        engine.upload_reads(reads, slots)
    if resume is not None:
        records, counters = resume
        engine.import_state(records)
        if counters is not None:
            engine.import_counters(counters, len(counters["reads_matched_per_db"]) if isinstance(counters, dict) else len(counters) - 2)
    n_idx = len(index_parts)
    single = sum(len(parts) for parts in index_parts) == 1
    for idx_num, parts in enumerate(index_parts):
        for part, ix in enumerate(parts):
            p = params_per_index[idx_num]
            p.index_num = first_index_num + idx_num
            p.part = part
            p.is_last_index_part = int(idx_num == n_idx - 1 and part == len(parts) - 1)
            engine.upload_index(ix, 0)
            engine.align_part(0, p)
            if with_cigar:
                engine.traceback(0, p)
            if id_cov is not None and single:
                engine.idcov_part(0, p, id_cov[0], id_cov[1])
            engine.unload_index(0)
    if id_cov is not None and not single:
        for idx_num, parts in enumerate(index_parts):
            for part, ix in enumerate(parts):
                p = params_per_index[idx_num]
                p.index_num = first_index_num + idx_num
                p.part = part
                engine.upload_index(ix, 0)
                engine.idcov_part(0, p, id_cov[0], id_cov[1])
                engine.unload_index(0)
    engine.fetch()


def align_resident(engine, index_slots, params_per_index, with_cigar=True, id_cov=None):
    if index_slots and not isinstance(index_slots[0], (list, tuple)):
        index_slots = [index_slots]
    n_idx = len(index_slots)
    for idx_num, slots in enumerate(index_slots):
        for part, slot in enumerate(slots):
            p = params_per_index[idx_num]
            p.index_num = idx_num
            p.part = part
            p.is_last_index_part = int(idx_num == n_idx - 1 and part == len(slots) - 1)
            engine.align_part(slot, p)
            if with_cigar:
                engine.traceback(slot, p)
    if id_cov is not None:
        if not with_cigar:
            raise SmrError("align_resident: id_cov needs the CIGARs (with_cigar=True)")
        for idx_num, slots in enumerate(index_slots):
            for part, slot in enumerate(slots):
                p = params_per_index[idx_num]
                p.index_num = idx_num
                p.part = part
                engine.idcov_part(slot, p, id_cov[0], id_cov[1])
    engine.fetch()
```

Measured before the change: 57.24 million.

## Add per-mini-trie neighbourhood bitmap to skip hopeless seed searches

At index upload, builds a device bitmap per root3 mini-trie. Each bitmap marks pattern prefixes that sit within edit distance one of some stored string. The seed kernel probes this bitmap and drops lanes whose pattern cannot match, so futile pigeonhole searches are skipped. This costs an extra global load per seed and a large device allocation, capped by a budget tuning value. It also adds a one-time build kernel, a census pass, and counters for probed, passed and empty lanes.

```diff
diff --git a/include/smr_hip.h b/include/smr_hip.h
--- a/include/smr_hip.h
+++ b/include/smr_hip.h
@@ -107,6 +107,8 @@
 int smr_index_pigeonhole(smr_index*, const uint32_t** pg, uint64_t* pg_words, const uint32_t** root3, uint64_t* root3_words, char* err, size_t errcap);
 int smr_seed_tuples_fetch(smr_ctx*, uint64_t* tuples, uint64_t cap_tuples, uint32_t* cbase, uint32_t cap_cbase, uint32_t meta[8]);
 int smr_seed_pool_info(smr_ctx*, uint64_t info[4]);
+int smr_seed_nbmap_info(smr_ctx*, int slot, uint64_t info[9]);
+int smr_seed_nbmap_fetch(smr_ctx*, int slot, uint64_t first, uint64_t n, uint32_t* out, uint64_t cap_words);
 #define SMR_ROUTE_RECORD 1u
 #define SMR_ROUTE_GATHER 2u
 #define SMR_ROUTE_CHAIN 4u
diff --git a/sortmerna_amd/capi.py b/sortmerna_amd/capi.py
--- a/sortmerna_amd/capi.py
+++ b/sortmerna_amd/capi.py
@@ -78,7 +78,7 @@
     "smr_params_default", "smr_params_refused", "smr_index_load_files", "smr_index_build", "smr_index_build_gpu", "smr_index_write_files", "smr_index_save", "smr_index_load_flat", "smr_index_selfcheck", "smr_index_free",
     "smr_index_get_info", "smr_minimal_score", "smr_minimal_score_split", "smr_refstats_corrected_split", "smr_reads_pack", "smr_reads_load_fastx", "smr_reads_load_fastx_mt", "smr_reads_load_fastx_text", "smr_reads_is_fastq", "smr_reads_record_text", "smr_reads_free", "smr_reads_slice",
     "smr_reads_digest", "smr_reads_count", "smr_reads_total_len", "smr_reads_min_len", "smr_reads_max_len", "smr_create", "smr_device_count", "smr_destroy",
-    "smr_last_error", "smr_tuning_text", "smr_index_upload", "smr_index_check_device", "smr_index_pigeonhole", "smr_seed_tuples_fetch", "smr_seed_pool_info", "smr_cand_info_enable", "smr_cand_info", "smr_cand_routes", "smr_index_unload", "smr_batch_select", "smr_set_seed_mode", "smr_reads_upload", "smr_reads_upload_batch", "smr_reads_upload_fastx", "smr_reads_upload_fastx_batch", "smr_reads_upload_fastx_file", "smr_fastx_info", "smr_fastx_times", "smr_fastx_split", "smr_fastx_split_times", "smr_rows_part", "smr_rows_times", "smr_rows_fmt_batch", "smr_pairwise_part", "smr_pairwise_times", "smr_state_reset", "smr_align_part",
+    "smr_last_error", "smr_tuning_text", "smr_index_upload", "smr_index_check_device", "smr_index_pigeonhole", "smr_seed_tuples_fetch", "smr_seed_pool_info", "smr_seed_nbmap_info", "smr_seed_nbmap_fetch", "smr_cand_info_enable", "smr_cand_info", "smr_cand_routes", "smr_index_unload", "smr_batch_select", "smr_set_seed_mode", "smr_reads_upload", "smr_reads_upload_batch", "smr_reads_upload_fastx", "smr_reads_upload_fastx_batch", "smr_reads_upload_fastx_file", "smr_fastx_info", "smr_fastx_times", "smr_fastx_split", "smr_fastx_split_times", "smr_rows_part", "smr_rows_times", "smr_rows_fmt_batch", "smr_pairwise_part", "smr_pairwise_times", "smr_state_reset", "smr_align_part",
     "smr_traceback", "smr_counters", "smr_counters_device", "smr_state_import", "smr_state_export", "smr_counters_import", "smr_results_fetch", "smr_result_record", "smr_result_record_batch", "smr_counters_accumulate",
     "smr_result_is_hit", "smr_seed_scan", "smr_seed_hits_fetch", "smr_sw_selfcheck", "smr_sw_mode", "smr_walk_rounds", "smr_ssw_batch", "smr_sw16_batch", "smr_sw16_prefix_batch", "smr_walk_prefix_stats", "smr_sw16_launches", "smr_sw16_f16", "smr_sw_long_rows", "smr_cigar_batch", "smr_idcov_part", "smr_idcov_counters", "smr_idcov_counters_device", "smr_idcov_batch", "smr_prof_reset", "smr_prof_get", "smr_prof_kernels", "smr_refstats_corrected", "smr_report_open",
     "smr_report_set_db", "smr_report_set_part", "smr_report_add", "smr_report_add_pair", "smr_report_add_fastx", "smr_report_skip_fastx", "smr_report_add_rows", "smr_report_skip_rows", "smr_report_add_pairwise", "smr_report_skip_pairwise", "smr_report_set_cmdline", "smr_report_otu_count", "smr_report_otu_merge", "smr_report_close", "smr_report_last_error",
@@ -162,6 +162,10 @@
     L.smr_seed_tuples_fetch.argtypes = [vp, vp, u64, vp, u32, C.POINTER(u32)]
     L.smr_seed_pool_info.restype = i32
     L.smr_seed_pool_info.argtypes = [vp, C.POINTER(u64)]
+    L.smr_seed_nbmap_info.restype = i32
+    L.smr_seed_nbmap_info.argtypes = [vp, i32, C.POINTER(u64)]
+    L.smr_seed_nbmap_fetch.restype = i32
+    L.smr_seed_nbmap_fetch.argtypes = [vp, i32, u64, u64, vp, u64]
     L.smr_cand_info_enable.restype = i32
     L.smr_cand_info_enable.argtypes = [vp, i32]
     L.smr_cand_info.restype = i32
diff --git a/sortmerna_amd/csrc/smr_devbuf.hpp b/sortmerna_amd/csrc/smr_devbuf.hpp
--- a/sortmerna_amd/csrc/smr_devbuf.hpp
+++ b/sortmerna_amd/csrc/smr_devbuf.hpp
@@ -37,6 +37,13 @@
     cap_ = count;
     return 0;
   }
+  bool try_alloc(size_t count) {
+    release();
+    if (count == 0) count = 1;
+    if (hipMalloc((void**)&p_, count * sizeof(T)) != hipSuccess) { p_ = nullptr; (void)hipGetLastError(); return false; }
+    cap_ = count;
+    return true;
+  }
   int reserve(smr_ctx* c, size_t need) { return (p_ && cap_ >= need) ? 0 : alloc(c, need); }
   int reserve_headroom(smr_ctx* c, size_t total, size_t slack) {
     return cap_ >= total + slack ? 0 : alloc(c, (size_t)((total + (total >> 3) + 4095u) & ~4095ull));
diff --git a/sortmerna_amd/csrc/smr_engine.hip b/sortmerna_amd/csrc/smr_engine.hip
--- a/sortmerna_amd/csrc/smr_engine.hip
+++ b/sortmerna_amd/csrc/smr_engine.hip
@@ -22,6 +22,7 @@
 #include "smr_gunzip.hpp"
 #include "smr_ibuild.hpp"
 #include "smr_pgbuild.hpp"
+#include "smr_nbmap.hpp"
 #include "smr_hostmem.hpp"
 #include "smr_devbuf.hpp"
 #include "smr_stage.hpp"
@@ -36,6 +37,7 @@
   bool used = false;
   DevBuf<Lookup> lookup; DevBuf<uint32_t> trie, pos_off; DevBuf<uint2> pos_arr;
   DevBuf<uint32_t> pg, root3, lkc;
+  DevBuf<uint32_t> nbmap; uint32_t nb_words = 0, nb_mask = 0, nb_slabs = 0; uint64_t nb_info[6] = {0, 0, 0, 0, 0, 0};
   DevBuf<uint8_t> ref_seq; DevBuf<uint64_t> ref_off;
   uint32_t n_refs = 0, n_ids = 0, lnwin = 0;
   uint32_t ref_any_n = 1;
@@ -286,7 +288,7 @@
 }
 
 DIndex dindex(const DevIndex& d) {
-  DIndex x; x.lookup = d.lookup; x.trie = d.trie; x.pg = d.pg; x.lkc = d.lkc; x.root3 = reinterpret_cast<const uint2*>(d.root3.get()); x.pos_off = d.pos_off; x.pos_arr = d.pos_arr; x.ref_seq = d.ref_seq; x.ref_off = d.ref_off;
+  DIndex x; x.lookup = d.lookup; x.trie = d.trie; x.pg = d.pg; x.lkc = d.lkc; x.root3 = reinterpret_cast<const uint2*>(d.root3.get()); x.nbmap = d.nbmap; x.nb_words = d.nb_words; x.nb_mask = d.nb_mask; x.pos_off = d.pos_off; x.pos_arr = d.pos_arr; x.ref_seq = d.ref_seq; x.ref_off = d.ref_off;
   x.n_refs = d.n_refs; x.n_ids = d.n_ids; x.lnwin = d.lnwin; x.partialwin = d.lnwin / 2; x.ref_any_n = d.ref_any_n;
   return x;
 }
@@ -470,6 +472,57 @@
   d.pg_words = W;
   return SMR_OK;
 }
+
+int build_nbmap(smr_ctx* c, DevIndex& d, uint32_t nk, uint32_t pw) {
+  int rc;
+  d.nb_words = d.nb_mask = d.nb_slabs = 0;
+  for (auto& x : d.nb_info) x = 0;
+  if ((rc = d.nbmap.alloc(c, 4))) return rc;
+  HIPCHK(c, hipMemsetAsync(d.nbmap, 0xFF, 16, c->stream));
+  const Tuning& t = c->tune;
+  if (t.seed_nbmap == 0) return SMR_OK;
+  const uint32_t nb = 2 * nk;
+  DevBuf<unsigned long long> cen;
+  if ((rc = cen.alloc(c, 2))) return rc;
+  HIPCHK(c, hipMemsetAsync(cen, 0, 16, c->stream));
+  launch(c, smr::k_nbmap_census, dim3((nb + 255) / 256), dim3(256), 0, (const uint32_t*)d.root3, nb, cen);
+  unsigned long long h[2] = {0, 0};
+  HIPCHK(c, hipMemcpyAsync(h, cen, 16, hipMemcpyDeviceToHost, c->stream));
+  HIPCHK(c, hipStreamSynchronize(c->stream));
+  d.nb_info[3] = h[0]; d.nb_info[4] = h[1];
+  if (h[0] == 0 || (t.seed_nbmap == 1 && h[1] < (unsigned long long)t.nbmap_min * h[0])) return SMR_OK;
+  uint64_t budget = t.nbmap_bytes;
+  if (t.seed_nbmap == 1) {
+    size_t mem_free = 0, mem_total = 0;
+    if (hipMemGetInfo(&mem_free, &mem_total) != hipSuccess) { (void)hipGetLastError(); return SMR_OK; }
+    budget = std::min<uint64_t>(budget, (uint64_t)mem_free / 4);
+  }
+  uint32_t drop = t.nbmap_drop;
+  auto bytes_at = [&](uint32_t s) { return (uint64_t)nb * smr::nb_slab_words(pw, s) * 4; };
+  while (drop < pw && pw - drop >= NB_MIN_CHARS && (pw - drop > NB_MAX_CHARS || bytes_at(drop) > budget)) drop++;
+  if (drop >= pw || pw - drop < NB_MIN_CHARS) { say(t, "index part: no search bitmap (none of at least %u pattern chars fits %.2f GB)\n", NB_MIN_CHARS, budget * 1e-9); return SMR_OK; }
+  const uint64_t bytes = bytes_at(drop);
+  DevBuf<uint32_t> map;
+  if (bytes > t.nbmap_alloc_max || !map.try_alloc(bytes / 4)) {
+    say(t, "index part: no search bitmap (no room for %.2f GB on the device)\n", bytes * 1e-9);
+    return SMR_OK;
+  }
+  const uint32_t words = (uint32_t)smr::nb_slab_words(pw, drop);
+  struct Ev { hipEvent_t e = nullptr; ~Ev() { if (e) (void)hipEventDestroy(e); } } e0, e1;
+  HIPCHK(c, hipEventCreate(&e0.e)); HIPCHK(c, hipEventCreate(&e1.e));
+  HIPCHK(c, hipEventRecord(e0.e, c->stream));
+  launch(c, smr::k_nbmap_build, dim3(nb), dim3(256), (size_t)words * 4, (const uint32_t*)d.root3, (const uint32_t*)d.pg, pw, drop, map.get());
+  HIPCHK(c, hipEventRecord(e1.e, c->stream));
+  HIPCHK(c, hipStreamSynchronize(c->stream));
+  HIPCHK(c, hipGetLastError());
+  float ms = 0;
+  (void)hipEventElapsedTime(&ms, e0.e, e1.e);
+  d.nbmap = std::move(map);
+  d.nb_words = words; d.nb_mask = (1u << (2 * (pw - drop))) - 1u; d.nb_slabs = nb;
+  d.nb_info[0] = 1; d.nb_info[1] = drop; d.nb_info[2] = bytes; d.nb_info[5] = (uint64_t)(ms * 1000.0f);
+  say(t, "index part: search bitmap %.2f GB (%u of %u pattern chars, %.0f strings per mini-trie), built in %.1f ms\n", bytes * 1e-9, pw - drop, pw, (double)h[1] / (double)h[0], ms);
+  return SMR_OK;
+}
 }
 
 extern "C" int smr_index_upload(smr_ctx* c, const smr_index* ix, int slot) {
@@ -513,6 +566,7 @@
   if ((rc = d.ref_seq.alloc(c, ix->ref_seq.size() + 64))) return rc;
   if ((rc = d.ref_off.alloc(c, ix->ref_off.size()))) return rc;
   HIPCHK(c, hipMemcpyAsync(d.ref_seq, ix->ref_seq.data(), ix->ref_seq.size(), hipMemcpyHostToDevice, c->stream));
+  if ((rc = build_nbmap(c, d, (uint32_t)ix->lookup.size(), ix->lnwin / 2))) return rc;
   d.ref_any_n = (!ix->ref_seq.empty() && memchr(ix->ref_seq.data(), 4, ix->ref_seq.size())) ? 1u : 0u;
   HIPCHK(c, hipMemcpyAsync(d.ref_off, ix->ref_off.data(), ix->ref_off.size() * 8, hipMemcpyHostToDevice, c->stream));
   HIPCHK(c, hipStreamSynchronize(c->stream));
@@ -998,6 +1052,27 @@
   return SMR_OK;
 }
 
+extern "C" int smr_seed_nbmap_info(smr_ctx* c, int slot, uint64_t info[9]) {
+  if (!c || !info || slot < 0 || slot >= 64) return SMR_ERR_ARG;
+  HIPCHK(c, hipSetDevice(c->device));
+  const DevIndex& d = c->idx[slot];
+  for (int q = 0; q < 6; q++) info[q] = d.used ? d.nb_info[q] : 0;
+  std::vector<unsigned long long> h(C_TOTAL, 0ull);
+  if (c->b->d_ctr) { int rc = read_ctr(c, h); if (rc) return rc; }
+  info[6] = h[C_NB_PROBED]; info[7] = h[C_NB_PASSED]; info[8] = h[C_NB_EMPTY];
+  return SMR_OK;
+}
+extern "C" int smr_seed_nbmap_fetch(smr_ctx* c, int slot, uint64_t first, uint64_t n, uint32_t* out, uint64_t cap_words) {
+  if (!c || !out || slot < 0 || slot >= 64 || !c->idx[slot].used) return SMR_ERR_ARG;
+  HIPCHK(c, hipSetDevice(c->device));
+  const DevIndex& d = c->idx[slot];
+  if (!d.nb_words) { set_err(c, "smr_seed_nbmap_fetch: the part has no bitmap"); return SMR_ERR_STATE; }
+  if (first > d.nb_slabs || n > d.nb_slabs - first) return SMR_ERR_ARG;
+  if (cap_words < n * d.nb_words) return SMR_ERR_CAPACITY;
+  if (n) HIPCHK(c, hipMemcpy(out, d.nbmap + first * d.nb_words, n * d.nb_words * 4, hipMemcpyDeviceToHost));
+  return SMR_OK;
+}
+
 extern "C" int smr_cand_info_enable(smr_ctx* c, int on) {
   if (!c) return SMR_ERR_ARG;
   c->cinfo_on = on != 0;
diff --git a/sortmerna_amd/csrc/smr_engine_chain.hpp b/sortmerna_amd/csrc/smr_engine_chain.hpp
--- a/sortmerna_amd/csrc/smr_engine_chain.hpp
+++ b/sortmerna_amd/csrc/smr_engine_chain.hpp
@@ -222,6 +222,7 @@
     for (int k = 0; k < C_SHARD_W; k++) {
       if (k < C_SHARD_X) h[C_WINDOWS + k] += h[C_SHARDS + C_SHARD_W * s + k];
       else if (k < C_SHARD_X + C_SHARD_NX) h[C_TUP_F + k - C_SHARD_X] += h[C_SHARDS + C_SHARD_W * s + k];
+      else if (k >= C_SHARD_NB && k < C_SHARD_NB + 3) h[C_NB_PROBED + k - C_SHARD_NB] += h[C_SHARDS + C_SHARD_W * s + k];
       h[C_SHARDS + C_SHARD_W * s + k] = 0;
     }
   unsigned long long mx = 0;
diff --git a/sortmerna_amd/csrc/smr_kernels.hpp b/sortmerna_amd/csrc/smr_kernels.hpp
--- a/sortmerna_amd/csrc/smr_kernels.hpp
+++ b/sortmerna_amd/csrc/smr_kernels.hpp
@@ -15,6 +15,8 @@
   const uint32_t* trie;
   const uint32_t* pg;
   const uint2* root3;
+  const uint32_t* nbmap;
+  uint32_t nb_words, nb_mask;
   const uint32_t* pos_off;
   const uint2* pos_arr;
   const uint8_t* ref_seq;
@@ -85,10 +87,11 @@
   C_ERR_HITCAP, C_ERR_POOL, C_ERR_SLOTS, C_ERR_PAIRS, C_ERR_CIGAR, C_ERR_TRACE, C_POOL_CURSOR, C_WORK_NEXT,
   C_CIGAR_CURSOR, C_TRACE_NEXT, C_ERR_SCAP, C_ERR_REDO, C_TRACE_DEFER, C_BEGIN_N, C_BEGIN_NEXT, C_FETCH_N, C_SW_SPEC, C_SW_SPEC_USED, C_SEED_REDO,
   C_TUP_F, C_TUP_ALL, C_B_KEYS, C_B_PG0, C_B_PG1, C_B_FIN,
-  C_IDCOV, C_IDCOV_FEW = C_IDCOV + 4, C_IDCOV_MANY, C_IDCOV_NOCIG, C_COUNT = 112,
-  C_NSHARD = 64, C_SHARD_W = 32, C_SHARD_X = 9, C_SHARD_NX = 6, C_SHARD_PH = 16, C_SHARDS = C_COUNT, C_PCUR = C_SHARDS + C_SHARD_W * C_NSHARD, C_PCUR_STRIDE = 16 , C_TOTAL = C_PCUR + C_NSHARD * C_PCUR_STRIDE
-};
-static_assert(C_IDCOV_NOCIG < C_COUNT, "counter block");
+  C_IDCOV, C_IDCOV_FEW = C_IDCOV + 4, C_IDCOV_MANY, C_IDCOV_NOCIG,
+  C_NB_PROBED, C_NB_PASSED, C_NB_EMPTY, C_COUNT = 112,
+  C_NSHARD = 64, C_SHARD_W = 32, C_SHARD_X = 9, C_SHARD_NX = 6, C_SHARD_PH = 16, C_SHARD_NB = 23, C_SHARDS = C_COUNT, C_PCUR = C_SHARDS + C_SHARD_W * C_NSHARD, C_PCUR_STRIDE = 16 , C_TOTAL = C_PCUR + C_NSHARD * C_PCUR_STRIDE
+};
+static_assert(C_NB_EMPTY < C_COUNT, "counter block");
 __device__ __forceinline__ void ctr_add(unsigned long long* ctr, int idx, unsigned long long v) {
   atomicAdd(&ctr[C_SHARDS + (blockIdx.x & (C_NSHARD - 1)) * C_SHARD_W + (idx >= C_TUP_F ? C_SHARD_X + idx - C_TUP_F : idx - C_WINDOWS)], v);
 }
diff --git a/sortmerna_amd/csrc/smr_nbmap.hpp b/sortmerna_amd/csrc/smr_nbmap.hpp
--- /dev/null
+++ b/sortmerna_amd/csrc/smr_nbmap.hpp
@@ -0,0 +1,55 @@
+#pragma once
+
+namespace smr {
+
+#define NB_MIN_CHARS 4u
+#define NB_MAX_CHARS 9u
+
+__host__ __device__ inline uint32_t nb_cands(uint32_t pw) { return 8u * pw + 2u; }
+__host__ __device__ inline uint32_t nb_candidate(uint32_t T, uint32_t pw, uint32_t c) {
+  const uint32_t m = (1u << (2 * pw)) - 1u;
+  if (c == 0) return T & m;
+  c -= 1;
+  if (c < 3 * pw) return (T & m) ^ ((c % 3u + 1u) << (2 * (c / 3u)));
+  c -= 3 * pw;
+  if (c < pw + 1) { const uint32_t lo = (1u << (2 * c)) - 1u; return ((T & lo) | ((T >> 2) & ~lo)) & m; }
+  c -= pw + 1;
+  const uint32_t j = c >> 2, lo = (1u << (2 * j)) - 1u;
+  return ((T & lo) | ((c & 3u) << (2 * j)) | ((T & ~lo) << 2)) & m;
+}
+__host__ __device__ inline uint64_t nb_slab_words(uint32_t pw, uint32_t drop) { return (uint64_t)1 << (2 * (pw - drop) - 5); }
+
+__global__ void __launch_bounds__(256) k_nbmap_census(const uint32_t* __restrict__ root3, uint32_t nb, unsigned long long* __restrict__ out) {
+  const uint32_t i = blockIdx.x * blockDim.x + threadIdx.x;
+  const bool have = i < nb && root3[2 * i] != NONE;
+  const unsigned long long n = have ? root3[2 * i + 1] & 0xFFFFFFu : 0u;
+  const unsigned long long present = __popcll(__ballot(have));
+  unsigned long long sum = n;
+  for (int o = 32; o; o >>= 1) sum += __shfl_xor(sum, o, 64);
+  if (lane_id() == 0 && present) { atomicAdd(&out[0], present); atomicAdd(&out[1], sum); }
+}
+
+__global__ void __launch_bounds__(256) k_nbmap_build(const uint32_t* __restrict__ root3, const uint32_t* __restrict__ pg, uint32_t pw, uint32_t drop,
+                                                    uint32_t* __restrict__ nbmap) {
+  SMR_DYN_LDS(uint32_t, slab);
+  const uint32_t i = blockIdx.x, words = (uint32_t)nb_slab_words(pw, drop), pm = (1u << (2 * (pw - drop))) - 1u;
+  uint32_t* out = nbmap + (size_t)i * words;
+  const uint32_t rx = root3[2 * i], ry = root3[2 * i + 1];
+  if (rx == NONE) {
+    for (uint32_t w = threadIdx.x; w < words; w += blockDim.x) out[w] = 0;
+    return;
+  }
+  for (uint32_t w = threadIdx.x; w < words; w += blockDim.x) slab[w] = 0;
+  __syncthreads();
+  const uint32_t n = ry & 0xFFFFFFu, nc = nb_cands(pw);
+  const uint32_t* tt = pg_strings_at(pg, rx, ry);
+  for (unsigned long long q = threadIdx.x; q < (unsigned long long)n * nc; q += blockDim.x) {
+    const uint32_t t = (uint32_t)(q / nc), c = (uint32_t)(q - (unsigned long long)t * nc);
+    const uint32_t T = tt[t], P = nb_candidate(T, pw, c);
+    if (lev1_entry(P, T, pw) & 1u) { const uint32_t b = P & pm; atomicOr(&slab[b >> 5], 1u << (b & 31u)); }
+  }
+  __syncthreads();
+  for (uint32_t w = threadIdx.x; w < words; w += blockDim.x) out[w] = slab[w];
+}
+
+}
diff --git a/sortmerna_amd/csrc/smr_seed_pg.hpp b/sortmerna_amd/csrc/smr_seed_pg.hpp
--- a/sortmerna_amd/csrc/smr_seed_pg.hpp
+++ b/sortmerna_amd/csrc/smr_seed_pg.hpp
@@ -134,7 +134,9 @@
   const uint32_t stride = gridDim.x * (blockDim.x >> 6);
   __shared__ unsigned long long s_acc[PG_WAVES][3];
   unsigned long long* acc = s_acc[threadIdx.x >> 6];
-  if (lane == 0) { acc[0] = 0; acc[1] = 0; acc[2] = 0; }
+  __shared__ uint32_t s_nbc[PG_WAVES][3];
+  uint32_t* nbc = s_nbc[threadIdx.x >> 6];
+  if (lane == 0) { acc[0] = 0; acc[1] = 0; acc[2] = 0; nbc[0] = 0; nbc[1] = 0; nbc[2] = 0; }
   for (uint32_t it = uni(blockIdx.x * (blockDim.x >> 6) + (threadIdx.x >> 6)); ; it += stride) {
   uint32_t vb = 0;
   { const int ck = chunk_of(it, vb); if (ck == 0) break; if (ck == 2) continue; }
@@ -143,6 +145,7 @@
   bool mine = DIR ? (pos >= n_fwd && pos < n_tup) : pos < n_fwd;
   uint32_t nh = 0, P9 = 0, slot = 0, gfl = 0;
   uint2 rt = make_uint2(NONE, 0);
+  uint32_t nbw = 0;
   uint32_t n_rep = 0;
   {
     const bool hit = pf && pf_vb == vb;
@@ -162,7 +165,9 @@
       while (pos >= nx) { c++; nx = sb.cbase[c + 1]; }
       SeedKey tk;
       tk.slot = (uint32_t)t; tk.chars = (uint32_t)(t >> 32) & ((1u << sb.cb) - 1u); tk.key = (c << sb.fb) | (uint32_t)(t >> (32u + sb.cb));
-      rt = ix.root3[2 * (tk.key - (DIR ? sb.nkh : 0u)) + DIR];
+      const uint32_t ri = 2 * (tk.key - (DIR ? sb.nkh : 0u)) + DIR;
+      rt = ix.root3[ri];
+      nbw = ix.nbmap[(size_t)ri * ix.nb_words + ((tk.chars & ix.nb_mask) >> 5)];
       P9 = tk.chars; slot = tk.slot;
       if (DIR == 1) gfl = sb.gflag[slot >> 11];
     }
@@ -171,6 +176,8 @@
   if (mine) {
     if (DIR == 1 && ((gfl >> ((slot >> 6) & 31u)) & 1u) && ((sb.zbits[slot >> 5] >> (slot & 31u)) & 1u)) mine = false;
   }
+  const uint32_t n_prob = (uint32_t)__popcll(__ballot(mine));
+  if (mine && !((nbw >> (P9 & 31u)) & 1u)) mine = false;
   if (lane == 0) s_ncand = 0;
   __syncthreads();
   GPH(0)
@@ -248,6 +255,10 @@
       if (p < sb.cap_redo) sb.redo[p] = vb; else atomicAdd(&ctr[C_ERR_REDO], 1ull);
     }
     continue;
+  }
+  if (ix.nb_words) {
+    const uint32_t n_pass = (uint32_t)__popcll(__ballot(srch)), n_empty = (uint32_t)__popcll(__ballot(srch && hd[lane] == PG_NIL));
+    if (lane == 0) { nbc[0] += n_prob; nbc[1] += n_pass; nbc[2] += n_empty; }
   }
   own[lane] = 0;
   __builtin_amdgcn_wave_barrier();
@@ -301,12 +312,14 @@
   unsigned long long w_bytes = (uint32_t)__popcll(__ballot(counted)) * ((uint32_t)sizeof(SeedTup) + 8u + (DIR ? 1u : 0u))
                              + 32u * (uint32_t)__popcll(__ballot(srch && cA)) + 4u * (uint32_t)__popcll(__ballot(wr));
   w_bytes += 4ull * wtot + 4ull * total + 8ull * min(s_ncand, ccap) + 2u + 8ull * n_rep;
+  if (ix.nb_words) w_bytes += 4ull * (uint32_t)__popcll(__ballot(counted));
   if (lane == 0) { acc[0] += w_node; acc[1] += w_entry; acc[2] += w_bytes; }
 #ifdef SMR_SEED_PHASES
   GPH(5)
   if (lane == 0) for (int q = 0; q < 7; q++) if (tph[q]) { atomicAdd(&ctr[C_SHARDS + (vb & (C_NSHARD - 1)) * C_SHARD_W + C_SHARD_PH + q], tph[q]); tph[q] = 0; }
 #endif
   }
+  if (lane == 0 && nbc[0]) for (int q = 0; q < 3; q++) atomicAdd(&ctr[C_SHARDS + (blockIdx.x & (C_NSHARD - 1)) * C_SHARD_W + C_SHARD_NB + q], (unsigned long long)nbc[q]);
   if (lane == 0) { if (acc[0]) ctr_add(ctr, C_NODE, acc[0]); if (acc[1]) ctr_add(ctr, C_ENTRY, acc[1]); if (acc[2]) ctr_add(ctr, DIR ? C_B_PG1 : C_B_PG0, acc[2]); }
 }
 
diff --git a/sortmerna_amd/csrc/smr_tuning.hpp b/sortmerna_amd/csrc/smr_tuning.hpp
--- a/sortmerna_amd/csrc/smr_tuning.hpp
+++ b/sortmerna_amd/csrc/smr_tuning.hpp
@@ -27,6 +27,11 @@
   uint32_t walk_assume = 3;
   uint32_t walk_prefix = 44;
   int sw16_f16 = 1;
+  int seed_nbmap = 1;
+  uint32_t nbmap_drop = 1;
+  uint32_t nbmap_min = 128;
+  uint64_t nbmap_bytes = 24ull << 30;
+  uint64_t nbmap_alloc_max = ~0ull;
   bool begins_x4 = false;
   bool pg_host = false;
   bool trace_global_rows = false;
@@ -69,6 +74,11 @@
   if ((e = getenv("SMR_WALK_ASSUME"))) t.walk_assume = (uint32_t)atoi(e);
   if ((e = getenv("SMR_WALK_PREFIX"))) t.walk_prefix = (uint32_t)std::max(0, std::min(100, atoi(e)));
   if ((e = getenv("SMR_SW16_F16"))) t.sw16_f16 = atoi(e) != 0 ? 1 : 0;
+  if ((e = getenv("SMR_SEED_NBMAP"))) t.seed_nbmap = std::max(0, std::min(2, atoi(e)));
+  if ((e = getenv("SMR_SEED_NBMAP_DROP"))) t.nbmap_drop = (uint32_t)std::max(0, std::min(10, atoi(e)));
+  if ((e = getenv("SMR_SEED_NBMAP_MIN"))) t.nbmap_min = (uint32_t)std::max(0, atoi(e));
+  if ((e = getenv("SMR_SEED_NBMAP_BYTES"))) t.nbmap_bytes = strtoull(e, nullptr, 0);
+  if ((e = getenv("SMR_SEED_NBMAP_ALLOC_MAX"))) t.nbmap_alloc_max = strtoull(e, nullptr, 0);
   t.begins_x4 = getenv("SMR_BEGINS_X4") != nullptr;
   if ((e = getenv("SMR_PG_HOST"))) t.pg_host = atoi(e) != 0;
   t.trace_global_rows = getenv("SMR_TRACE_GLOBAL_ROWS") != nullptr;
diff --git a/sortmerna_amd/engine.py b/sortmerna_amd/engine.py
--- a/sortmerna_amd/engine.py
+++ b/sortmerna_amd/engine.py
@@ -795,6 +795,16 @@
         buf = C.create_string_buffer(max(self.L.smr_tuning_text(self.h, None, 0), 1))
         self.L.smr_tuning_text(self.h, buf, len(buf))
         return {k: int(v) for k, v in (line.split("=") for line in buf.value.decode().splitlines())}
+
+    def seed_nbmap_info(self, slot=0):
+        info = (C.c_uint64 * 9)()
+        self._chk(self.L.smr_seed_nbmap_info(self.h, slot, info), "smr_seed_nbmap_info")
+        return dict(zip(("built", "drop", "bytes", "tries", "strings", "build_us", "probed", "passed", "empty"), (int(x) for x in info)))
+
+    def seed_nbmap_fetch(self, slot, first, n, words_per_slab):
+        out = np.empty((n, words_per_slab), dtype=np.uint32)
+        self._chk(self.L.smr_seed_nbmap_fetch(self.h, slot, first, n, out.ctypes.data_as(C.c_void_p), out.size), "smr_seed_nbmap_fetch")
+        return out
 
     def seed_pool_info(self):
         info = (C.c_uint64 * 4)()
```

New measurement: 58.32 million, median of 6. 1.9% higher.
